# KTH-RPL/neural_graph_mapping

Hardware: AMD Instinct MI355X
Metric: ray-samples/sec (train step: fwd+loss+bwd+Adam, 4096 rays x 128 samples per GPU) (higher is better)
Workload: dtype f32 via 3xbf16 split, fp32 accumulate (hidden-layer matrix products, forward and backward); everything else f32; 1 GPU; M1: 8 fields x 512 rays x (64 coarse + 64 depth-guided) samples per GPU, Fourier(64,raw)+2x64 MLP, nrgbd compositing, NRGBD intrinsics; fields_per_gpu=8, rays_per_field=512, samples_per_ray=128, ranks_seen=1, spin_up_steps=200, jitter=in-kernel Philox, launch=hipGraph replay

## Files before the change

include/ngm_hip.h:

```cpp
#ifndef NGM_HIP_H
#define NGM_HIP_H

#include <stdint.h>

#ifdef __cplusplus
extern "C" {
#endif

#define NGM_ABI_VERSION 11
#define NGM_MAX_LAYERS 4
#define NGM_NUM_LOSS_SUMS 16

enum ngm_status {
  NGM_OK = 0,
  NGM_E_INVALID = -1,
  NGM_E_UNSUPPORTED = -2,
  NGM_E_WORKSPACE = -3,
  NGM_E_HIP = -4
};

enum ngm_encoding { NGM_ENC_NONE = 0, NGM_ENC_FOURIER = 1, NGM_ENC_NERF = 2, NGM_ENC_PERMUTO = 3, NGM_ENC_TRIPLANE = 4 };
enum ngm_triplane_mode { NGM_TRI_SUM = 0, NGM_TRI_PRODUCT = 1, NGM_TRI_CONCAT = 2 };
enum ngm_skip_mode { NGM_SKIP_NO = 0, NGM_SKIP_ADD = 1, NGM_SKIP_CONCAT = 2 };
enum ngm_matmul_mode { NGM_MATMUL_F32 = 0, NGM_MATMUL_BF16X3 = 1, NGM_MATMUL_AUTO = 2 };
// ... 11 lines not shown
  NGM_LS_TSDF_SUM = 6,
  NGM_LS_TSDF_CNT = 7,
  NGM_LS_TERM_SUM = 8,
  NGM_LS_TERM_CNT = 9,
  NGM_LS_PHOTO_L1_SUM = 10
};

typedef struct ngm_field_cfg {
  int32_t encoding;
  int32_t dim_enc;
  int32_t raw_coords;
  int32_t num_octaves;
  int32_t start_octave;
  int32_t num_layers;
  int32_t dim_hidden;
  int32_t dim_out;
  int32_t scale_mode;
  float field_radius;
  int32_t nr_levels;
  int32_t nr_feat_per_level;
  int32_t log2_hashmap_size;
  float coarsest_scale, finest_scale;
  float level_scale[16 * 3];
  int32_t skip_mode;
  int32_t matmul_mode;
  int32_t tri_resolution;
  int32_t tri_mode;
  int32_t activation_stash;
  int32_t hash_grad_atomics;
} ngm_field_cfg;
enum ngm_activation_stash { NGM_STASH_FULL = 0, NGM_STASH_HALF = 1 };
enum ngm_hash_grad_atomics { NGM_HASH_ATOMICS_EXACT = 0, NGM_HASH_ATOMICS_FLOAT = 1 };

int ngm_permuto_fill_scales(ngm_field_cfg* cfg);

typedef struct ngm_params {
  const float* enc_w;
  int64_t enc_w_stride;
  const float* w[NGM_MAX_LAYERS + 1];
  int64_t w_stride[NGM_MAX_LAYERS + 1];
  const float* b[NGM_MAX_LAYERS + 1];
  int64_t b_stride[NGM_MAX_LAYERS + 1];
  const int64_t* field_index;
  const float* lattice;
  int64_t lattice_stride;
  const float* shift;
  int64_t shift_stride;
  int32_t dtype;
  int32_t reserved_;
  const float* planes;
  int64_t planes_stride;
  const float* neus_sd;
  int64_t neus_sd_stride;
} ngm_params;

typedef struct ngm_grads {
  float* enc_w;
  int64_t enc_w_stride;
  float* w[NGM_MAX_LAYERS + 1];
  int64_t w_stride[NGM_MAX_LAYERS + 1];
  float* b[NGM_MAX_LAYERS + 1];
  int64_t b_stride[NGM_MAX_LAYERS + 1];
  float* lattice;
  int64_t lattice_stride;
  float* neus_sd;
  float* planes;
  int64_t planes_stride;
} ngm_grads;

typedef enum ngm_photometric_mode { NGM_PHOTO_L1 = 0, NGM_PHOTO_L2 = 1, NGM_PHOTO_GAUSSIAN_NLL = 2 } ngm_photometric_mode;
typedef enum ngm_depth_mode { NGM_DEPTH_HUBER = 0, NGM_DEPTH_GAUSSIAN_NLL = 1, NGM_DEPTH_LAPLACIAN_NLL = 2 } ngm_depth_mode;

typedef struct ngm_render_cfg {
  int32_t geometry_mode;
  int32_t num_samples_coarse;
  int32_t num_samples_guided;
  int32_t overwrite_behind_camera;
  float geometry_factor;
  float color_factor;
  float truncation_distance;
  float range_depth_guided;
  float fx, fy, cx, cy;
  float w_termination, w_photometric, w_depth, w_freespace, w_tsdf;
  float huber_delta;
  float term_threshold;
  int32_t photometric_mode;
  int32_t depth_mode;
} ngm_render_cfg;

typedef struct ngm_rays {
  int32_t F, R;
  const int64_t* ijs;
  const float* c2ws;
  int32_t c2w_per_ray;
  int32_t philox_offset_autoinc;
  const float* near;
  const float* far;
  const float* gt;
  float near_const, far_const;
  const float* field_pos;
  const float* field_quat;
  const float* u_coarse;
  const float* u_guided;
  const float* lin_coarse;
  const float* lin_guided;
  uint64_t philox_seed;
// ... 61 lines not shown
int ngm_composite_bwd(const ngm_render_cfg* cfg, int64_t N, int32_t S, const float* colors,
                      const float* geoms, const float* dists, const float* depths,
                      const float* neus_isds, const float* dC, const float* dD,
                      const float* dterm, float* d_colors, float* d_geoms, float* d_neus_isds,
                      void* stream);

int64_t ngm_render_workspace(const ngm_field_cfg* fcfg, const ngm_render_cfg* rcfg, int32_t F,
                             int32_t R, int32_t train);
int ngm_render_fwd(const ngm_field_cfg* fcfg, const ngm_render_cfg* rcfg,
                   const ngm_params* params, const ngm_rays* rays, const ngm_targets* targets,
                   const ngm_prediction* pred, float* loss_sums, void* workspace,
                   int64_t workspace_bytes, void* stream);
int ngm_render_bwd(const ngm_field_cfg* fcfg, const ngm_render_cfg* rcfg,
                   const ngm_params* params, const ngm_rays* rays, const ngm_targets* targets,
                   const ngm_prediction* pred, const float* loss_sums, const ngm_grads* grads,
                   float* loss_out, void* workspace, int64_t workspace_bytes, void* stream);
int ngm_render_bwd_seeded(const ngm_field_cfg* fcfg, const ngm_render_cfg* rcfg,
                          const ngm_params* params, const ngm_rays* rays, const float* d_rgbds,
                          const float* d_term, const float* d_geom_samples,
                          const ngm_grads* grads, void* workspace, int64_t workspace_bytes,
                          void* stream);
int ngm_render_bwd_seeded_vars(const ngm_field_cfg* fcfg, const ngm_render_cfg* rcfg,
                               const ngm_params* params, const ngm_rays* rays, const ngm_prediction* pred,
                               const float* d_rgbds, const float* d_color_vars, const float* d_depth_vars,
                               const float* d_term, const float* d_geom_samples, const ngm_grads* grads,
                               void* workspace, int64_t workspace_bytes, void* stream);
int ngm_render_read_samples(const ngm_field_cfg* fcfg, const ngm_render_cfg* rcfg, int32_t F,
                            int32_t R, int32_t S, const void* workspace, float* geoms, float* dists,
                            void* stream);

int ngm_adam_sparse(float* param, float* exp_avg, float* exp_avg_sq, int64_t stride,
                    const float* grad, int64_t grad_stride, const int64_t* field_index, int32_t F,
                    int64_t numel_per_field, int64_t step, float lr, float beta1, float beta2,
                    float eps, float weight_decay, void* stream);

typedef struct ngm_adam_tensor {
  float* param; float* exp_avg; float* exp_avg_sq;
  const float* grad;
  int64_t stride, grad_stride, numel;
  void* param_lp;
  int32_t lp_dtype;
  int32_t reserved_;
} ngm_adam_tensor;
int ngm_adam_sparse_multi(const ngm_adam_tensor* tensors, int32_t num_tensors, const int64_t* field_index,
                          int32_t F, int64_t step, int64_t* step_dev, float lr, float beta1, float beta2,
                          float eps, float weight_decay, int32_t advance_step_dev,
                          uint64_t* advance_philox_offset_dev, void* stream);
int ngm_render_bwd_adam(const ngm_field_cfg* fcfg, const ngm_render_cfg* rcfg, const ngm_params* params,
                        const ngm_rays* rays, const ngm_targets* targets, const ngm_prediction* pred,
                        const float* loss_sums, const ngm_grads* grads, const ngm_adam_tensor* mlp_tensors,
                        int32_t num_mlp_tensors, const ngm_adam_tensor* lattice_tensor, const int64_t* field_index,
                        int64_t step, int64_t* step_dev, float lr, float beta1, float beta2, float eps,
                        float weight_decay, float* loss_values, void* workspace, int64_t workspace_bytes, void* stream);
int ngm_render_fwd_counted(const ngm_field_cfg* fcfg, const ngm_render_cfg* rcfg,
                           const ngm_params* params, const ngm_rays* rays, const ngm_targets* targets,
                           const ngm_prediction* pred, float* loss_sums, void* workspace,
                           int64_t workspace_bytes, void* stream, const int32_t* num_active);
int ngm_render_bwd_counted(const ngm_field_cfg* fcfg, const ngm_render_cfg* rcfg,
                           const ngm_params* params, const ngm_rays* rays, const ngm_targets* targets,
                           const ngm_prediction* pred, const float* loss_sums, const ngm_grads* grads,
                           float* loss_out, void* workspace, int64_t workspace_bytes, void* stream,
                           const int32_t* num_active);
int ngm_render_bwd_adam_counted(const ngm_field_cfg* fcfg, const ngm_render_cfg* rcfg, const ngm_params* params,
                                const ngm_rays* rays, const ngm_targets* targets, const ngm_prediction* pred,
                                const float* loss_sums, const ngm_grads* grads, const ngm_adam_tensor* mlp_tensors,
                                int32_t num_mlp_tensors, const ngm_adam_tensor* lattice_tensor, const int64_t* field_index,
                                int64_t step, int64_t* step_dev, float lr, float beta1, float beta2, float eps,
                                float weight_decay, float* loss_values, void* workspace, int64_t workspace_bytes, void* stream,
                                const int32_t* num_active);
int ngm_step_advance(int64_t* step_dev, uint64_t* philox_offset_dev, void* stream);

int64_t ngm_field_eval_knn_workspace(int32_t num_fields, int64_t P, int32_t num_knn);
int ngm_field_eval_knn(const ngm_field_cfg* fcfg, const ngm_params* params, int32_t num_fields,
                       int64_t P, const float* points, const float* field_pos,
                       const float* field_quat, int32_t num_knn, float distance_factor,
                       float outside_value, float mask_radius, float* out, void* workspace, int64_t workspace_bytes,
                       void* stream);

int64_t ngm_render_eval_knn_workspace(const ngm_render_cfg* rcfg, int32_t num_fields, int32_t ray_block, int32_t num_knn);
int ngm_render_eval_knn(const ngm_field_cfg* fcfg, const ngm_render_cfg* rcfg, const ngm_params* params,
                        int32_t num_fields, const float* field_pos, const float* field_quat, const ngm_rays* rays,
                        int32_t num_knn, float distance_factor, float outside_value, float mask_radius, int32_t ray_block,
                        const ngm_prediction* pred, void* workspace, int64_t workspace_bytes, void* stream);

typedef struct ngm_keyframes {
  int32_t num_frames;
  int32_t height, width;
  int32_t reserved0;
  const float* c2ws;
  const float* rgbd;
  const int64_t* frame_to_store;
  float fx, fy, cx, cy;
} ngm_keyframes;

typedef struct ngm_target_out {
  int64_t* ijs;
  float* c2ws;
  float* near;
  float* far;
  float* gt;
  float* rgbds;
  uint8_t* rgb_mask;
  uint8_t* depth_mask;
  float* term_probs;
  uint8_t* term_mask;
} ngm_target_out;
// ... 174 lines not shown
```

neural_graph_mapping_amd/_capi.py:

```python
import ctypes as C
import os

HERE = os.path.dirname(os.path.abspath(__file__))
LIB_PATH = os.environ.get("NGM_LIB_PATH") or os.path.join(HERE, "lib", "libngm_hip.so")

NGM_MAX_LAYERS = 4
NGM_NUM_LOSS_SUMS = 16
ENC = {"none": 0, "fourier": 1, "nerf": 2, "permuto": 3, "triplane": 4}
TRI = {"sum": 0, "product": 1, "concat": 2}
SCALE = {"no": 0, "unit_ball": 1, "unit_cube": 2}
GEO = {"nrgbd": 0, "occupancy": 1, "density": 2, "neus": 3}
PHOTO = {"l1": 0, "l2": 1, "gaussian_nll": 2}
DEPTH = {"huber": 0, "gaussian_nll": 1, "laplacian_nll": 2}
LS = dict(PHOTO_SUM=0, PHOTO_CNT=1, DEPTH_SUM=2, DEPTH_CNT=3, FS_SUM=4, FS_CNT=5, TSDF_SUM=6,
          TSDF_CNT=7, TERM_SUM=8, TERM_CNT=9, PHOTO_L1_SUM=10)

f32p = C.c_void_p
LArr = C.c_void_p * (NGM_MAX_LAYERS + 1)
SArr = C.c_int64 * (NGM_MAX_LAYERS + 1)


class FieldCfg(C.Structure):
    _fields_ = [("encoding", C.c_int32), ("dim_enc", C.c_int32), ("raw_coords", C.c_int32),
                ("num_octaves", C.c_int32), ("start_octave", C.c_int32), ("num_layers", C.c_int32),
                ("dim_hidden", C.c_int32), ("dim_out", C.c_int32), ("scale_mode", C.c_int32),
                ("field_radius", C.c_float), ("nr_levels", C.c_int32), ("nr_feat_per_level", C.c_int32),
                ("log2_hashmap_size", C.c_int32), ("coarsest_scale", C.c_float), ("finest_scale", C.c_float),
                ("level_scale", C.c_float * 48), ("skip_mode", C.c_int32), ("matmul_mode", C.c_int32),
                ("tri_resolution", C.c_int32), ("tri_mode", C.c_int32),
                ("activation_stash", C.c_int32), ("hash_grad_atomics", C.c_int32)]


class Params(C.Structure):
    _fields_ = [("enc_w", f32p), ("enc_w_stride", C.c_int64), ("w", LArr), ("w_stride", SArr),
                ("b", LArr), ("b_stride", SArr), ("field_index", C.c_void_p),
                ("lattice", f32p), ("lattice_stride", C.c_int64), ("shift", f32p), ("shift_stride", C.c_int64),
                ("dtype", C.c_int32), ("reserved_", C.c_int32), ("planes", f32p), ("planes_stride", C.c_int64),
                ("neus_sd", f32p), ("neus_sd_stride", C.c_int64)]


class Grads(C.Structure):
    _fields_ = [("enc_w", f32p), ("enc_w_stride", C.c_int64), ("w", LArr), ("w_stride", SArr),
                ("b", LArr), ("b_stride", SArr), ("lattice", f32p), ("lattice_stride", C.c_int64), ("neus_sd", f32p),
                ("planes", f32p), ("planes_stride", C.c_int64)]


class RenderCfg(C.Structure):
    _fields_ = [("geometry_mode", C.c_int32), ("num_samples_coarse", C.c_int32),
                ("num_samples_guided", C.c_int32), ("overwrite_behind_camera", C.c_int32),
                ("geometry_factor", C.c_float), ("color_factor", C.c_float),
                ("truncation_distance", C.c_float), ("range_depth_guided", C.c_float),
                ("fx", C.c_float), ("fy", C.c_float), ("cx", C.c_float), ("cy", C.c_float),
                ("w_termination", C.c_float), ("w_photometric", C.c_float), ("w_depth", C.c_float),
                ("w_freespace", C.c_float), ("w_tsdf", C.c_float), ("huber_delta", C.c_float),
                ("term_threshold", C.c_float), ("photometric_mode", C.c_int32), ("depth_mode", C.c_int32)]


class Rays(C.Structure):
    _fields_ = [("F", C.c_int32), ("R", C.c_int32), ("ijs", C.c_void_p), ("c2ws", f32p),
                ("c2w_per_ray", C.c_int32), ("philox_offset_autoinc", C.c_int32), ("near", f32p), ("far", f32p),
                ("gt", f32p), ("near_const", C.c_float), ("far_const", C.c_float),
                ("field_pos", f32p), ("field_quat", f32p), ("u_coarse", f32p), ("u_guided", f32p),
                ("lin_coarse", f32p), ("lin_guided", f32p), ("philox_seed", C.c_uint64),
                ("philox_offset", C.c_uint64), ("pose_index", C.c_void_p), ("philox_offset_dev", C.c_void_p)]


class AdamTensor(C.Structure):
    _fields_ = [("param", f32p), ("exp_avg", f32p), ("exp_avg_sq", f32p), ("grad", f32p),
                ("stride", C.c_int64), ("grad_stride", C.c_int64), ("numel", C.c_int64),
                ("param_lp", C.c_void_p), ("lp_dtype", C.c_int32), ("reserved_", C.c_int32)]


class PeerExchange(C.Structure):
    _fields_ = [("world", C.c_int32), ("rank", C.c_int32), ("mailbox", C.c_void_p * 8), ("seq", C.c_void_p),
                ("status", C.c_void_p)]


class Targets(C.Structure):
    _fields_ = [("rgbds", f32p), ("depth_mask", C.c_void_p), ("term_mask", C.c_void_p),
                ("term_probs", f32p)]


class Prediction(C.Structure):
    _fields_ = [("rgbds", f32p), ("color_vars", f32p), ("depth_vars", f32p), ("term_probs", f32p)]


class Keyframes(C.Structure):
    _fields_ = [("num_frames", C.c_int32), ("height", C.c_int32), ("width", C.c_int32), ("reserved0", C.c_int32),
                ("c2ws", f32p), ("rgbd", f32p), ("frame_to_store", C.c_void_p),
                ("fx", C.c_float), ("fy", C.c_float), ("cx", C.c_float), ("cy", C.c_float)]

# ... 85 lines not shown
def grow_counts(num_current, num_fields, max_current, max_fields, num_train_fields):
    nf = min(max(num_fields, 0), max_fields)
    nc = min(max(num_current, 0), min(max_current, nf))
    n_obs = min(num_train_fields // 2, nc)
    return nf, nc, n_obs, max(min(num_train_fields - n_obs, nf - n_obs), 0)


_lib = None


def lib():
    global _lib
    if _lib is not None:
        return _lib
    if not os.path.exists(LIB_PATH):
        raise RuntimeError(
            f"{LIB_PATH} is missing: the HIP extension is not built. Run "
            "`python -m neural_graph_mapping_amd.build` (hipcc, gfx950). There is no CPU fallback.")
    L = C.CDLL(LIB_PATH)
    vp, i32, i64, f32 = C.c_void_p, C.c_int32, C.c_int64, C.c_float
    P = C.POINTER
    L.ngm_abi_version.restype = C.c_int
    L.ngm_permuto_fill_scales.argtypes = [P(FieldCfg)]
    L.ngm_permuto_fill_scales.restype = C.c_int
    L.ngm_last_error.restype = C.c_char_p
    L.ngm_device_info.argtypes = [P(C.c_int), C.c_char_p, C.c_int]
    L.ngm_sample_rays.argtypes = [P(RenderCfg), P(Rays), vp, vp, vp, vp]
    L.ngm_sample_rays_world.argtypes = [P(RenderCfg), P(Rays), vp, vp, vp, vp, vp]
    L.ngm_sample_rays_weighted.argtypes = [P(RenderCfg), P(Rays), i32, vp, vp, vp, vp, vp, vp]
    L.ngm_sample_rays_weighted.restype = C.c_int
    L.ngm_composite_fwd_packed.argtypes = [P(RenderCfg), i64, i32, vp, vp, vp, vp, vp, vp, vp, vp]
    L.ngm_sample_rays_world.restype = C.c_int
    L.ngm_composite_fwd_packed.restype = C.c_int
    L.ngm_field_eval_fwd.argtypes = [P(FieldCfg), P(Params), i32, i64, vp, vp, vp, vp, vp]
    L.ngm_encode_fwd.argtypes = [P(FieldCfg), P(Params), i32, i64, vp, vp, vp, vp, vp]
    L.ngm_encode_fwd.restype = C.c_int
    L.ngm_encode_bwd.argtypes = [P(FieldCfg), P(Params), i32, i64, vp, vp, vp, vp, P(Grads), vp, i64, vp]
    L.ngm_encode_bwd.restype = C.c_int
    L.ngm_encode_bwd_workspace.argtypes = [P(FieldCfg), i32, i64]
    L.ngm_encode_bwd_workspace.restype = i64
    L.ngm_field_eval_bwd.argtypes = [P(FieldCfg), P(Params), i32, i64, vp, vp, vp, vp, P(Grads), vp, i64, vp]
    L.ngm_field_eval_bwd_workspace.argtypes = [P(FieldCfg), i32, i64]
    L.ngm_field_eval_bwd_workspace.restype = i64
    L.ngm_field_eval_stash_bytes.argtypes = [P(FieldCfg), i32, i64]
    L.ngm_field_eval_stash_bytes.restype = i64
    L.ngm_field_eval_fwd_train.argtypes = [P(FieldCfg), P(Params), i32, i64, vp, vp, vp, vp, vp, i64, vp]
    L.ngm_field_eval_fwd_train.restype = C.c_int
    L.ngm_field_eval_bwd_stash.argtypes = [P(FieldCfg), P(Params), i32, i64, vp, vp, vp, vp, P(Grads), vp, i64, vp, i64, vp]
    L.ngm_field_eval_bwd_stash.restype = C.c_int
    L.ngm_composite_fwd.argtypes = [P(RenderCfg), i64, i32] + [vp] * 11 + [vp]
    L.ngm_composite_bwd.argtypes = [P(RenderCfg), i64, i32] + [vp] * 11 + [vp]
    L.ngm_render_workspace.argtypes = [P(FieldCfg), P(RenderCfg), i32, i32, i32]
    L.ngm_render_workspace.restype = i64
    L.ngm_render_fwd.argtypes = [P(FieldCfg), P(RenderCfg), P(Params), P(Rays), P(Targets),
                                 P(Prediction), vp, vp, i64, vp]
    L.ngm_render_bwd.argtypes = [P(FieldCfg), P(RenderCfg), P(Params), P(Rays), P(Targets),
                                 P(Prediction), vp, P(Grads), vp, vp, i64, vp]
    L.ngm_render_bwd_seeded.argtypes = [P(FieldCfg), P(RenderCfg), P(Params), P(Rays), vp, vp, vp,
                                        P(Grads), vp, i64, vp]
    L.ngm_render_bwd_seeded_vars.argtypes = [P(FieldCfg), P(RenderCfg), P(Params), P(Rays), P(Prediction), vp, vp, vp, vp, vp,
                                             P(Grads), vp, i64, vp]
    L.ngm_render_bwd_seeded_vars.restype = C.c_int
    L.ngm_render_bwd_adam.argtypes = [P(FieldCfg), P(RenderCfg), P(Params), P(Rays), P(Targets), P(Prediction), vp,
                                      P(Grads), P(AdamTensor), i32, P(AdamTensor), vp, i64, vp, f32, f32, f32, f32, f32,
                                      vp, vp, i64, vp]
    L.ngm_render_bwd_adam.restype = C.c_int
    for name in ("ngm_render_fwd", "ngm_render_bwd", "ngm_render_bwd_adam"):
        counted = getattr(L, name + "_counted")
        counted.argtypes = list(getattr(L, name).argtypes) + [vp]
        counted.restype = C.c_int
    L.ngm_render_read_samples.argtypes = [P(FieldCfg), P(RenderCfg), i32, i32, i32, vp, vp, vp, vp]
    L.ngm_adam_sparse.argtypes = [vp, vp, vp, i64, vp, i64, vp, i32, i64, i64, f32, f32, f32, f32, f32, vp]
    L.ngm_adam_sparse_multi.argtypes = [P(AdamTensor), i32, vp, i32, i64, vp, f32, f32, f32, f32, f32, i32, vp, vp]
    L.ngm_step_advance.argtypes = [vp, vp, vp]
    L.ngm_peer_mailbox_bytes.restype = i64
    L.ngm_peer_alloc.argtypes = [i64, P(C.c_void_p)]
    L.ngm_peer_free.argtypes = [vp]
    L.ngm_ipc_export.argtypes = [vp, C.c_char_p]
    L.ngm_ipc_open.argtypes = [C.c_char_p, P(C.c_void_p)]
    L.ngm_ipc_close.argtypes = [vp]
    L.ngm_loss_exchange.argtypes = [P(PeerExchange), vp, vp]
    L.ngm_peer_set_timeout.argtypes = [C.c_double]
    L.ngm_peer_set_timeout.restype = C.c_double
    L.ngm_adam_sparse_multi.restype = C.c_int
    L.ngm_step_advance.restype = C.c_int
    L.ngm_field_eval_knn.argtypes = [P(FieldCfg), P(Params), i32, i64, vp, vp, vp, i32, f32, f32, f32, vp, vp, i64, vp]
    L.ngm_field_eval_knn_workspace.argtypes = [i32, i64, i32]
    L.ngm_field_eval_knn_workspace.restype = i64
    L.ngm_render_eval_knn.argtypes = [P(FieldCfg), P(RenderCfg), P(Params), i32, vp, vp, P(Rays), i32, f32, f32, f32, i32,
                                      P(Prediction), vp, i64, vp]
    L.ngm_render_eval_knn.restype = C.c_int
    L.ngm_render_eval_knn_workspace.argtypes = [P(RenderCfg), i32, i32, i32]
    L.ngm_render_eval_knn_workspace.restype = i64
    L.ngm_target_visibility.argtypes = [P(Keyframes), i32, vp, i32, vp, f32, vp, vp, vp]
    L.ngm_target_rays.argtypes = [P(Keyframes), i32, i32, vp, f32, vp, vp, vp, P(TargetOut), vp]
    L.ngm_target_visibility.restype = C.c_int
    L.ngm_target_rays.restype = C.c_int
    L.ngm_target_sv_intersect.argtypes = [i32, i64, vp, vp, f32, vp, vp]
    L.ngm_target_sv_intersect.restype = C.c_int
    L.ngm_target_sv_rays.argtypes = [i32, i32, vp, f32, vp, vp, vp, i32, i32, f32, f32, f32, f32, P(TargetOut), vp]
    L.ngm_target_sv_rays.restype = C.c_int
    L.ngm_target_sample_mv_workspace.argtypes = [i32, i32, i32, i32]
    L.ngm_target_sample_mv_workspace.restype = i64
    L.ngm_target_sample_mv.argtypes = [P(Keyframes), P(TargetSample), P(TargetOut), vp, i64, vp]
    L.ngm_target_sample_mv.restype = C.c_int
    L.ngm_target_sample_mv_live_workspace.argtypes = [i32, i32, i32, i32]
    L.ngm_target_sample_mv_live_workspace.restype = i64
    L.ngm_target_sample_mv_live.argtypes = [P(Keyframes), P(TargetSample), P(TargetLive), P(TargetOut), vp, i64, vp]
    L.ngm_target_sample_mv_live.restype = C.c_int
    L.ngm_target_observed_fields_workspace.argtypes = [i32, i32]
    L.ngm_target_observed_fields_workspace.restype = i64
    L.ngm_target_observed_fields.argtypes = [P(ObservedFields), vp, i64, vp]
    L.ngm_target_observed_fields.restype = C.c_int
    L.ngm_field_counts_add.argtypes = [vp, vp, i32, vp, i32, vp]
    L.ngm_field_counts_add.restype = C.c_int
    L.ngm_fields_append.argtypes = [P(FieldsAppendArgs), vp]
    L.ngm_fields_append.restype = C.c_int
    L.ngm_target_sample_mv_grow_workspace.argtypes = [i32, i32, i32, i32]
    L.ngm_target_sample_mv_grow_workspace.restype = i64
    L.ngm_target_sample_mv_grow.argtypes = [P(Keyframes), P(TargetSample), P(TargetLive), vp, P(TargetOut), vp, i64, vp]
    L.ngm_target_sample_mv_grow.restype = C.c_int
    L.ngm_target_observed_fields_grow_workspace.argtypes = [i32, i32]
    L.ngm_target_observed_fields_grow_workspace.restype = i64
    L.ngm_target_observed_fields_grow.argtypes = [P(ObservedFields), vp, vp, i64, vp]
    L.ngm_target_observed_fields_grow.restype = C.c_int
    L.ngm_marching_cubes_workspace.argtypes = [i32, i32, i32]
    L.ngm_marching_cubes_workspace.restype = i64
    L.ngm_marching_cubes_count.argtypes = [vp, i32, i32, i32, f32, vp, vp, i64, vp]
    L.ngm_marching_cubes_emit.argtypes = [vp, i32, i32, i32, f32, vp, i64, vp, i64, vp, i64, vp]
    L.ngm_marching_cubes_tables.argtypes = [vp, vp]
    for name in ("ngm_marching_cubes_count", "ngm_marching_cubes_emit", "ngm_marching_cubes_tables"):
        getattr(L, name).restype = C.c_int
    L.ngm_debug_plan_bwd.argtypes = [P(FieldCfg), P(RenderCfg), i32, i64, i32, i32, i32, P(i32)]
    L.ngm_debug_plan_bwd.restype = C.c_int
    L.ngm_debug_plan_fwd.argtypes = [P(FieldCfg), P(RenderCfg), i32, i32, i64, i32, P(i32)]
    L.ngm_debug_plan_fwd.restype = C.c_int
    L.ngm_profile_enable.argtypes = [i32]
    L.ngm_profile_read.argtypes = [i32, P(C.c_double), P(i64)]
    for name in ("ngm_profile_enable", "ngm_profile_reset", "ngm_profile_read"):
        getattr(L, name).restype = C.c_int
    for name in ("ngm_sample_rays", "ngm_field_eval_fwd", "ngm_field_eval_bwd", "ngm_composite_fwd",
                 "ngm_composite_bwd", "ngm_render_fwd", "ngm_render_bwd", "ngm_render_bwd_seeded",
                 "ngm_render_read_samples", "ngm_adam_sparse", "ngm_field_eval_knn", "ngm_device_info"):
        getattr(L, name).restype = C.c_int
    _lib = L
    return L


EXPORTED = ["ngm_abi_version", "ngm_last_error", "ngm_device_info", "ngm_permuto_fill_scales", "ngm_sample_rays", "ngm_sample_rays_world", "ngm_sample_rays_weighted",
            "ngm_composite_fwd_packed",
            "ngm_field_eval_fwd", "ngm_encode_fwd", "ngm_encode_bwd", "ngm_encode_bwd_workspace", "ngm_field_eval_bwd", "ngm_field_eval_bwd_workspace",
            "ngm_field_eval_stash_bytes", "ngm_field_eval_fwd_train", "ngm_field_eval_bwd_stash",
            "ngm_composite_fwd", "ngm_composite_bwd", "ngm_render_workspace", "ngm_render_fwd",
            "ngm_render_bwd", "ngm_render_bwd_adam", "ngm_render_bwd_seeded", "ngm_render_bwd_seeded_vars", "ngm_render_read_samples", "ngm_adam_sparse",
            "ngm_field_eval_knn", "ngm_field_eval_knn_workspace", "ngm_render_eval_knn", "ngm_render_eval_knn_workspace", "ngm_adam_sparse_multi", "ngm_step_advance", "ngm_profile_enable", "ngm_profile_reset", "ngm_profile_read",
            "ngm_debug_phase_cycles", "ngm_debug_fwd_phase_cycles", "ngm_debug_last_bwd_variant", "ngm_debug_last_matmul", "ngm_debug_last_fwd_one_tile", "ngm_debug_last_comp_fused", "ngm_debug_disable_fused_comp", "ngm_debug_stash_mode", "ngm_debug_last_stash_mode", "ngm_debug_plan_bwd", "ngm_debug_plan_fwd", "ngm_target_visibility", "ngm_target_rays", "ngm_target_sv_intersect", "ngm_target_sv_rays",
            "ngm_target_sample_mv_workspace", "ngm_target_sample_mv",
            "ngm_target_sample_mv_live_workspace", "ngm_target_sample_mv_live", "ngm_target_observed_fields_workspace",
            "ngm_target_observed_fields", "ngm_field_counts_add",
            "ngm_fields_append", "ngm_target_sample_mv_grow_workspace", "ngm_target_sample_mv_grow",
            "ngm_target_observed_fields_grow_workspace", "ngm_target_observed_fields_grow",
            "ngm_render_fwd_counted", "ngm_render_bwd_counted", "ngm_render_bwd_adam_counted",
            "ngm_peer_mailbox_bytes", "ngm_peer_alloc", "ngm_peer_free", "ngm_ipc_export", "ngm_ipc_open", "ngm_ipc_close", "ngm_loss_exchange", "ngm_peer_set_timeout",
            "ngm_marching_cubes_workspace", "ngm_marching_cubes_count", "ngm_marching_cubes_emit", "ngm_marching_cubes_tables"]

NO_GRAD_PARAMS = frozenset({"_encoding.random_shift_per_level"})

KERNEL_IDS = dict(render_fwd=0, stash_bwd=1, field_bwd=2, grad_reduce=3, adam=4, points_fwd=5, composite_fwd=6,
                  composite_bwd=7, hash_grad=8, hash_reduce=9, loss_reduce=10, knn_assign=11, knn_eval=12, sampler=13)


NGM_OK, NGM_E_INVALID, NGM_E_UNSUPPORTED, NGM_E_WORKSPACE, NGM_E_HIP = 0, -1, -2, -3, -4


class NgmError(RuntimeError):

    def __init__(self, msg, code=None):
        super().__init__(msg)
        self.code = code


def check(rc, what=""):
    if rc != 0:
        msg = lib().ngm_last_error().decode(errors="replace")
        raise NgmError(f"{what} failed with status {rc}: {msg}", code=int(rc))


SKIP = {"no": 0, "add": 1, "concat": 2}
STASH = {"full": 0, "half": 1}
HASH_ATOMICS = {"exact": 0, "float": 1}
MATMUL = {"f32": 0, "bf16x3": 1, "auto": 2}


def field_cfg(encoding="fourier", dim_enc=64, raw_coords=True, num_octaves=8, start_octave=0,
              num_layers=2, dim_hidden=None, dim_out=4, scale_mode="unit_cube", field_radius=1.0,
              nr_levels=16, nr_feat_per_level=2, log2_hashmap_size=12, coarsest_scale=1.0, finest_scale=1e-4,
              skip_mode="no", matmul_mode="f32", resolution=32, num_components=64, tri_mode="sum"):
    if skip_mode not in SKIP:
        raise NotImplementedError(f"skip_mode={skip_mode!r}: 'no', 'add' and 'concat' have kernels; the reference's own "
                                  "constructor raises for 'rezero' (models.py:131-132)")
    if encoding == "nerf":
        dim_enc = 6 * num_octaves
    if encoding == "none":
        dim_enc = 3
    if encoding == "permuto":
        dim_enc = nr_levels * nr_feat_per_level
# ... 104 lines not shown
```

neural_graph_mapping_amd/csrc/ngm_api.hip:

```cpp
#include <hip/hip_runtime.h>
#include <stdio.h>
#include <stdlib.h>
#include <string.h>

#include "../../include/ngm_hip.h"
#include "ngm_launch.h"

int ngm_launch_sampler_weighted(const ngm_render_cfg* rc, const ngm_rays* rays, int S, int B, const float* boundaries,
                                const float* weights, float* points_cam, float* distances, float* dirs, hipStream_t st);
int ngm_launch_sampler(const ngm_render_cfg* rc, const ngm_rays* rays, int S, float* points_cam, float* distances,
                       float* dirs, float* points_world, hipStream_t st);
int ngm_launch_loss_values(const ngm_render_cfg* rc, const float* sums, float* out, hipStream_t st);
int ngm_launch_loss_reduce(const float* partials, int nblocks, float* sums, uint64_t* counter, hipStream_t st);
int ngm_launch_neus_sd_grad(const float* d_isd_rays, int F, int R, const float* neus_sd, int64_t sd_stride,
                            const int64_t* field_index, float* d_sd, hipStream_t st);
int ngm_launch_read_stash(const float4* sa, const float2* sb, int64_t n, float* geoms, float* dists, hipStream_t st);
int ngm_launch_adam(float* param, float* m, float* v, int64_t stride, const float* grad, int64_t gstride, int F, int64_t numel,
                    const AdamHyper& h, hipStream_t st);
int ngm_launch_adam_multi(const ngm_adam_tensor* tensors, int n, int F, const AdamHyper& h, int64_t* advance_step,
                          uint64_t* advance_offset, hipStream_t st, const int32_t* num_active = nullptr);
int ngm_launch_step_advance(int64_t* step_dev, uint64_t* off_dev, hipStream_t st);
int64_t ngm_mc_workspace_bytes(int nx, int ny, int nz);
int ngm_launch_mc_count(const float* vol, int nx, int ny, int nz, float iso, int64_t* counts, void* workspace,
                        int64_t workspace_bytes, hipStream_t st);
// ... 286 lines not shown
  switch (p.variant) {
    case 3: e = ngm_launch_field_bwd_b3(a, blocks, st); break;
    case 5: e = ngm_launch_hash_mlp_bwd(a, blocks, st); break;
    case 2: e = ngm_launch_field_bwd16s(a, blocks, st); break;
    case 1: e = ngm_launch_field_bwd16(a, blocks, st); break;
    case 0: e = ngm_launch_field_bwd(a, blocks, st); break;
  }
  return e ? fail(e, "MLP backward: the launcher does not take the planned problem (internal error)") : check_launch("ngm_field_bwd");
}

static int check_field_cfg(const ngm_field_cfg* fc, bool mlp = true) {
  if (!fc) return fail(NGM_E_INVALID, "field cfg is NULL");
  if (fc->dim_out != 4) return fail(NGM_E_UNSUPPORTED, "dim_out must be 4 (r,g,b,geometry)");
  if (fc->num_layers < 1 || fc->num_layers > NGM_MAX_LAYERS) return fail(NGM_E_UNSUPPORTED, "num_layers out of range");
  if (mlp && fc->num_layers > 3)
    return fail(NGM_E_UNSUPPORTED, "num_layers = 4: no entry point has a kernel for four hidden layers (1-2: everything; 3: forward only, 33..64-wide)");
  if (mlp && fc->num_layers == 3 && (fc->dim_enc <= 32 || fc->dim_hidden <= 32))
    return fail(NGM_E_UNSUPPORTED, "num_layers = 3 needs dim_enc and dim_hidden in 33..64: no entry point has a three-layer kernel for layers of 32 units or fewer");
  if (fc->encoding == NGM_ENC_PERMUTO) {
    if (fc->nr_feat_per_level != 2 || fc->nr_levels < 1 || fc->nr_levels > 16 || fc->dim_enc != 2 * fc->nr_levels)
      return fail(NGM_E_UNSUPPORTED, "permutohedral encoding: nr_feat_per_level must be 2, nr_levels <= 16, no concat_points");
    if (fc->log2_hashmap_size < 4 || fc->log2_hashmap_size > 24) return fail(NGM_E_UNSUPPORTED, "permutohedral: log2_hashmap_size out of range");
    if (!(fc->level_scale[0] > 0.f)) return fail(NGM_E_INVALID, "permutohedral: level_scale not filled (ngm_permuto_fill_scales)");
  }
  if (fc->encoding == NGM_ENC_NERF && fc->dim_enc != 6 * fc->num_octaves) return fail(NGM_E_INVALID, "nerf: dim_enc != 6*octaves");
  if (fc->encoding == NGM_ENC_TRIPLANE) {
    if (fc->tri_resolution < 2 || fc->tri_resolution > 4096 || fc->tri_mode < NGM_TRI_SUM || fc->tri_mode > NGM_TRI_CONCAT ||
        (fc->tri_mode == NGM_TRI_CONCAT && fc->dim_enc % 3))
      return fail(NGM_E_INVALID, "triplane: resolution / mode / dim_enc inconsistent");
  }
  if (fc->encoding == NGM_ENC_NONE && fc->dim_enc != 3) return fail(NGM_E_INVALID, "no encoding: dim_enc must be 3");
  if (fc->dim_enc < 1 || fc->dim_enc > 64 || fc->dim_hidden < 1 || fc->dim_hidden > 64)
    return fail(NGM_E_UNSUPPORTED, "dim_enc / dim_hidden must be <= 64");
  if (((fc->dim_enc + 31) / 32) != ((fc->dim_hidden + 31) / 32) && !(fc->dim_enc <= 32 && fc->dim_hidden <= 32))
    return fail(NGM_E_UNSUPPORTED, "dim_enc and dim_hidden must pad to the same multiple of 32");
  if (fc->skip_mode != NGM_SKIP_NO && fc->skip_mode != NGM_SKIP_ADD && fc->skip_mode != NGM_SKIP_CONCAT)
    return fail(NGM_E_UNSUPPORTED, "skip_mode: no / add / concat");
  if (fc->skip_mode == NGM_SKIP_ADD && fc->dim_hidden < fc->dim_enc)
    return fail(NGM_E_UNSUPPORTED, "skip_mode add: needs dim_hidden >= dim_enc");
  if (fc->activation_stash != NGM_STASH_FULL && fc->activation_stash != NGM_STASH_HALF)
    return fail(NGM_E_INVALID, "activation_stash: NGM_STASH_FULL / NGM_STASH_HALF (ABI 10: is the struct the caller built 276 bytes?)");
  if (fc->hash_grad_atomics != NGM_HASH_ATOMICS_EXACT && fc->hash_grad_atomics != NGM_HASH_ATOMICS_FLOAT)
    return fail(NGM_E_INVALID, "hash_grad_atomics: NGM_HASH_ATOMICS_EXACT / NGM_HASH_ATOMICS_FLOAT");
  return NGM_OK;
}
static int check_params(const ngm_field_cfg* fc, const ngm_params* pr) {
  if (!pr) return fail(NGM_E_INVALID, "params is NULL");
  if (fc->encoding == NGM_ENC_FOURIER && !pr->enc_w) return fail(NGM_E_INVALID, "fourier encoding needs enc_w");
  if (fc->encoding == NGM_ENC_PERMUTO && (!pr->lattice || !pr->shift)) return fail(NGM_E_INVALID, "permutohedral encoding needs lattice + shift");
  if (fc->encoding == NGM_ENC_TRIPLANE && (!pr->planes || pr->dtype != NGM_DT_F32)) return fail(NGM_E_INVALID, "triplane encoding needs fp32 planes");
  for (int l = 0; l <= fc->num_layers; ++l)
    if (!pr->w[l] || !pr->b[l]) return fail(NGM_E_INVALID, "missing layer weight/bias pointer");
  if (pr->dtype != NGM_DT_F32 && pr->dtype != NGM_DT_BF16 && pr->dtype != NGM_DT_F16) return fail(NGM_E_INVALID, "params.dtype");
  return NGM_OK;
}

extern "C" {

int ngm_abi_version(void) { return NGM_ABI_VERSION; }

int ngm_permuto_fill_scales(ngm_field_cfg* cfg) {
  if (!cfg || cfg->nr_levels < 1 || cfg->nr_levels > 16 || !(cfg->coarsest_scale > 0) || !(cfg->finest_scale > 0))
    return fail(NGM_E_INVALID, "ngm_permuto_fill_scales: bad configuration");
  const int L = cfg->nr_levels;
  const double la = log10((double)cfg->coarsest_scale), lb = log10((double)cfg->finest_scale);
  for (int l = 0; l < L; ++l) {
    double sig = (L == 1) ? cfg->coarsest_scale : pow(10.0, la + (lb - la) * (double)l / (double)(L - 1));
    if (l == 0) sig = cfg->coarsest_scale;
    if (l == L - 1 && L > 1) sig = cfg->finest_scale;
    for (int i = 0; i < 3; ++i) cfg->level_scale[3 * l + i] = (float)((1.0 / sqrt((double)((i + 1) * (i + 2)))) / sig);
  }
  return NGM_OK;
}
const char* ngm_last_error(void) { return g_err; }

int ngm_profile_enable(int32_t on) {
  std::lock_guard<std::mutex> lk(g_prof_mu);
  g_prof_on = on != 0;
  return NGM_OK;
}
int ngm_profile_reset(void) {
  std::lock_guard<std::mutex> lk(g_prof_mu);
  prof_drain();
  for (int k = 0; k < NGM_K_COUNT; ++k) { g_prof_ms[k] = 0; g_prof_n[k] = 0; }
  return NGM_OK;
}
int ngm_profile_read(int32_t kernel_id, double* total_ms, int64_t* launches) {
  if (kernel_id < 0 || kernel_id >= NGM_K_COUNT) return fail(NGM_E_INVALID, "bad kernel id");
  std::lock_guard<std::mutex> lk(g_prof_mu);
  prof_drain();
  if (total_ms) *total_ms = g_prof_ms[kernel_id];
  if (launches) *launches = g_prof_n[kernel_id];
  return NGM_OK;
}

static int check_keyframes(const ngm_keyframes* kf) {
  if (!kf || !kf->c2ws || !kf->rgbd || !kf->frame_to_store) return fail(NGM_E_INVALID, "target sampler: NULL keyframe argument");
  if (kf->num_frames < 1 || kf->height < 1 || kf->width < 1) return fail(NGM_E_INVALID, "target sampler: empty keyframe set");
  return NGM_OK;
}
int ngm_target_visibility(const ngm_keyframes* kf, int32_t F, const float* field_pos, int32_t num_offsets, const float* offsets,
                          float radius, uint8_t* kf_mask, float* bbox, void* stream) {
  int e = check_keyframes(kf);
  if (e) return e;
  if (F < 0 || num_offsets < 1 || !field_pos || !offsets || !kf_mask || !bbox) return fail(NGM_E_INVALID, "ngm_target_visibility: bad argument");
  if (F == 0) return NGM_OK;
// ... 451 lines not shown
  if (!cfg || !colors || !geoms || !dists || !depths || N < 0) return fail(NGM_E_INVALID, "ngm_composite_bwd: bad argument");
  if (N == 0) return NGM_OK;
  CompositeArgs a;
  memset(&a, 0, sizeof(a));
  a.rc = *cfg; a.N = N; a.S = S; a.colors = colors; a.geoms = geoms; a.dists = dists; a.depths = depths; a.isds = neus_isds;
  a.dC = dC; a.dD = dD; a.dterm = dterm; a.d_colors = d_colors; a.d_geoms = d_geoms; a.d_isds = d_neus_isds;
  const int rc = ngm_launch_composite_bwd(a, (hipStream_t)stream);
  if (rc) return fail(rc, "ngm_composite_bwd: S > 1024");
  return check_launch("ngm_composite_bwd");
}

struct RenderPlan {
  int S;
  FwdPlan fwd;
  BwdPlan bwd;
  int64_t p_pad;
  int64_t off_rayseed;
  int64_t off_raytab, off_stashA, off_stashB, off_losspart, off_gradpart, off_hash, off_act, act_layer_stride, total;
  int64_t off_dout, off_disd;
};
static RenderPlan plan_render(const ngm_field_cfg* fc, const ngm_render_cfg* rc, int F, int R, bool guided, bool train,
                              BwdAsk ask = BwdAsk(), bool counted = false) {
  RenderPlan p = RenderPlan();
  p.S = rc->num_samples_coarse + (guided ? rc->num_samples_guided : 0);
  FwdAsk fq;
  fq.rc = rc; fq.F = F; fq.n = R; fq.S = p.S; fq.counted = counted;
  p.fwd = plan_fwd(fc, fq);
  p.p_pad = param_pad(fc);
  int64_t o = 0;
  if (train) {
    const int64_t NR = (int64_t)F * R, NS = NR * p.S;
    p.off_raytab = o; o = align_up(o + NR * 8 * 4, 256);
    p.off_rayseed = o; o = align_up(o + NR * 8 * 4, 256);
    p.off_stashA = o; o = align_up(o + NS * 16, 256);
    p.off_stashB = o; o = align_up(o + NS * 8, 256);
    p.off_losspart = o; o = align_up(o + (int64_t)p.fwd.blocks * NGM_NUM_LOSS_SUMS * 4, 256);
    if (rc->geometry_mode == NGM_GEO_NEUS) {
      p.off_dout = o; o = align_up(o + NS * 16, 256);
      p.off_disd = o; o = align_up(o + NR * 4, 256);
    }
    ask.rc = rc; ask.F = F; ask.P = (int64_t)R * p.S;
    p.bwd = plan_mlp_bwd(fc, ask);
    p.off_gradpart = o; o = align_up(o + (int64_t)F * p.bwd.blocks_per_field * p.p_pad * 4, 256);
    p.off_hash = o; o = align_up(o + hash_scratch_bytes(fc, F, (int64_t)R * p.S), 256);
    if (p.bwd.stash_kind) {
      p.act_layer_stride = p.bwd.stash_kind == 1 ? align_up(NS, 32) * 64 + 2048 : align_up(NS, 32) * 32 + 1024;
      p.off_act = o; o = align_up(o + p.bwd.stash_layers * p.act_layer_stride * 4 + 64, 256);
    }
  }
  p.total = o + 256;
  return p;
}

int64_t ngm_render_workspace(const ngm_field_cfg* fcfg, const ngm_render_cfg* rcfg, int32_t F, int32_t R, int32_t train) {
  const int e = check_field_cfg(fcfg);
  if (e) return e;
  if (!rcfg || F < 1 || R < 1) return NGM_E_INVALID;
  return plan_render(fcfg, rcfg, F, R, true, train != 0).total;
}

static int check_enc_grads(const ngm_field_cfg* fc, const ngm_grads* grads, FieldBwdArgs& a) {
  if (fc->encoding == NGM_ENC_TRIPLANE) {
    if (!grads->planes || grads->planes_stride < tri_numel(fc)) return fail(NGM_E_INVALID, "triplane: grads.planes missing / stride too small");
    if (!a.tri_acc) return fail(NGM_E_WORKSPACE, "triplane: no accumulator scratch");
    a.planes_grad = grads->planes; a.planes_grad_stride = grads->planes_stride;
    return NGM_OK;
  }
  if (fc->encoding != NGM_ENC_PERMUTO) return NGM_OK;
  if (!grads->lattice) return fail(NGM_E_INVALID, "permutohedral: grads.lattice is NULL");
  const int64_t per = (int64_t)fc->nr_levels * ((int64_t)1 << fc->log2_hashmap_size) * 2;
  if (grads->lattice_stride < per) return fail(NGM_E_INVALID, "permutohedral: grads.lattice_stride too small");
  a.lattice_grad = grads->lattice; a.lattice_grad_stride = grads->lattice_stride;
  return NGM_OK;
}

static int check_render(const ngm_field_cfg* fc, const ngm_render_cfg* rc, const ngm_params* pr, const ngm_rays* rays) {
  int e = check_field_cfg(fc);
  if (e) return e;
  e = check_params(fc, pr);
  if (e) return e;
  if (!rc || !rays || !rays->ijs || !rays->c2ws || !rays->field_pos || !rays->field_quat)
    return fail(NGM_E_INVALID, "render: NULL ray argument");
  if (rays->F < 1 || rays->R < 1) return fail(NGM_E_INVALID, "render: empty batch");
  if (rc->geometry_mode == NGM_GEO_NEUS && !pr->neus_sd)
    return fail(NGM_E_INVALID, "fused render: the neus geometry mode needs params.neus_sd (the per-field _neus_sd, rm.py:641-644)");
  const int S = rc->num_samples_coarse + (rays->gt ? rc->num_samples_guided : 0);
  if (S < 1 || S > 1024) return fail(NGM_E_UNSUPPORTED, "fused render: samples per ray must be in [1,1024]");
  return NGM_OK;
}

static int check_counted(const char* who, const ngm_field_cfg* fc, const ngm_render_cfg* rc, const int32_t* num_active) {
  char msg[256];
  if (!num_active) {
    snprintf(msg, sizeof(msg), "%s: num_active is NULL (the un-suffixed entry point is the call for all F rows)", who);
    return fail(NGM_E_INVALID, msg);
  }
  const char* why = nullptr;
  if (rc && rc->geometry_mode == NGM_GEO_NEUS) why = "the neus geometry mode";
  else if (fc && fc->encoding == NGM_ENC_TRIPLANE) why = "the triplane encoding";
  else if (rc && (rc->photometric_mode == NGM_PHOTO_GAUSSIAN_NLL || rc->depth_mode != NGM_DEPTH_HUBER)) why = "the *_nll loss modes";
  if (why) {
    snprintf(msg, sizeof(msg), "%s: %s is outside the counted step (it launches over all F rows): slice the batch to its count and call the un-suffixed entry point", who, why);
    return fail(NGM_E_UNSUPPORTED, msg);
  }
  return NGM_OK;
}

static int render_fwd_impl(const ngm_field_cfg* fcfg, const ngm_render_cfg* rcfg, const ngm_params* params, const ngm_rays* rays,
                           const ngm_targets* targets, const ngm_prediction* pred, float* loss_sums, void* workspace,
                           int64_t workspace_bytes, void* stream, const int32_t* num_active) {
  int e = check_render(fcfg, rcfg, params, rays);
  if (e) return e;
  if (!pred) return fail(NGM_E_INVALID, "render_fwd: pred is NULL");
  const bool has_tg = targets != nullptr;
  const bool save = workspace != nullptr;
  if (has_tg && (!targets->rgbds || !targets->depth_mask)) return fail(NGM_E_INVALID, "render_fwd: incomplete targets");
  if (has_tg && targets->term_mask && !targets->term_probs) return fail(NGM_E_INVALID, "render_fwd: term_mask without term_probs");
  if (has_tg && !save) return fail(NGM_E_WORKSPACE, "render_fwd: targets need a workspace");
  if (save && (!pred->rgbds || !pred->term_probs)) return fail(NGM_E_INVALID, "render_fwd(save): pred.rgbds/term_probs required");
  const RenderPlan p = plan_render(fcfg, rcfg, rays->F, rays->R, rays->gt != nullptr, save, BwdAsk(), num_active != nullptr);
  if (p.fwd.status) return fail(p.fwd.status, p.fwd.why);
  if (save && workspace_bytes < p.total) return fail(NGM_E_WORKSPACE, "render_fwd: workspace too small");
  char* ws = reinterpret_cast<char*>(align_up((int64_t)workspace, 256));
  RenderFwdArgs a;
  memset(&a, 0, sizeof(a));
  a.fc = *fcfg; a.pr = *params; a.rc = *rcfg; a.rays = *rays; a.pred = *pred;
  a.fc.matmul_mode = p.fwd.matmul;
  if (p.fwd.neus) { a.neus_sd = params->neus_sd; a.neus_sd_stride = params->neus_sd_stride; }
  a.has_targets = has_tg ? 1 : 0;
  a.num_active = num_active;
  if (has_tg) a.tg = *targets;
  a.S = p.S; a.rays_per_block = p.fwd.rays_per_block; a.waves_per_block = p.fwd.waves; a.maxs = p.fwd.maxs;
  if (save) {
    a.raytab = reinterpret_cast<float*>(ws + p.off_raytab);
    if (has_tg) a.rayseed = reinterpret_cast<float*>(ws + p.off_rayseed);
    a.stashA = reinterpret_cast<float4*>(ws + p.off_stashA);
    a.stashB = reinterpret_cast<float2*>(ws + p.off_stashB);
    a.loss_partials = reinterpret_cast<float*>(ws + p.off_losspart);
    if (p.act_layer_stride) { a.act = reinterpret_cast<float*>(ws + p.off_act); a.act_layer_stride = p.act_layer_stride; }
    a.act_layers = p.bwd.half;
    static const bool timing = getenv("NGM_PHASE_TIMING") != nullptr;
    if (timing) {
      if (!g_debug_cycles_fwd) { (void)hipMalloc(&g_debug_cycles_fwd, NGM_FWD_DEBUG_WORDS * 8); (void)hipMemset(g_debug_cycles_fwd, 0, NGM_FWD_DEBUG_WORDS * 8); }
      a.debug_cycles = g_debug_cycles_fwd;
    }
  }
  e = ngm_launch_render_fwd(a, p.fwd, (hipStream_t)stream);
  if (e) return fail(e, no_instance);
  g_last_fwd[NGM_FWD_RENDER] = p.fwd;
  if (save) {
    note_forward_stash(workspace, p.bwd.half);
    note_forward_seeds(workspace, a.rayseed ? targets->rgbds : nullptr);
  }
  e = check_launch("ngm_render_fwd");
  if (e) return e;
  if (has_tg && loss_sums) {
    ngm_launch_loss_reduce(a.loss_partials, p.fwd.blocks, loss_sums,
                           (rays->philox_offset_autoinc && rays->philox_offset_dev) ? const_cast<uint64_t*>(rays->philox_offset_dev) : nullptr,
                           (hipStream_t)stream);
    e = check_launch("ngm_loss_reduce");
  }
  return e;
}
int ngm_render_fwd(const ngm_field_cfg* fcfg, const ngm_render_cfg* rcfg, const ngm_params* params, const ngm_rays* rays,
                   const ngm_targets* targets, const ngm_prediction* pred, float* loss_sums, void* workspace,
                   int64_t workspace_bytes, void* stream) {
  return render_fwd_impl(fcfg, rcfg, params, rays, targets, pred, loss_sums, workspace, workspace_bytes, stream, nullptr);
}
int ngm_render_fwd_counted(const ngm_field_cfg* fcfg, const ngm_render_cfg* rcfg, const ngm_params* params, const ngm_rays* rays,
                           const ngm_targets* targets, const ngm_prediction* pred, float* loss_sums, void* workspace,
                           int64_t workspace_bytes, void* stream, const int32_t* num_active) {
  const int e = check_counted("ngm_render_fwd_counted", fcfg, rcfg, num_active);
  if (e) return e;
  return render_fwd_impl(fcfg, rcfg, params, rays, targets, pred, loss_sums, workspace, workspace_bytes, stream, num_active);
// ... 14 lines not shown
    return fail(NGM_E_INVALID, "render_bwd: the *_nll loss modes need pred.color_vars and pred.depth_vars");
  char* ws = reinterpret_cast<char*>(align_up((int64_t)workspace, 256));
  FieldBwdArgs a;
  memset(&a, 0, sizeof(a));
  a.fc = *fcfg; a.pr = *params; a.F = rays->F; a.P = (int64_t)rays->R * p.S; a.S = p.S;
  a.num_active = num_active;
  carve_hash_scratch(fcfg, rays->F, a.P, ws + p.off_hash, a);
  int e = check_enc_grads(fcfg, grads, a);
  if (e) return e;
  sb.rc = *rcfg; sb.F = rays->F; sb.R = rays->R; sb.S = p.S;
  sb.num_active = num_active;
  if (!rays->gt) sb.rc.w_freespace = sb.rc.w_tsdf = 0.f;
  sb.stashA = reinterpret_cast<float4*>(ws + p.off_stashA);
  sb.stashB = reinterpret_cast<const float2*>(ws + p.off_stashB);
  sb.raytab = reinterpret_cast<const float*>(ws + p.off_raytab);
  const bool neus = rcfg->geometry_mode == NGM_GEO_NEUS;
  if (neus) {
    sb.neus_sd = params->neus_sd; sb.neus_sd_stride = params->neus_sd_stride; sb.field_index = params->field_index;
    sb.d_out = reinterpret_cast<float4*>(ws + p.off_dout);
    sb.d_isd_rays = reinterpret_cast<float*>(ws + p.off_disd);
  }
  if (sb.seed_mode == 0 && !sb.loss_sums) {
    sb.loss_partials = reinterpret_cast<const float*>(ws + p.off_losspart);
    sb.n_partials = p.fwd.blocks;
    sb.counter = (rays->philox_offset_autoinc && rays->philox_offset_dev)
                     ? reinterpret_cast<unsigned long long*>(const_cast<uint64_t*>(rays->philox_offset_dev)) : nullptr;
  }
  a.per_block = p.bwd.per_block; a.blocks_per_field = p.bwd.blocks_per_field;
  a.raytab = sb.raytab; a.stashB = sb.stashB; a.d_out = neus ? sb.d_out : sb.stashA;
  a.partials = reinterpret_cast<float*>(ws + p.off_gradpart); a.p_pad = p.p_pad;
  if (p.bwd.stash_kind) { a.act = reinterpret_cast<const float*>(ws + p.off_act); a.act_layer_stride = p.act_layer_stride; a.act_half = p.bwd.half; }
  if (p.bwd.fused_comp) {
    a.fused_comp = 1; a.rc = sb.rc;
    a.rayseed = reinterpret_cast<const float*>(ws + p.off_rayseed);
    a.loss_sums = sb.loss_sums; a.loss_partials = sb.loss_partials; a.n_partials = sb.n_partials;
    a.sums_out = sb.sums_out; a.loss_out = sb.loss_out; a.counter = sb.counter;
  } else {
    sb.xyz_out = a.hash_xyz;
    a.hash_xyz_ready = a.hash_xyz != nullptr;
    e = ngm_launch_stash_bwd(sb, st);
    if (e) return fail(e, "render_bwd: unsupported geometry mode");
    e = check_launch("ngm_stash_bwd");
    if (e) return e;
  }
  if (neus && grads->neus_sd)
    ngm_launch_neus_sd_grad(sb.d_isd_rays, rays->F, rays->R, params->neus_sd, params->neus_sd_stride, params->field_index,
                            grads->neus_sd, st);
  if (a.tri_acc) (void)hipMemsetAsync(a.tri_acc, 0, (size_t)a.F * a.tri_numel * 8, st);
  e = launch_mlp_bwd(p.bwd, a, st);
  if (e) return e;
  if (fcfg->encoding == NGM_ENC_TRIPLANE) { ngm_launch_tri_finish(a, st); e = check_launch("ngm_tri_finish"); if (e) return e; }
  GradReduceArgs g;
  memset(&g.adam, 0, sizeof(g.adam));
  if (adam) g.adam = *adam;
  g.num_active = num_active;
  g.fc = *fcfg; g.gr = *grads; g.F = rays->F; g.blocks_per_field = a.blocks_per_field; g.partials = a.partials; g.p_pad = a.p_pad;
  bool mlp_reduced = false;
  if (fcfg->encoding == NGM_ENC_PERMUTO) {
    if (lattice_adam) a.lattice_adam = *lattice_adam;
    e = ngm_launch_hash_grad(a, st, lattice_adam_applied, &g, &mlp_reduced);
    if (e == NGM_E_INVALID) return fail(e, "render_bwd_adam: adam tensors do not match the parameter segments");
    if (e) return fail(e, "permutohedral backward: hash table too large for the LDS-staged scatter");
    e = check_launch("ngm_hash_grad");
    if (e) return e;
  }
  if (mlp_reduced) return NGM_OK;
  if (ngm_launch_grad_reduce(g, st)) return fail(NGM_E_INVALID, "render_bwd_adam: adam tensors do not match the parameter segments");
  return check_launch("ngm_grad_reduce");
}

static int render_bwd_impl(const ngm_field_cfg* fcfg, const ngm_render_cfg* rcfg, const ngm_params* params, const ngm_rays* rays,
                           const ngm_targets* targets, const ngm_prediction* pred, const float* loss_sums, const ngm_grads* grads,
                           float* loss_out, void* workspace, int64_t workspace_bytes, void* stream, const int32_t* num_active) {
  int e = check_render(fcfg, rcfg, params, rays);
  if (e) return e;
  if (!targets || !targets->rgbds || !targets->depth_mask || !pred || !pred->rgbds || !pred->term_probs || !grads)
    return fail(NGM_E_INVALID, "render_bwd: NULL argument");
  StashBwdArgs sb;
  memset(&sb, 0, sizeof(sb));
  sb.seed_mode = 0; sb.tg = *targets; sb.pred = *pred; sb.loss_sums = loss_sums;
  sb.loss_out = loss_out;
  return render_bwd_common(fcfg, rcfg, params, rays, sb, grads, workspace, workspace_bytes, (hipStream_t)stream, nullptr, nullptr,
                           nullptr, num_active);
}
int ngm_render_bwd(const ngm_field_cfg* fcfg, const ngm_render_cfg* rcfg, const ngm_params* params, const ngm_rays* rays,
                   const ngm_targets* targets, const ngm_prediction* pred, const float* loss_sums, const ngm_grads* grads,
                   float* loss_out, void* workspace, int64_t workspace_bytes, void* stream) {
  return render_bwd_impl(fcfg, rcfg, params, rays, targets, pred, loss_sums, grads, loss_out, workspace, workspace_bytes, stream,
                         nullptr);
}
int ngm_render_bwd_counted(const ngm_field_cfg* fcfg, const ngm_render_cfg* rcfg, const ngm_params* params, const ngm_rays* rays,
                           const ngm_targets* targets, const ngm_prediction* pred, const float* loss_sums, const ngm_grads* grads,
                           float* loss_out, void* workspace, int64_t workspace_bytes, void* stream, const int32_t* num_active) {
  const int e = check_counted("ngm_render_bwd_counted", fcfg, rcfg, num_active);
  if (e) return e;
  return render_bwd_impl(fcfg, rcfg, params, rays, targets, pred, loss_sums, grads, loss_out, workspace, workspace_bytes, stream,
                         num_active);
}

static int render_bwd_adam_impl(const ngm_field_cfg* fcfg, const ngm_render_cfg* rcfg, const ngm_params* params, const ngm_rays* rays,
                                const ngm_targets* targets, const ngm_prediction* pred, const float* loss_sums, const ngm_grads* grads,
                                const ngm_adam_tensor* mlp_tensors, int32_t num_mlp_tensors, const ngm_adam_tensor* lattice_tensor,
                                const int64_t* field_index, int64_t step, int64_t* step_dev, float lr, float beta1, float beta2,
                                float eps, float weight_decay, float* loss_out, void* workspace, int64_t workspace_bytes,
                                void* stream, const int32_t* num_active) {
  int e = check_render(fcfg, rcfg, params, rays);
  if (e) return e;
// ... 296 lines not shown
```

neural_graph_mapping_amd/csrc/ngm_field.h:

```cpp
#pragma once
#include "ngm_device.h"

#define NGM_FK_ZERO 0.0f
#define NGM_FK_RAW 1.0f
#define NGM_FK_SIN 2.0f
#define NGM_FK_COS 3.0f

template <int MI, int MH, int L, bool CAT = false>
struct FieldLds {
  static constexpr int MIN(int l) { return l == 0 ? MI : (CAT ? MH + MI : MH); }
  static constexpr int MOUT_IN = CAT ? MH + MI : MH;
  static constexpr int ENCW = 0;
  static constexpr int ENCW_SIZE = MI * 32 * 4;
  static constexpr int w_off(int l) {
    int o = ENCW + ENCW_SIZE;
    for (int i = 0; i < l; ++i) o += wfrag_size(MH, MIN(i)) + MH * 32;
    return o;
  }
  static constexpr int b_off(int l) { return w_off(l) + wfrag_size(MH, MIN(l)); }
  static constexpr int WOUT = b_off(L - 1) + MH * 32;
  static constexpr int BOUT = WOUT + MOUT_IN * 32 * 4;
  static constexpr int TOTAL = (BOUT + 4 + 3) & ~3;
};

// ... 474 lines not shown

__device__ __forceinline__ void b3_split8(const float (&x)[8], ngm_bf16x8& H, ngm_bf16x8& M, ngm_bf16x8& Lo) {
#ifdef NGM_ABLB_NOSPLIT
  H = __builtin_bit_cast(ngm_bf16x8, ngm_u32x4{__float_as_uint(x[0]), __float_as_uint(x[1]), __float_as_uint(x[2]), __float_as_uint(x[3])});
  M = __builtin_bit_cast(ngm_bf16x8, ngm_u32x4{__float_as_uint(x[4]), __float_as_uint(x[5]), __float_as_uint(x[6]), __float_as_uint(x[7])});
  Lo = H;
  return;
#endif
  ngm_u32x4 h4, m4, l4;
#pragma unroll
  for (int p = 0; p < 4; ++p) {
    uint32_t h0, m0, l0, h1, m1, l1;
    b3_split(x[2 * p], h0, m0, l0);
    b3_split(x[2 * p + 1], h1, m1, l1);
    h4[p] = b3_pack(h0, h1); m4[p] = b3_pack(m0, m1); l4[p] = b3_pack(l0, l1);
  }
  H = __builtin_bit_cast(ngm_bf16x8, h4); M = __builtin_bit_cast(ngm_bf16x8, m4); Lo = __builtin_bit_cast(ngm_bf16x8, l4);
}

template <int MIN, int MOUT>
struct B3Planes {
  static constexpr int KB = 2 * MIN;
  static constexpr int PLANE = MOUT * KB * 2 * 32;
  static constexpr int LAYER = 3 * PLANE;
  static constexpr int idx(int p, int mo, int kb, int kh, int io) { return p * PLANE + ((mo * KB + kb) * 2 + kh) * 32 + io; }
};
template <int MI, int MH, int L>
struct B3Lds {
  static constexpr int off(int l) { return l == 0 ? 0 : B3Planes<MI, MH>::LAYER + (l - 1) * B3Planes<MH, MH>::LAYER; }
  static constexpr int TOTAL = off(L);
};

template <int MI, int MH, int L>
__device__ __forceinline__ void b3_build_planes(const float* sm, ngm_u32x4* planes) {
  using LY = FieldLds<MI, MH, L, false>;
#pragma unroll
  for (int l = 0; l < L; ++l) {
    const int MIN = (l == 0) ? MI : MH, KB = 2 * MIN;
    const float* W = sm + LY::w_off(l);
    ngm_u32x4* P = planes + B3Lds<MI, MH, L>::off(l);
    const int plane = MH * KB * 2 * 32;
    for (int e4 = threadIdx.x; e4 < plane; e4 += blockDim.x) {
      const int io = e4 & 31, kh = (e4 >> 5) & 1, kb = (e4 >> 6) % KB, mo = (e4 >> 6) / KB;
      const int mi = kb >> 1, b = kb & 1;
      float x[8];
#pragma unroll
      for (int e = 0; e < 8; ++e) x[e] = W[((((mo * MIN + mi) * 16 + 8 * b + e) * 2 + kh) * NGM_WGS) + io];
      ngm_bf16x8 H, M, Lo;
      b3_split8(x, H, M, Lo);
      P[e4] = __builtin_bit_cast(ngm_u32x4, H);
      P[plane + e4] = __builtin_bit_cast(ngm_u32x4, M);
      P[2 * plane + e4] = __builtin_bit_cast(ngm_u32x4, Lo);
    }
  }
}

__device__ __forceinline__ f32x16 mfma_bf16(ngm_bf16x8 a, ngm_bf16x8 b, f32x16 c) {
#ifdef NGM_ABLB_NOMFMA
  const ngm_u32x4 ua = __builtin_bit_cast(ngm_u32x4, a), ub = __builtin_bit_cast(ngm_u32x4, b);
  c[0] += __uint_as_float((ua[0] ^ ub[1]) & 0x3fffffffu);
  return c;
#endif
  return __builtin_amdgcn_mfma_f32_32x32x16_bf16(a, b, c, 0, 0, 0);
}

struct ActStash {
  float* base;
  int64_t layer_stride;
  int64_t g0;
  int nvalid;
  int nlayers;
};

template <int MIN, int MOUT, int NT>
__device__ __forceinline__ void layer_fwd_b3(const ngm_u32x4* __restrict__ P, const float* __restrict__ B, int lane,
                                             const f32x16 (&X)[NT][MIN], f32x16 (&Y)[NT][MOUT]) {
  using PL = B3Planes<MIN, MOUT>;
  const int io = lane & 31, hi = lane >> 5;
#pragma unroll
  for (int mo = 0; mo < MOUT; ++mo)
#pragma unroll
    for (int q = 0; q < 4; ++q) {
      const float4 b4 = *reinterpret_cast<const float4*>(B + 32 * mo + 8 * q + 4 * hi);
#pragma unroll
      for (int nt = 0; nt < NT; ++nt) {
        Y[nt][mo][4 * q] = b4.x; Y[nt][mo][4 * q + 1] = b4.y; Y[nt][mo][4 * q + 2] = b4.z; Y[nt][mo][4 * q + 3] = b4.w;
      }
    }
#pragma unroll
  for (int kb = 0; kb < PL::KB; ++kb) {
    const int mi = kb >> 1, b = kb & 1;
    ngm_bf16x8 ah[MOUT], am[MOUT], al[MOUT];
#pragma unroll
    for (int mo = 0; mo < MOUT; ++mo) {
      ah[mo] = __builtin_bit_cast(ngm_bf16x8, P[PL::idx(0, mo, kb, hi, io)]);
      am[mo] = __builtin_bit_cast(ngm_bf16x8, P[PL::idx(1, mo, kb, hi, io)]);
      al[mo] = __builtin_bit_cast(ngm_bf16x8, P[PL::idx(2, mo, kb, hi, io)]);
    }
    ngm_bf16x8 bh[NT], bm[NT], bl[NT];
#pragma unroll
    for (int nt = 0; nt < NT; ++nt) {
      float x[8];
#pragma unroll
      for (int e = 0; e < 8; ++e) x[e] = X[nt][mi][8 * b + e];
      b3_split8(x, bh[nt], bm[nt], bl[nt]);
    }
// ... 254 lines not shown
```

neural_graph_mapping_amd/csrc/ngm_field_bwd.hip:

```cpp
#include <stdlib.h>
#include <string.h>
#include <algorithm>
#include "ngm_field.h"
#include "ngm_launch.h"

#define WAVE_SYNC()                                        \
  do {                                                     \
    __builtin_amdgcn_fence(__ATOMIC_RELEASE, "wavefront"); \
    __builtin_amdgcn_wave_barrier();                       \
    __builtin_amdgcn_fence(__ATOMIC_ACQUIRE, "wavefront"); \
  } while (0)

template <int MI, int MH, int L, bool CAT = false>
struct BwdLds {
  using LY = FieldLds<MI, MH, L, CAT>;
  static constexpr int STR_E = 32 * MI + 4;
  static constexpr int STR_H = 32 * MH + 4;
  static constexpr int STR_D = (STR_E > STR_H) ? STR_E : STR_H;
  static constexpr int X0 = 0;
  static constexpr int x_off(int l) { return l == 0 ? 0 : 32 * STR_E + (l - 1) * 32 * STR_H; }
  static constexpr int DBUF = 32 * STR_E + (L - 1) * 32 * STR_H;
  static constexpr int PBUF = DBUF + 32 * STR_D;
  static constexpr int OBUF = PBUF + 128;
  static constexpr int WAVE_TOTAL = OBUF + 128;
// ... 417 lines not shown
      for (int mo = 0; mo < MH; ++mo) {
#pragma unroll
        for (int r = 0; r < 16; ++r) {
          const int o = 32 * mo + frow(r, hi);
          if (o < H) {
#pragma unroll
            for (int mi = 0; mi < MI; ++mi) {
              const int i = 32 * mi + j;
              if (i < D) red[w_off[0] + (int64_t)o * D + i] += acc0[mo][mi][r];
            }
#pragma unroll
            for (int l = 1; l < L; ++l) {
#pragma unroll
              for (int mi = 0; mi < MH; ++mi) {
                const int i = 32 * mi + j;
                if (i < H) red[w_off[l] + (int64_t)o * DC + i] += accH[l - 1][mo][mi][r];
              }
              if constexpr (CAT) {
#pragma unroll
                for (int mi = 0; mi < MI; ++mi) {
                  const int i = 32 * mi + j;
                  if (i < D) red[w_off[l] + (int64_t)o * DC + H + i] += accE[l - 1][mo][mi][r];
                }
              }
            }
          }
        }
      }
      if (lane < 32 * MH && lane < H) {
#pragma unroll
        for (int l = 0; l < L; ++l) red[b_off[l] + lane] += dbh[l];
#pragma unroll
        for (int c = 0; c < 4; ++c) red[w_off[L] + (int64_t)c * DC + lane] += dwo[c];
      }
      if (CAT && lane < 32 * MI && lane < D) {
#pragma unroll
        for (int c = 0; c < 4; ++c) red[w_off[L] + (int64_t)c * DC + H + lane] += dwoE[c];
      }
      if (lane < 4) red[b_off[L] + lane] += (lane == 0 ? dbo[0] : lane == 1 ? dbo[1] : lane == 2 ? dbo[2] : dbo[3]);
      if (ENC_GRAD && a.fc.encoding == NGM_ENC_FOURIER) {
        const int n_raw = a.fc.raw_coords ? 3 : 0;
        if (lane < 32 * MI && lane < D && lane >= n_raw) {
#pragma unroll
          for (int c = 0; c < 3; ++c) red[enc_off + (int64_t)(lane - n_raw) * 3 + c] += dwf[c];
        }
      }
    }
    __syncthreads();
  }
  float* dst = a.partials + (int64_t)blockIdx.x * a.p_pad;
  for (int64_t p = threadIdx.x; p < ptot; p += NGM_BLOCK) dst[p] = red[p];
}

struct GradSeg { int64_t off, size; float* dst; int64_t stride; float* param; float* m; float* v; int64_t pstride; void* lp; int lp_dt; };
struct GradReduceK {
  int F, blocks_per_field, nseg;
  const float* partials;
  int64_t p_pad, ptot;
  GradSeg seg[2 * (NGM_MAX_LAYERS + 1) + 1];
  AdamHyper hyper;
  const int32_t* num_active;
};

template <bool COUNTED>
__global__ void __launch_bounds__(256) k_grad_reduce(GradReduceK a) {
  __shared__ float part[4][64];
  const int f = blockIdx.y, q = threadIdx.x >> 6, l = threadIdx.x & 63;
  if constexpr (COUNTED) {
    if (f >= *a.num_active) return;
  }
  const int64_t p = (int64_t)blockIdx.x * 64 + l;
  int seg = -1;
  int64_t so = 0;
  float pv = 0.f, m0 = 0.f, v0 = 0.f;
  AdamCoef co = {0.f, 1.f};
  const bool adam = q == 0 && p < a.ptot;
  if (adam) {
    for (int k = 0; k < a.nseg; ++k)
      if (p >= a.seg[k].off && p < a.seg[k].off + a.seg[k].size) { seg = k; break; }
    if (seg >= 0 && a.seg[seg].param) {
      const int64_t row = a.hyper.field_index ? a.hyper.field_index[f] : f;
      so = row * a.seg[seg].pstride + (p - a.seg[seg].off);
      pv = a.seg[seg].param[so]; m0 = a.seg[seg].m[so]; v0 = a.seg[seg].v[so];
    }
  }
  const float* src = a.partials + (int64_t)f * a.p_pad + p;
  const int64_t cs = (int64_t)a.F * a.p_pad;
  int c = q;
  float v8[8] = {0.f, 0.f, 0.f, 0.f, 0.f, 0.f, 0.f, 0.f};
  const bool pre = p < a.ptot && c + 28 < a.blocks_per_field;
  if (pre) {
#pragma unroll
    for (int j = 0; j < 8; ++j) v8[j] = src[(c + 4 * j) * cs];
  }
  if (adam && seg >= 0 && a.seg[seg].param) {
    const double step = (double)(a.hyper.step_dev ? *a.hyper.step_dev : a.hyper.step);
    co = adam_coef(a.hyper.lr, a.hyper.beta1, a.hyper.beta2, step);
  }
  float s = 0.f;
  if (pre) {
#pragma unroll
    for (int j = 0; j < 8; ++j) s += v8[j];
    c += 32;
  }
  if (p < a.ptot) {
#pragma unroll 1
    for (; c + 28 < a.blocks_per_field; c += 32) {
      float v[8];
#pragma unroll
      for (int j = 0; j < 8; ++j) v[j] = src[(c + 4 * j) * cs];
#pragma unroll
      for (int j = 0; j < 8; ++j) s += v[j];
    }
#pragma unroll 1
    for (; c + 12 < a.blocks_per_field; c += 16) {
      const float v0_ = src[c * cs], v1 = src[(c + 4) * cs], v2 = src[(c + 8) * cs], v3 = src[(c + 12) * cs];
      s += v0_; s += v1; s += v2; s += v3;
    }
    for (; c < a.blocks_per_field; c += 4) s += src[c * cs];
  }
  part[q][l] = s;
  __syncthreads();
  if (q != 0 || p >= a.ptot || seg < 0) return;
  s = ((part[0][l] + part[1][l]) + part[2][l]) + part[3][l];
  const int64_t i = p - a.seg[seg].off;
  if (a.seg[seg].dst) a.seg[seg].dst[(int64_t)f * a.seg[seg].stride + i] = s;
  if (a.seg[seg].param) {
    const float pn = adam_update(pv, m0, v0, s, co, a.hyper.beta1, a.hyper.beta2, a.hyper.eps, a.hyper.wd);
    a.seg[seg].m[so] = m0; a.seg[seg].v[so] = v0;
    a.seg[seg].param[so] = pn;
    if (a.seg[seg].lp) ngm_stp(a.seg[seg].lp, so, pn, a.seg[seg].lp_dt);
  }
}

template <bool COUNTED>
__device__ __forceinline__ void grad_reduce_one(const GradReduceK& a, int f, int64_t p) {
  if (p >= a.ptot) return;
  if constexpr (COUNTED) {
    if (f >= *a.num_active) return;
  }
  int seg = -1;
  for (int k = 0; k < a.nseg; ++k)
    if (p >= a.seg[k].off && p < a.seg[k].off + a.seg[k].size) { seg = k; break; }
  int64_t so = 0;
  float pv = 0.f, m0 = 0.f, v0 = 0.f;
  const bool adam = seg >= 0 && a.seg[seg].param;
  if (adam) {
    const int64_t row = a.hyper.field_index ? a.hyper.field_index[f] : f;
    so = row * a.seg[seg].pstride + (p - a.seg[seg].off);
    pv = a.seg[seg].param[so]; m0 = a.seg[seg].m[so]; v0 = a.seg[seg].v[so];
  }
  const float* src = a.partials + (int64_t)f * a.p_pad + p;
  const int64_t cs = (int64_t)a.F * a.p_pad;
  float q[4] = {0.f, 0.f, 0.f, 0.f};
  if (a.blocks_per_field <= 8) {
    float v[8];
#pragma unroll
    for (int c = 0; c < 8; ++c) v[c] = (c < a.blocks_per_field) ? src[c * cs] : 0.f;
#pragma unroll
    for (int i = 0; i < 4; ++i) {
      float s = 0.f;
      if (i < a.blocks_per_field) s += v[i];
      if (i + 4 < a.blocks_per_field) s += v[i + 4];
      q[i] = s;
    }
  } else {
    for (int c0 = 0; c0 < a.blocks_per_field; c0 += 16) {
      float v[16];
#pragma unroll
      for (int u = 0; u < 16; ++u) v[u] = (c0 + u < a.blocks_per_field) ? src[(int64_t)(c0 + u) * cs] : 0.f;
#pragma unroll
      for (int u = 0; u < 16; ++u)
        if (c0 + u < a.blocks_per_field) q[u & 3] += v[u];
    }
  }
  AdamCoef co = {0.f, 1.f};
  if (adam) {
    const double step = (double)(a.hyper.step_dev ? *a.hyper.step_dev : a.hyper.step);
    co = adam_coef(a.hyper.lr, a.hyper.beta1, a.hyper.beta2, step);
  }
  const float s = ((q[0] + q[1]) + q[2]) + q[3];
  if (seg < 0) return;
  const int64_t i = p - a.seg[seg].off;
  if (a.seg[seg].dst) a.seg[seg].dst[(int64_t)f * a.seg[seg].stride + i] = s;
  if (adam) {
    const float pn = adam_update(pv, m0, v0, s, co, a.hyper.beta1, a.hyper.beta2, a.hyper.eps, a.hyper.wd);
    a.seg[seg].m[so] = m0; a.seg[seg].v[so] = v0;
    a.seg[seg].param[so] = pn;
    if (a.seg[seg].lp) ngm_stp(a.seg[seg].lp, so, pn, a.seg[seg].lp_dt);
  }
}
template <bool COUNTED>
__global__ void __launch_bounds__(256) k_grad_reduce_flat(GradReduceK a) {
  grad_reduce_one<COUNTED>(a, blockIdx.y, (int64_t)blockIdx.x * 256 + threadIdx.x);
}

static int build_grad_reduce(const GradReduceArgs& g, GradReduceK& k) {
  k.F = g.F; k.blocks_per_field = g.blocks_per_field; k.partials = g.partials; k.p_pad = g.p_pad;
  k.num_active = g.num_active;
  int64_t enc_off, w_off[NGM_MAX_LAYERS + 1], b_off[NGM_MAX_LAYERS + 1];
  k.ptot = ngm_param_offsets(&g.fc, &enc_off, w_off, b_off);
  int n = 0;
  if (g.fc.encoding == NGM_ENC_FOURIER) {
    const int64_t sz = (int64_t)(g.fc.raw_coords ? g.fc.dim_enc - 3 : g.fc.dim_enc) * 3;
    k.seg[n++] = GradSeg{enc_off, sz, g.gr.enc_w, g.gr.enc_w_stride, nullptr, nullptr, nullptr, 0, nullptr, 0};
  }
  for (int l = 0; l <= g.fc.num_layers; ++l) {
    const int din = (l == 0) ? g.fc.dim_enc : g.fc.dim_hidden + (g.fc.skip_mode == NGM_SKIP_CONCAT ? g.fc.dim_enc : 0);
    const int dout = (l == g.fc.num_layers) ? g.fc.dim_out : g.fc.dim_hidden;
    k.seg[n++] = GradSeg{w_off[l], (int64_t)din * dout, g.gr.w[l], g.gr.w_stride[l], nullptr, nullptr, nullptr, 0, nullptr, 0};
    k.seg[n++] = GradSeg{b_off[l], (int64_t)dout, g.gr.b[l], g.gr.b_stride[l], nullptr, nullptr, nullptr, 0, nullptr, 0};
  }
  k.nseg = n;
  k.hyper = AdamHyper{nullptr, nullptr, 1, 0.f, 0.f, 0.f, 0.f, 0.f};
  if (g.adam.tensors) {
    if (g.adam.num != n) return NGM_E_INVALID;
    for (int i = 0; i < n; ++i) {
      const ngm_adam_tensor& t = g.adam.tensors[i];
      if (t.numel != k.seg[i].size || !t.param || !t.exp_avg || !t.exp_avg_sq) return NGM_E_INVALID;
      k.seg[i].param = t.param; k.seg[i].m = t.exp_avg; k.seg[i].v = t.exp_avg_sq; k.seg[i].pstride = t.stride;
      k.seg[i].lp = t.param_lp; k.seg[i].lp_dt = t.lp_dtype;
    }
    k.hyper = g.adam.hyper;
  }
  return 0;
}
int ngm_launch_grad_reduce(const GradReduceArgs& g, hipStream_t st) {
  NgmProfScope prof_(NGM_K_GRAD_REDUCE, st);
  GradReduceK k;
  const int rc = build_grad_reduce(g, k);
  if (rc) return rc;
  if (k.blocks_per_field <= 8) {
    dim3 grid((unsigned)((k.ptot + 255) / 256), (unsigned)g.F);
    if (k.num_active) hipLaunchKernelGGL(k_grad_reduce_flat<true>, grid, dim3(256), 0, st, k);
    else hipLaunchKernelGGL(k_grad_reduce_flat<false>, grid, dim3(256), 0, st, k);
    return 0;
  }
  dim3 grid((unsigned)((k.ptot + 63) / 64), (unsigned)g.F);
  if (k.num_active) hipLaunchKernelGGL(k_grad_reduce<true>, grid, dim3(256), 0, st, k);
  else hipLaunchKernelGGL(k_grad_reduce<false>, grid, dim3(256), 0, st, k);
  return 0;
}

template <int MI, int MH, int L>
static int launch_bwd(const FieldBwdArgs& a, int blocks, hipStream_t st) {
#define NGM_LB(NC, EG, HS, CT)                                                                                          \
  do {                                                                                                                  \
    const size_t lds = BwdLds<MI, MH, L, CT>::TOTAL * sizeof(float);                                                    \
    static_assert(BwdLds<MI, MH, L, CT>::TOTAL * sizeof(float) <= NGM_LDS_MAX, "k_field_bwd: LDS over 160 KiB");          \
    (void)hipFuncSetAttribute((const void*)k_field_bwd<MI, MH, L, NC, EG, HS, CT>, hipFuncAttributeMaxDynamicSharedMemorySize, \
                              (int)lds);                                                                                \
    hipLaunchKernelGGL((k_field_bwd<MI, MH, L, NC, EG, HS, CT>), dim3(blocks), dim3(NGM_BLOCK), lds, st, a);            \
  } while (0)
  const bool cat = a.fc.skip_mode == NGM_SKIP_CONCAT;
  if (a.fc.encoding == NGM_ENC_PERMUTO) {
    if constexpr (MI == 1) { if (cat) NGM_LB(false, false, 1, true); else NGM_LB(false, false, 1, false); }
    else return NGM_E_INVALID;
  } else if (a.fc.encoding == NGM_ENC_TRIPLANE) {
    if (!a.tri_acc) return NGM_E_INVALID;
    if (cat) NGM_LB(false, false, 2, true); else NGM_LB(false, false, 2, false);
  } else if (a.fc.encoding == NGM_ENC_FOURIER) { if (cat) NGM_LB(false, true, 0, true); else NGM_LB(false, true, 0, false); }
  else if (a.fc.encoding == NGM_ENC_NERF) { if (cat) NGM_LB(true, false, 0, true); else NGM_LB(true, false, 0, false); }
  else { if (cat) NGM_LB(false, false, 0, true); else NGM_LB(false, false, 0, false); }
#undef NGM_LB
  return 0;
}

__global__ void k_tri_finish(const long long* acc, int64_t numel, float* grad, int64_t gstride) {
  const int f = blockIdx.y;
  for (int64_t i = (int64_t)blockIdx.x * blockDim.x + threadIdx.x; i < numel; i += (int64_t)gridDim.x * blockDim.x)
    grad[(int64_t)f * gstride + i] = (float)((double)acc[(int64_t)f * numel + i] * (1.0 / 1099511627776.0));
}
int ngm_launch_tri_finish(const FieldBwdArgs& a, hipStream_t st) {
  if (!a.tri_acc || !a.planes_grad) return NGM_E_INVALID;
  const int bx = (int)std::min<int64_t>((a.tri_numel + 255) / 256, 1024);
  hipLaunchKernelGGL(k_tri_finish, dim3(bx, a.F), dim3(256), 0, st, a.tri_acc, a.tri_numel, a.planes_grad, a.planes_grad_stride);
// ... 327 lines not shown
```

neural_graph_mapping_amd/csrc/ngm_field_bwd_b3.hip:

```cpp
#include "ngm_bwd_b3.h"

template <bool NEED_COS, bool ENC_GRAD>
__device__ __forceinline__ void recompute_with_encoding(const ngm_u32x4* __restrict__ P, const float* __restrict__ tile,
                                                        const float* __restrict__ pb, const float4 (&encw)[2], int lane,
                                                        f32x16 (&Hc)[2], float (&Eb)[2][2][8], float (&Cb)[2][2][8]) {
  const int hi = lane >> 5;
  const float inv2pi = 0.15915494309189535f;
  const f32x16 zero = {0.f, 0.f, 0.f, 0.f, 0.f, 0.f, 0.f, 0.f, 0.f, 0.f, 0.f, 0.f, 0.f, 0.f, 0.f, 0.f};
  RowRegs R;
  PlaneRegs W[2];
  float4 pq[2][4];
  load_rows(tile, lane, R);
  load_planes(P, 0, lane, W[0]);
  auto ldq = [&](int q) __attribute__((always_inline)) {
#pragma unroll
    for (int j = 0; j < 4; ++j) {
      const int b = q >> 1, e = 4 * (q & 1) + j;
      pq[q & 1][j] = *reinterpret_cast<const float4*>(pb + 4 * (8 * ((8 * b + e) >> 2) + 4 * hi + (e & 3)));
    }
  };
  ldq(0);
  __builtin_amdgcn_sched_barrier(0);
  B3Op A = b3_rows(R.g[0][0], R.g[0][1]);
  __builtin_amdgcn_sched_barrier(0);
// ... 6 lines not shown
      const int j = idx >> 1, m = idx & 1, b = kb >> 1, e = 4 * (kb & 1) + j;
      float4 p = pq[kb & 1][j];
      asm volatile("" : "+v"(p.x));
      const float4 w = encw[m];
      const float arg = fmaf(w.z, p.z, fmaf(w.y, p.y, w.x * p.x));
      const float rev = __builtin_amdgcn_fractf(arg * inv2pi);
      const float sn = __builtin_amdgcn_sinf(rev);
      float v = sn;
      if (NEED_COS) v = (w.w == NGM_FK_COS) ? __builtin_amdgcn_cosf(rev) : sn;
      if (m == 0) v = (w.w == NGM_FK_RAW) ? arg : v;
      asm volatile("" : "+v"(v));
      Eb[b][m][e] = v;
      if (ENC_GRAD) {
        float c = __builtin_amdgcn_cosf(rev);
        asm volatile("" : "+v"(c));
        Cb[b][m][e] = c;
      }
    };
    auto spl = [&](int pr) __attribute__((always_inline)) {
      if (kb < 3) {
        const float4 g = R.g[kb < 3 ? kb + 1 : 3][pr >> 1];
        float x0 = (pr & 1) ? g.z : g.x, x1 = (pr & 1) ? g.w : g.y;
        asm volatile("" : "+v"(x0), "+v"(x1));
        b3_split2(x0, x1, nh[pr], nm[pr], nl[pr]);
        asm volatile("" : "+v"(nh[pr]), "+v"(nm[pr]), "+v"(nl[pr]));
      }
    };
#define NGM_HS_STEP(PA, PW, NT_, Z, WORK)                                                                       \
    asm volatile("" : "+v"(A.PA));             \
    Hc[NT_] = mfma_bf16(A.PA, __builtin_bit_cast(ngm_bf16x8, Wk.PW[NT_]), (Z) ? zero : Hc[NT_]);                \
    WORK;                                                                                                       \
    __builtin_amdgcn_sched_barrier(0);
    NGM_HS_STEP(l, h, 0, kb == 0, enc(0))
    NGM_HS_STEP(l, h, 1, kb == 0, spl(0))
    NGM_HS_STEP(h, l, 0, false, enc(1))
    NGM_HS_STEP(h, l, 1, false, enc(2))
    NGM_HS_STEP(m, m, 0, false, spl(1))
    NGM_HS_STEP(m, m, 1, false, enc(3))
    NGM_HS_STEP(m, h, 0, false, enc(4))
    NGM_HS_STEP(m, h, 1, false, spl(2))
    NGM_HS_STEP(h, m, 0, false, enc(5))
    NGM_HS_STEP(h, m, 1, false, enc(6))
    NGM_HS_STEP(h, h, 0, false, spl(3))
    NGM_HS_STEP(h, h, 1, false, enc(7))
#undef NGM_HS_STEP
    if (kb < 3) {
      A.h = __builtin_bit_cast(ngm_bf16x8, ngm_u32x4{nh[0], nh[1], nh[2], nh[3]});
      A.m = __builtin_bit_cast(ngm_bf16x8, ngm_u32x4{nm[0], nm[1], nm[2], nm[3]});
      A.l = __builtin_bit_cast(ngm_bf16x8, ngm_u32x4{nl[0], nl[1], nl[2], nl[3]});
    }
  }
}

template <int L, bool NEED_COS, bool ENC_GRAD, bool FC = false, bool HS = false, bool COUNTED = false>
__global__ __launch_bounds__(B3B_THREADS) void k_field_bwd_b3(FieldBwdArgs a) {
  extern __shared__ __attribute__((aligned(16))) float sm[];
  using LY = LdsB3b<L, ENC_GRAD, HS>;
#ifdef NGM_PROLOGUE_TIMING
  unsigned long long ptk_[8] = {0, 0, 0, 0, 0, 0, 0, 0};
  const unsigned long long pt0_ = __builtin_readcyclecounter();
#define PTK(i) ptk_[i] = __builtin_readcyclecounter() - pt0_
#else
#define PTK(i)
#endif
  const int f = blockIdx.x % a.F, chunk = blockIdx.x / a.F;
  if constexpr (COUNTED) {
    if (f >= *a.num_active) {
      if constexpr (FC) ngm_counted_idle_bookkeeping(a);
      return;
    }
  }
  const int64_t row = a.pr.field_index ? a.pr.field_index[f] : f;
  const int lane = threadIdx.x & 63, wave = threadIdx.x >> 6;
  const int i = lane & 31, hi = lane >> 5;
  PTK(0);
  ngm_u32x4* planes = reinterpret_cast<ngm_u32x4*>(sm);
  float* wl = sm + LY::PLANES + wave * LY::WAVE_TOTAL;
  float* inb = wl + LY::INB;
  float* pbuf = wl + LY::PB;
  float* obuf = wl + LY::OB;
  float* inb2 = wl + LY::INB2;
  float* pbuf2 = wl + LY::PB2;
  float* obuf2 = wl + LY::OB2;
  const uint32_t wl_lds = __builtin_amdgcn_readfirstlane((uint32_t)(uintptr_t)(__attribute__((address_space(3))) char*)wl);
  float4* accl = reinterpret_cast<float4*>(wl + LY::ACCL) + lane;
  if constexpr (HS) {
#pragma unroll
    for (int q = 0; q < 5; ++q) accl[64 * q] = make_float4(0.f, 0.f, 0.f, 0.f);
  }

  f32x16 acc[L][2][2];
#pragma unroll
  for (int l = 0; l < L; ++l)
#pragma unroll
    for (int mo = 0; mo < 2; ++mo)
#pragma unroll
      for (int mi = 0; mi < 2; ++mi)
#pragma unroll
        for (int r = 0; r < 16; ++r) acc[l][mo][mi][r] = 0.f;
  float dbh[L][2], dwo[2][4], dwf[2][3], dbo[4];
#pragma unroll
  for (int m = 0; m < 2; ++m) {
#pragma unroll
    for (int l = 0; l < L; ++l) dbh[l][m] = 0.f;
#pragma unroll
    for (int c = 0; c < 4; ++c) dwo[m][c] = 0.f;
    dwf[m][0] = dwf[m][1] = dwf[m][2] = 0.f;
  }
  dbo[0] = dbo[1] = dbo[2] = dbo[3] = 0.f;

// ... 9 lines not shown
    tstep = -32;
  } else {
    end = bend;
    first = beg + 32u * (uint32_t)wave;
    ntiles = first < end ? (end - first + TSTRIDE - 1u) / TSTRIDE : 0u;
    tstep = (int32_t)TSTRIDE;
  }
  FieldStreams fs;
  const bool pts = !FC && a.points != nullptr;
  const char* pts_base = pts ? reinterpret_cast<const char*>(a.points + (int64_t)f * a.P * 3) : nullptr;
  __shared__ float s_pose[12];
  if (pts && threadIdx.x == 0) {
    float div, off;
    scale_consts(a.fc.scale_mode, a.fc.field_radius, &div, &off);
    const bool posed = a.pos != nullptr;
    s_pose[0] = posed ? a.pos[3 * f] : 0.f; s_pose[1] = posed ? a.pos[3 * f + 1] : 0.f; s_pose[2] = posed ? a.pos[3 * f + 2] : 0.f;
    s_pose[3] = posed ? a.quat[4 * f] : 1.f; s_pose[4] = posed ? a.quat[4 * f + 1] : 0.f; s_pose[5] = posed ? a.quat[4 * f + 2] : 0.f;
    s_pose[6] = posed ? a.quat[4 * f + 3] : 0.f; s_pose[7] = div; s_pose[8] = off; s_pose[9] = posed ? 1.f : 0.f;
  }
  {
    const int64_t g0 = (int64_t)f * a.P;
    fs.raytab = pts ? nullptr : reinterpret_cast<const char*>(a.raytab) + 32 * (g0 / a.S);
    fs.dout = reinterpret_cast<const char*>(a.d_out + g0);
    fs.tpair = pts ? nullptr : reinterpret_cast<const char*>(a.stashB + (g0 & ~(int64_t)1));
    fs.par = (uint32_t)(g0 & 1);
    fs.gb = (uint32_t)(g0 & 31);
    fs.act[0] = reinterpret_cast<const char*>(a.act + (g0 >> 5) * 2048);
    fs.act[1] = reinterpret_cast<const char*>(a.act + a.act_layer_stride + (g0 >> 5) * 2048);
  }
  const char* seeds = FC ? reinterpret_cast<const char*>(a.rayseed) + 32 * (((int64_t)f * a.P) / a.S) : nullptr;
  const float inv_s = 1.0f / (float)a.S;
  auto issue_small = [&](uint32_t n0, int which) __attribute__((always_inline)) {
    const uint32_t dst = wl_lds + (which ? LY::INB2 : LY::INB) * 4;
    issue_inputs(fs, a.S, n0, end, lane, dst);
    issue_inputs(fs, a.S, n0 + 16, end, lane, dst + 1024);
    uint32_t n = n0 + (uint32_t)(lane & 31);
    if (n >= end) n = end - 1;
    dma16_so_c(seeds, 32u * (uint32_t)fdiv_idx32((int)n, inv_s, a.S) + 16u * (uint32_t)(lane >> 5), dst + 2048);
  };
  if (ntiles) {
    if constexpr (FC) {
      issue_small(first, 0);
      if (ntiles > 1u) issue_small(first - 32u, 1);
    } else if (pts) {
      issue_inputs_pts(fs.dout, pts_base, first, end, lane, wl_lds + LY::INB * 4, wl_lds + LY::INB * 4 + 2048);
      issue_inputs_pts(fs.dout, pts_base, first + 16, end, lane, wl_lds + LY::INB * 4 + 1024, wl_lds + LY::INB * 4 + 2048 + 256);
    } else {
      issue_inputs(fs, a.S, first, end, lane, wl_lds + LY::INB * 4);
      issue_inputs(fs, a.S, first + 16, end, lane, wl_lds + LY::INB * 4 + 1024);
    }
    if constexpr (!HS) issue_tile32(fs.act[L - 1], fs.gb, first, end, lane, wl_lds + LY::HL * 4);
    if (L == 2) issue_tile32(fs.act[0], fs.gb, first, end, lane, wl_lds + LY::H1 * 4);
  }
  float4* cwout = reinterpret_cast<float4*>(sm + LY::CONSTS);
  float4* cenc = cwout + 64;
  __shared__ float s_red[FC ? 16 : 1][17];
  __shared__ float s_sums[NGM_NUM_LOSS_SUMS];
  constexpr int NSETS = (ENC_GRAD ? 1 : 0) + (L == 2 ? 1 : 0) + (HS ? 1 : 0);
  constexpr int NPX = NSETS > 0 ? NSETS * 16 : 1;
  float px_[NPX];
  {
    int off_[NPX];
    int si = 0;
    if (ENC_GRAD) { planes_offsets<false>(a.fc, 0, 0, *reinterpret_cast<int(*)[8]>(off_ + 16 * si)); planes_offsets<false>(a.fc, 0, 1, *reinterpret_cast<int(*)[8]>(off_ + 16 * si + 8)); ++si; }
    if (L == 2) { planes_offsets<false>(a.fc, 1, 0, *reinterpret_cast<int(*)[8]>(off_ + 16 * si)); planes_offsets<false>(a.fc, 1, 1, *reinterpret_cast<int(*)[8]>(off_ + 16 * si + 8)); ++si; }
    if (HS) { planes_offsets<true>(a.fc, 1, 0, *reinterpret_cast<int(*)[8]>(off_ + 16 * si)); planes_offsets<true>(a.fc, 1, 1, *reinterpret_cast<int(*)[8]>(off_ + 16 * si + 8)); ++si; }
    si = 0;
    if (ENC_GRAD) { ngm_ldp_gather<16>(a.pr.w[0], row * a.pr.w_stride[0], *reinterpret_cast<int(*)[16]>(off_ + 16 * si), a.pr.dtype, *reinterpret_cast<float(*)[16]>(px_ + 16 * si)); ++si; }
    if (L == 2) { ngm_ldp_gather<16>(a.pr.w[1], row * a.pr.w_stride[1], *reinterpret_cast<int(*)[16]>(off_ + 16 * si), a.pr.dtype, *reinterpret_cast<float(*)[16]>(px_ + 16 * si)); ++si; }
    if (HS) { ngm_ldp_gather<16>(a.pr.w[1], row * a.pr.w_stride[1], *reinterpret_cast<int(*)[16]>(off_ + 16 * si), a.pr.dtype, *reinterpret_cast<float(*)[16]>(px_ + 16 * si)); ++si; }
  }
  constexpr int PMAX = 20;
  float pv_[FC ? PMAX : 1];
  const int lslot = threadIdx.x & 15, lpart = threadIdx.x >> 4;
  if constexpr (FC) {
    if (a.loss_partials) {
#pragma unroll
      for (int q = 0; q < PMAX; ++q) {
        const int b_ = lpart + 16 * q;
        pv_[q] = (b_ < a.n_partials) ? a.loss_partials[(int64_t)b_ * NGM_NUM_LOSS_SUMS + lslot] : 0.f;
      }
    }
  }
  float4 cw_ = make_float4(0.f, 0.f, 0.f, 0.f), ce_ = make_float4(0.f, 0.f, 0.f, NGM_FK_ZERO);
  float cb_ = 0.f;
  if (threadIdx.x < 64) {
    const int ft = threadIdx.x, H = a.fc.dim_hidden;
    const float* W = a.pr.w[L];
    const int64_t w0 = row * a.pr.w_stride[L];
    if (ft < H) cw_ = make_float4(ngm_ldp(W, w0 + ft, a.pr.dtype), ngm_ldp(W, w0 + H + ft, a.pr.dtype),
                                  ngm_ldp(W, w0 + 2 * H + ft, a.pr.dtype), ngm_ldp(W, w0 + 3 * H + ft, a.pr.dtype));
    ce_ = enc_row_of(a.fc, a.pr, row, ft);
    if constexpr (HS) cb_ = (ft < H) ? ngm_ldp(a.pr.b[1], row * a.pr.b_stride[1] + ft, a.pr.dtype) : 0.f;
  }
  if (threadIdx.x < 64) {
    cwout[threadIdx.x] = cw_;
    cenc[threadIdx.x] = ce_;
    if constexpr (HS) sm[LY::CONSTS + 512 + threadIdx.x] = cb_;
  }
  if constexpr (FC) {
    if (a.loss_partials) {
      float s_ = 0.f;
#pragma unroll
      for (int q = 0; q < PMAX; ++q) s_ += pv_[q];
      for (int b_ = lpart + 16 * PMAX; b_ < a.n_partials; b_ += 16) s_ += a.loss_partials[(int64_t)b_ * NGM_NUM_LOSS_SUMS + lslot];
      s_red[lpart][lslot] = s_;
    }
  }
  {
    int si = 0;
    if (ENC_GRAD) { planes_commit<false>(a.fc, 0, 0, px_ + 16 * si, planes + LY::plane_slot(0) * 3 * PLANE_G); planes_commit<false>(a.fc, 0, 1, px_ + 16 * si + 8, planes + LY::plane_slot(0) * 3 * PLANE_G); ++si; }
    if (L == 2) { planes_commit<false>(a.fc, 1, 0, px_ + 16 * si, planes + LY::plane_slot(1) * 3 * PLANE_G); planes_commit<false>(a.fc, 1, 1, px_ + 16 * si + 8, planes + LY::plane_slot(1) * 3 * PLANE_G); ++si; }
    if (HS) { planes_commit<true>(a.fc, 1, 0, px_ + 16 * si, planes + LY::fwd_slot() * 3 * PLANE_G); planes_commit<true>(a.fc, 1, 1, px_ + 16 * si + 8, planes + LY::fwd_slot() * 3 * PLANE_G); ++si; }
  }
  PTK(1);
  __syncthreads();
  PTK(2);
  __shared__ __attribute__((aligned(16))) float s_k[8];
  if constexpr (FC) {
    if (threadIdx.x < NGM_NUM_LOSS_SUMS) {
      float t = 0.f;
      if (a.loss_partials) {
#pragma unroll
        for (int p = 0; p < 16; ++p) t += s_red[p][threadIdx.x];
      } else t = a.loss_sums[threadIdx.x];
      s_sums[threadIdx.x] = t;
      if (blockIdx.x == 0 && a.sums_out) a.sums_out[threadIdx.x] = t;
    }
    __syncthreads();
    if (threadIdx.x == 0) {
      const float n_m = s_sums[NGM_LS_PHOTO_CNT], n_d = s_sums[NGM_LS_DEPTH_CNT], n_t = s_sums[NGM_LS_TERM_CNT],
                  n_fs = s_sums[NGM_LS_FS_CNT], n_ts = s_sums[NGM_LS_TSDF_CNT];
      float k_photo = n_m > 0 ? a.rc.w_photometric / (3.0f * n_m) : 0.f;
      if (a.rc.photometric_mode == NGM_PHOTO_L2) k_photo = 2.0f * k_photo;
      s_k[0] = k_photo;
      s_k[1] = n_d > 0 ? a.rc.w_depth / n_d : 0.f;
      s_k[2] = n_t > 0 ? a.rc.w_termination * 2.0f / n_t : 0.f;
      s_k[3] = n_fs > 0 ? a.rc.w_freespace * 2.0f / n_fs : 0.f;
      s_k[4] = n_ts > 0 ? a.rc.w_tsdf * 2.0f / n_ts : 0.f;
      if (blockIdx.x == 0) {
        if (a.loss_partials && a.counter) *a.counter += 1ull;
        if (a.loss_out) loss_values_from_sums(a.rc, s_sums, a.loss_out);
      }
    }
    __syncthreads();
  }
  PTK(3);
  float carryQ = 0.f;
  if constexpr (FC) {
    if (ntiles) carryQ = comp_suffix_beyond(a, (int64_t)f * a.P, end, lane, inv_s, s_k[0], s_k[1], s_k[2]);
  }

  int col[4];
#pragma unroll
  for (int j = 0; j < 4; ++j) col[j] = (i >> 2) * 128 + (i & 3) + 4 * ((4 * hi + j) ^ (i >> 2));
#define COL_OFF(m, r) ((m) * 1024 + col[(r) & 3] + 32 * ((r) >> 2))

  PTK(4);
  DMA_WAIT(0);
  PTK(5);
  TICK_DECL;
  TICK(0);
// ... 427 lines not shown
    for (int it = 0; it < NIV; ++it) {
      const int e = it * B3B_THREADS + threadIdx.x;
      const int k = min(e >> 5, NV - 1), ii = e & 31;
      float s0 = 0.f;
#pragma unroll
      for (int w = 0; w < B3B_WAVES; ++w) s0 += stagev[(w * NV + k) * 64 + ii] + stagev[(w * NV + k) * 64 + 32 + ii];
      sv[it] = s0;
    }
#pragma unroll
    for (int it = 0; it < NIV; ++it) {
      const int e = it * B3B_THREADS + threadIdx.x;
      if (e >= NV * 32) break;
      const int k = e >> 5, ii = e & 31;
      const float s0 = sv[it];
      if (k < 2 * L) {
        const int l = k >> 1, ft = 32 * (k & 1) + ii;
        if (ft < H) dst[b_off[l] + ft] = s0;
      } else if (k < 2 * L + 8) {
        const int u = k - 2 * L, ft = 32 * (u >> 2) + ii, c = u & 3;
        if (ft < H) dst[w_off[L] + (int64_t)c * H + ft] = s0;
      } else if (k < 2 * L + 14) {
        const int u = k - 2 * L - 8, ft = 32 * (u / 3) + ii, c = u % 3;
        if (fourier && ft < D && ft >= n_raw) dst[enc_off + (int64_t)(ft - n_raw) * 3 + c] = s0;
      } else if (ii == 0) {
        dst[b_off[L] + (k - 2 * L - 14)] = 0.5f * s0;
      }
    }
  }
  if (!fourier)
    for (int64_t p = enc_off + threadIdx.x; p < w_off[0]; p += B3B_THREADS) dst[p] = 0.f;
  TICK(11);
  TICK_REPORT
#ifdef NGM_PROLOGUE_TIMING
  PTK(7);
  if (a.debug_cycles && blockIdx.x == gridDim.x / 2 && threadIdx.x == 0) {
    for (int k = 0; k < 8; ++k) a.debug_cycles[k] = ptk_[k];
    for (int k = 8; k < 13; ++k) a.debug_cycles[k] = 0;
    a.debug_cycles[12] = ptk_[7];
  }
#endif
#undef PTK
}

template <int L, bool HS>
static int launch_bwd_b3(const FieldBwdArgs& a, int blocks, hipStream_t st) {
#define NGM_LBB3(NC, EG)                                                                                              \
  do {                                                                                                                \
    static_assert(LdsB3b<L, EG, HS>::TOTAL * sizeof(float) <= NGM_LDS_MAX, "k_field_bwd_b3: LDS over 160 KiB");       \
    const size_t lds = (size_t)LdsB3b<L, EG, HS>::TOTAL * sizeof(float);                                              \
    if (a.fused_comp) NGM_LBB3_ONE(NC, EG, true); else NGM_LBB3_ONE(NC, EG, false);                                    \
  } while (0)
#define NGM_LBB3_ONE(NC, EG, FC_)                                                                                     \
  do {                                                                                                                \
    if (a.num_active) {                                                                                               \
      (void)hipFuncSetAttribute((const void*)k_field_bwd_b3<L, NC, EG, FC_, HS, true>, hipFuncAttributeMaxDynamicSharedMemorySize, \
                                (int)lds);                                                                            \
      hipLaunchKernelGGL((k_field_bwd_b3<L, NC, EG, FC_, HS, true>), dim3(blocks), dim3(B3B_THREADS), lds, st, a);    \
    } else {                                                                                                          \
      (void)hipFuncSetAttribute((const void*)k_field_bwd_b3<L, NC, EG, FC_, HS>, hipFuncAttributeMaxDynamicSharedMemorySize, \
                                (int)lds);                                                                            \
      hipLaunchKernelGGL((k_field_bwd_b3<L, NC, EG, FC_, HS>), dim3(blocks), dim3(B3B_THREADS), lds, st, a);          \
    }                                                                                                                 \
  } while (0)
  if (a.fc.encoding == NGM_ENC_FOURIER) NGM_LBB3(false, true);
  else if (a.fc.encoding == NGM_ENC_NERF) NGM_LBB3(true, false);
  else NGM_LBB3(false, false);
#undef NGM_LBB3
#undef NGM_LBB3_ONE
  return 0;
}

bool ngm_field_bwd_b3_takes(const ngm_field_cfg& fc, const BwdProblem& q) {
  const int MI = (fc.dim_enc + 31) / 32, MH = (fc.dim_hidden + 31) / 32, L = fc.num_layers;
  if (q.stash_kind != 1 || (q.points && (q.fused_comp || q.half)) || fc.skip_mode != NGM_SKIP_NO || fc.matmul_mode == NGM_MATMUL_F32 || MI != 2 || MH != 2 || L < 1 || L > 2)
    return false;
  if (fc.encoding != NGM_ENC_FOURIER && fc.encoding != NGM_ENC_NERF && fc.encoding != NGM_ENC_NONE) return false;
  if ((q.P + 64) * 256 >= ((int64_t)1 << 32)) return false;
  if (q.half && L != 2) return false;
  if (q.fused_comp && q.per_block % (B3B_WAVES * 32)) return false;
#ifdef NGM_FAST_BUILD
  if (L != 2) return false;
#endif
  return true;
}
int ngm_launch_field_bwd_b3(const FieldBwdArgs& a, int blocks, hipStream_t st) {
  if (!ngm_field_bwd_b3_takes(a.fc, bwd_problem(a)) || (a.fused_comp && !a.rayseed)) return NGM_E_INVALID;
  NgmProfScope prof_(NGM_K_FIELD_BWD, st);
  if (a.fc.num_layers == 2) return a.act_half ? launch_bwd_b3<2, true>(a, blocks, st) : launch_bwd_b3<2, false>(a, blocks, st);
#ifndef NGM_FAST_BUILD
  if (a.fc.num_layers == 1) return launch_bwd_b3<1, false>(a, blocks, st);
#endif
  return NGM_E_INVALID;
}
```

neural_graph_mapping_amd/csrc/ngm_field_fwd.hip:

```cpp
#include "ngm_field.h"
#include "ngm_launch.h"

#include <algorithm>
#include <cstring>

#define WAVE_SYNC()                                        \
  do {                                                     \
    __builtin_amdgcn_fence(__ATOMIC_RELEASE, "wavefront"); \
    __builtin_amdgcn_wave_barrier();                       \
    __builtin_amdgcn_fence(__ATOMIC_ACQUIRE, "wavefront"); \
  } while (0)

template <int MI, int MH, int L, bool NEED_COS, int HASH, int SKIP, bool B3 = false, int NT = NGM_BLOCK>
__global__ __launch_bounds__(NT) void k_field_points_fwd(PointsFwdArgs a) {
  extern __shared__ __attribute__((aligned(16))) float sm[];
  const int f = blockIdx.x % a.F, chunk = blockIdx.x / a.F;
  const int64_t row = a.pr.field_index ? a.pr.field_index[f] : f;
  {
    FieldStage<MI, MH, L, SKIP == 2> fstage;
    fstage.issue(a.fc, a.pr, row);
    fstage.commit(sm, a.fc);
  }
  __syncthreads();
  ngm_u32x4* const b3w = reinterpret_cast<ngm_u32x4*>(sm + FieldLds<MI, MH, L, SKIP == 2>::TOTAL);
// ... 570 lines not shown
        }
        if (ra[10] != 0.f) {
          const float e = term - ra[11];
          ls[NGM_LS_TERM_SUM] += e * e; cnt_r += 1u << 20;
        }
        if (a.rayseed) {
          const float e0 = ra[0] - tg.x, e1 = ra[1] - tg.y, e2 = ra[2] - tg.z, ed = ra[3] - tg.w, dlt = a.rc.huber_delta;
          const bool l2 = a.rc.photometric_mode == NGM_PHOTO_L2;
          float4 s0 = make_float4(0.f, 0.f, 0.f, 0.f);
          if (m) {
            s0.x = l2 ? e0 : (float)((e0 > 0.f) - (e0 < 0.f)); s0.y = l2 ? e1 : (float)((e1 > 0.f) - (e1 < 0.f));
            s0.z = l2 ? e2 : (float)((e2 > 0.f) - (e2 < 0.f));
            s0.w = (fabsf(ed) < dlt) ? ed : dlt * (float)((ed > 0.f) - (ed < 0.f));
          }
          float4* o = reinterpret_cast<float4*>(a.rayseed + ray * 8);
          o[0] = s0;
          o[1] = make_float4((ra[10] != 0.f) ? term - ra[11] : 0.f, 0.f, 0.f, 0.f);
        }
      }
    }
    WAVE_SYNC();
    PTICK(pc, 10);
    if (rb + BR < r_end) prepare(rb + BR);
  }
  if (a.has_targets && a.loss_partials) {
    __syncthreads();
    float* red = sm + LY::TOTAL;
    ls[NGM_LS_FS_CNT] = (float)(cnt_s & 0xffffu); ls[NGM_LS_TSDF_CNT] = (float)(cnt_s >> 16);
    ls[NGM_LS_PHOTO_CNT] = (float)(cnt_r & 1023u); ls[NGM_LS_DEPTH_CNT] = (float)((cnt_r >> 10) & 1023u);
    ls[NGM_LS_TERM_CNT] = (float)(cnt_r >> 20);
#pragma unroll
    for (int i = 0; i < 11; ++i) {
      const float v = wave_sum(ls[i]);
      if (lane == 0) red[wave * 16 + i] = v;
    }
    __syncthreads();
    if (threadIdx.x < NGM_NUM_LOSS_SUMS) {
      float v = 0.f;
      if (threadIdx.x < 11)
        for (int w = 0; w < nwaves; ++w) v += red[w * 16 + threadIdx.x];
      a.loss_partials[(int64_t)blockIdx.x * NGM_NUM_LOSS_SUMS + threadIdx.x] = v;
    }
  }
#ifdef NGM_PHASE_TIMING
  PTICK(pc, 11);
  if (pc && blockIdx.x == gridDim.x / 2 && threadIdx.x == 0) {
    for (int k = 0; k < 14; ++k) a.debug_cycles[k] = pclk.acc[k];
    a.debug_cycles[14] = __builtin_readcyclecounter() - pclk.start;
    a.debug_cycles[15] = __builtin_amdgcn_s_memrealtime() - pclk.rstart;
  }
#endif
}

static bool fwd_shape_compiled(const ngm_field_cfg& fc) { return ngm_fwd_lds_bytes(fc, false, 0, 0) >= 0; }
int64_t ngm_fwd_lds_bytes(const ngm_field_cfg& fc, bool b3, int waves, int maxs) {
  const FieldShape s = field_shape(&fc);
  const bool cat = fc.skip_mode == NGM_SKIP_CONCAT;
  const int64_t wave_floats = (int64_t)waves * RenderWaveLds::floats(maxs);
#define NGM_FWD_LDS(MI_, MH_, L_)                                                                                              \
  if (s.MI == MI_ && s.MH == MH_ && s.L == L_)                                                                                 \
    return ((cat ? FieldLds<MI_, MH_, L_, true>::TOTAL : FieldLds<MI_, MH_, L_>::TOTAL) + wave_floats) * (int64_t)sizeof(float) + \
           (b3 ? (int64_t)B3Lds<MI_, MH_, L_>::TOTAL * 16 : 0);
  NGM_FWD_SHAPES(NGM_FWD_LDS)
#undef NGM_FWD_LDS
  return -1;
}
bool ngm_points_fwd_takes(const ngm_field_cfg& fc, bool b3) {
  if (!fwd_shape_compiled(fc) || (fc.encoding == NGM_ENC_PERMUTO && fc.dim_enc > 32)) return false;
  return !b3 || ngm_fwd_split_takes(fc);
}
bool ngm_render_fwd_takes(const ngm_field_cfg& fc, bool neus, bool b3) {
  if (!ngm_points_fwd_takes(fc, b3)) return false;
  return !neus || (!b3 && fc.skip_mode == NGM_SKIP_NO && (fc.encoding == NGM_ENC_FOURIER || fc.encoding == NGM_ENC_NONE));
}

template <typename Args>
static int launch_inst(void (*kernel)(Args), const Args& a, const FwdPlan& p, hipStream_t st) {
  (void)hipFuncSetAttribute((const void*)kernel, hipFuncAttributeMaxDynamicSharedMemorySize, (int)p.lds_bytes);
  hipLaunchKernelGGL(kernel, dim3(p.blocks), dim3(p.threads), (size_t)p.lds_bytes, st, a);
  return 0;
}
template <int MI, int MH, int L, bool NC, int HS>
static int launch_points_skips(const PointsFwdArgs& a, const FwdPlan& p, hipStream_t st) {
  return p.skip == 1   ? launch_inst(k_field_points_fwd<MI, MH, L, NC, HS, 1>, a, p, st)
         : p.skip == 2 ? launch_inst(k_field_points_fwd<MI, MH, L, NC, HS, 2>, a, p, st)
                       : launch_inst(k_field_points_fwd<MI, MH, L, NC, HS, 0>, a, p, st);
}
template <int MI, int MH, int L>
static int launch_points(const PointsFwdArgs& a, const FwdPlan& p, hipStream_t st) {
  if (p.matmul == NGM_MATMUL_BF16X3) {
    if constexpr (ngm_fwd_split_shape(MI, MH, L)) {
      if (p.need_cos || p.hash || p.skip || p.threads != 512) return NGM_E_INVALID;
      return launch_inst(k_field_points_fwd<MI, MH, L, false, 0, 0, true, 512>, a, p, st);
    }
    return NGM_E_INVALID;
  }
  if (p.threads != NGM_BLOCK) return NGM_E_INVALID;
  if (p.hash == 1) {
    if constexpr (MI == 1) return launch_points_skips<MI, MH, L, false, 1>(a, p, st);
    return NGM_E_INVALID;
  }
  if (p.hash == 2) return launch_points_skips<MI, MH, L, false, 2>(a, p, st);
  return p.need_cos ? launch_points_skips<MI, MH, L, true, 0>(a, p, st) : launch_points_skips<MI, MH, L, false, 0>(a, p, st);
}
template <int MI, int MH, int L, bool NC, int HS, int SK, bool B3, bool HALF>
static int launch_render_inst(const RenderFwdArgs& a, const FwdPlan& p, hipStream_t st) {
// ... 55 lines not shown
```

neural_graph_mapping_amd/csrc/ngm_launch.h:

```cpp
#pragma once
#include <hip/hip_runtime.h>

#include "../../include/ngm_hip.h"
#include "ngm_adam.h"

#ifndef NGM_BLOCK
#define NGM_WAVE 64
#define NGM_BLOCK 256
#define NGM_WAVES_PER_BLOCK 4
#endif

struct PointsFwdArgs {
  ngm_field_cfg fc;
  ngm_params pr;
  int F;
  int64_t P;
  int64_t per_block;
  const float* points;
  const float* pos;
  const float* quat;
  float* out;
  float* act;
  int64_t act_layer_stride;
};
// ... 45 lines not shown
  const float4* d_out;
  float* partials;
  int64_t p_pad;
  float* lattice_grad;
  int64_t lattice_grad_stride;
  float2* hash_dE;
  float4* hash_xyz;
  float* hash_part;
  int hash_xyz_ready;
  long long* tri_acc;
  int64_t tri_numel;
  float* planes_grad;
  int64_t planes_grad_stride;
  const float* act;
  int64_t act_layer_stride;
  int act_half;
  unsigned long long* debug_cycles;
  GradAdam lattice_adam;
  int fused_comp;
  ngm_render_cfg rc;
  const float* rayseed;
  const float* loss_sums;
  const float* loss_partials; int n_partials;
  float* sums_out; float* loss_out; unsigned long long* counter;
  const int32_t* num_active;
};
struct BwdProblem {
  bool points;
  int64_t P, per_block;
  int stash_kind;
  bool half, fused_comp;
};
static inline BwdProblem bwd_problem(const FieldBwdArgs& a) {
  return {a.points != nullptr, a.P, a.per_block, a.act ? (a.fc.encoding == NGM_ENC_PERMUTO ? 2 : 1) : 0, a.act_half != 0, a.fused_comp != 0};
}
bool ngm_field_bwd_b3_takes(const ngm_field_cfg& fc, const BwdProblem& q);
bool ngm_hash_mlp_bwd_takes(const ngm_field_cfg& fc, const BwdProblem& q);
bool ngm_field_bwd16s_takes(const ngm_field_cfg& fc, const BwdProblem& q);
bool ngm_field_bwd16_takes(const ngm_field_cfg& fc, const BwdProblem& q);
bool ngm_field_bwd_takes(const ngm_field_cfg& fc, const BwdProblem& q);
struct GradReduceArgs;
int ngm_launch_hash_grad(const FieldBwdArgs& a, hipStream_t st, bool* adam_applied = nullptr, const GradReduceArgs* mlp_reduce = nullptr,
                         bool* mlp_reduced = nullptr);

struct GradReduceArgs {
  ngm_field_cfg fc;
  ngm_grads gr;
  int F;
  int blocks_per_field;
  const float* partials;
  int64_t p_pad;
  GradAdam adam;
  const int32_t* num_active = nullptr;
};

struct CompositeArgs {
  ngm_render_cfg rc;
  int64_t N;
  int S;
  const float* colors; const float* geoms; const float* dists; const float* depths; const float* isds;
  const float4* out4; const float* pcam; float* rgbd;
  const int* pair_field; const float* pair_w; const float4* pair_out; int pair_K; float outside_value; const float* ray_dir;
  float* C; float* D; float* Cv; float* Dv; float* term; float* weights;
  const float* dC; const float* dD; const float* dterm;
  float* d_colors; float* d_geoms; float* d_isds;
};

struct StashBwdArgs {
  ngm_render_cfg rc;
  int F, R, S;
  float4* stashA;
  const float2* stashB;
  const float* raytab;
  int seed_mode;
  ngm_targets tg;
  ngm_prediction pred;
  const float* loss_sums;
  const float* d_rgbds;
  const float* d_term;
  const float* d_geom_samples;
  const float* d_cvars;
  const float* d_dvars;
  float* loss_out;
  const float* neus_sd; int64_t neus_sd_stride; const int64_t* field_index;
  float4* d_out;
  float* d_isd_rays;
  const float* loss_partials;
  int n_partials;
  float* sums_out;
  unsigned long long* counter;
  float4* xyz_out;
  const int32_t* num_active;
};

#ifdef NGM_FAST_BUILD
#define NGM_FWD_SHAPES(X) X(2, 2, 2)
#else
#define NGM_FWD_SHAPES(X) X(2, 2, 2) X(2, 2, 1) X(1, 1, 1) X(1, 1, 2) X(2, 2, 3)
#endif
#define NGM_LDS_MAX (160 * 1024)
constexpr bool ngm_fwd_split_shape(int MI, int MH, int L) { return MI == 2 && MH == 2 && L <= 2; }
static inline bool ngm_fwd_split_takes(const ngm_field_cfg& fc) {
  return ngm_fwd_split_shape((fc.dim_enc + 31) / 32, (fc.dim_hidden + 31) / 32, fc.num_layers) && fc.skip_mode == NGM_SKIP_NO &&
         (fc.encoding == NGM_ENC_FOURIER || fc.encoding == NGM_ENC_NONE);
}
enum { NGM_FWD_RENDER = 0, NGM_FWD_POINTS = 1, NGM_FWD_KNN = 2 };
struct FwdPlan {
  int status = NGM_OK; const char* why = nullptr;
  int surface = NGM_FWD_RENDER;
  int MI = 0, MH = 0, L = 0;
  int matmul = -1;
  bool need_cos = false;
  int hash = 0, skip = 0;
  bool neus = false, one_tile = false, counted = false;
  int waves = 0, threads = 0;
  int rays_per_block = 0, maxs = 0;
  int64_t per_block = 0;
  int blocks = 0;
  int64_t lds_bytes = 0;
};
bool ngm_render_fwd_takes(const ngm_field_cfg& fc, bool neus, bool b3);
bool ngm_points_fwd_takes(const ngm_field_cfg& fc, bool b3);
bool ngm_knn_eval_takes(const ngm_field_cfg& fc, bool b3);
int64_t ngm_fwd_lds_bytes(const ngm_field_cfg& fc, bool b3, int waves, int maxs);
int ngm_launch_points_fwd(const PointsFwdArgs& a, const FwdPlan& p, hipStream_t st);
int64_t ngm_encode_bwd_fourier_scratch(int F, int64_t P);
int ngm_launch_encode_bwd_fourier(const ngm_field_cfg& fc, const ngm_params& pr, int F, int64_t P, const float* points,
                                  const float* pos, const float* quat, const float* d_enc, float* grad, int64_t grad_stride,
                                  float* scratch, hipStream_t st);
int ngm_launch_encode_bwd_prep_hash(const ngm_field_cfg& fc, const ngm_params& pr, int F, int64_t P, const float* points,
                                    const float* pos, const float* quat, const float* d_enc, float2* dE, float4* xyz,
                                    hipStream_t st);
int ngm_launch_encode_points(const ngm_field_cfg& fc, const ngm_params& pr, int F, int64_t P, const float* points, const float* pos,
                             const float* quat, float* out, hipStream_t st);
int ngm_launch_render_fwd(const RenderFwdArgs& a, const FwdPlan& p, hipStream_t st);
int ngm_launch_field_bwd(const FieldBwdArgs& a, int blocks, hipStream_t st);
int ngm_launch_tri_finish(const FieldBwdArgs& a, hipStream_t st);
int ngm_launch_field_bwd_b3(const FieldBwdArgs& a, int blocks, hipStream_t st);
int ngm_launch_hash_mlp_bwd(const FieldBwdArgs& a, int blocks, hipStream_t st);
int ngm_launch_field_bwd16s(const FieldBwdArgs& a, int blocks, hipStream_t st);
int ngm_launch_field_bwd16(const FieldBwdArgs& a, int blocks, hipStream_t st);
int ngm_launch_grad_reduce(const GradReduceArgs& a, hipStream_t st);
int ngm_launch_composite_fwd(const CompositeArgs& a, hipStream_t st);
int ngm_launch_composite_bwd(const CompositeArgs& a, hipStream_t st);
int ngm_launch_stash_bwd(const StashBwdArgs& a, hipStream_t st);
int ngm_launch_loss_exchange(const ngm_peer_exchange& px, float* sums, hipStream_t st);
double ngm_peer_set_timeout_impl(double seconds);
int ngm_peer_alloc_impl(int64_t bytes, void** out);

int ngm_launch_target_visibility(const ngm_keyframes& kf, int F, const float* field_pos, int num_offsets, const float* offsets,
                                 float radius, uint8_t* kf_mask, float* bbox, hipStream_t st);
int ngm_launch_target_sv_intersect(int F, int64_t N, const float* pos_c, const float* points, float radius, uint8_t* hit, hipStream_t st);
int ngm_launch_target_sv_rays(int F, int R, const float* pos_c, float radius, const int64_t* pts_ijs, const int64_t* segments,
                              const float* image, int height, int width, float fx, float fy, float cx, float cy, const ngm_target_out& o,
                              hipStream_t st);
int ngm_launch_target_rays(const ngm_keyframes& kf, int F, int R, const float* field_pos, float radius, const float* bbox,
                           const int64_t* frame_cids, const float* u_xy, const ngm_target_out& o, hipStream_t st);
int64_t ngm_target_sample_mv_bytes(int num_frames, int num_current, int num_fields, int capacity);
int ngm_launch_target_sample_mv(const ngm_keyframes& kf, const ngm_target_sample& s, const ngm_target_live* live ,
                                const ngm_target_out& o, void* workspace, hipStream_t st,
                                const int32_t* num_fields_dev = nullptr );
int64_t ngm_target_observed_fields_bytes(int height, int width);
int ngm_launch_target_observed_fields(const ngm_observed_fields& a, void* workspace, hipStream_t st,
                                      const int32_t* num_fields_dev = nullptr);
int ngm_launch_fields_append(const ngm_fields_append_args& a, hipStream_t st);
int ngm_launch_field_counts_add(const int64_t* field_ids, const int32_t* count, int rows, int num_fields, int64_t* training_iterations,
                                hipStream_t st);

__host__ __device__ static inline int64_t ngm_param_offsets(const ngm_field_cfg* fc, int64_t* enc_off, int64_t* w_off, int64_t* b_off) {
  int64_t o = 0;
  *enc_off = 0;
  if (fc->encoding == NGM_ENC_FOURIER) o += (int64_t)(fc->raw_coords ? fc->dim_enc - 3 : fc->dim_enc) * 3;
  for (int l = 0; l <= fc->num_layers; ++l) {
    const int din = (l == 0) ? fc->dim_enc : fc->dim_hidden + (fc->skip_mode == NGM_SKIP_CONCAT ? fc->dim_enc : 0);
    const int dout = (l == fc->num_layers) ? fc->dim_out : fc->dim_hidden;
    w_off[l] = o; o += (int64_t)din * dout;
    b_off[l] = o; o += dout;
  }
// ... 9 lines not shown
```

neural_graph_mapping_amd/ops.py:

```python
import ctypes as C
from typing import Dict, List, Optional, Tuple

import torch

from . import _capi as K


NS = "ngm355"


_BLOBS: Dict[bytes, torch.Tensor] = {}
_STRUCTS: Dict[int, object] = {}


def cfg_blob(struct) -> torch.Tensor:
    raw = bytes(struct)
    t = _BLOBS.get(raw)
    if t is None:
        if len(_BLOBS) > 4096:
            _BLOBS.clear(); _STRUCTS.clear()
        t = _BLOBS[raw] = torch.frombuffer(bytearray(raw), dtype=torch.uint8)
        _STRUCTS[id(t)] = type(struct).from_buffer_copy(raw)
    return t

# ... 749 lines not shown

@_op("adam_sparse_", mutates_args=("param", "exp_avg", "exp_avg_sq"))
def _adam_sparse_op(param: torch.Tensor, exp_avg: torch.Tensor, exp_avg_sq: torch.Tensor, grad: torch.Tensor,
                    field_index: torch.Tensor, step: int, lr: float, beta1: float, beta2: float, eps: float,
                    weight_decay: float) -> None:
    F = grad.shape[0]
    numel = grad[0].numel()
    K.check(K.lib().ngm_adam_sparse(_ptr(param), _ptr(exp_avg), _ptr(exp_avg_sq), param.stride(0), _ptr(grad),
                                    grad.stride(0), _ptr(field_index), F, numel, int(step), lr, beta1, beta2, eps,
                                    weight_decay, _stream()), "ngm_adam_sparse")


def adam_sparse_(param, exp_avg, exp_avg_sq, grad, field_index, step, lr=1e-3, betas=(0.9, 0.999), eps=1e-15,
                 weight_decay=1e-5):
    _require_gpu(param, exp_avg, exp_avg_sq, grad, field_index)
    torch.ops.ngm355.adam_sparse_(param, exp_avg, exp_avg_sq, grad, field_index, int(step), float(lr), float(betas[0]),
                                  float(betas[1]), float(eps), float(weight_decay))


def _adam_tensor(p, st, g, lp=None):
    t = K.AdamTensor(p.data_ptr(), st["exp_avg"].data_ptr(), st["exp_avg_sq"].data_ptr(), g.data_ptr(), p.stride(0), g.stride(0),
                     g[0].numel())
    if lp is not None and lp.dtype != torch.float32:
        if lp.shape != p.shape or lp.stride(0) != p.stride(0):
            raise ValueError("reduced-precision copy must mirror the master tensor's layout")
        t.param_lp, t.lp_dtype = lp.data_ptr(), _TORCH_DT[lp.dtype]
    return t


def adam_tensor_arrays(fc, params, state, grads, lp=None):
    names = [n for n in K.param_names(fc) if n not in K.NO_GRAD_PARAMS]
    mlp = [n for n in names if n not in ("_encoding.lattice_values", "_encoding.plane_coef")]
    arr = (K.AdamTensor * len(mlp))()
    for i, n in enumerate(mlp):
        arr[i] = _adam_tensor(params[n], state[n], grads[n], None if lp is None else lp[n])
    lat = None
    if "_encoding.lattice_values" in names:
        n = "_encoding.lattice_values"
        lat = (K.AdamTensor * 1)(_adam_tensor(params[n], state[n], grads[n], None if lp is None else lp[n]))
    return arr, len(mlp), lat


def adam_sparse_multi_(fc, params, state, grads, field_index, step, step_dev=None, lr=1e-3, betas=(0.9, 0.999),
                       eps=1e-15, weight_decay=1e-5, advance=False, philox_offset_dev=None, lp=None):
    names = [n for n in K.param_names(fc) if n not in K.NO_GRAD_PARAMS]
    arr = (K.AdamTensor * len(names))()
    for i, n in enumerate(names):
        arr[i] = _adam_tensor(params[n], state[n], grads[n], None if lp is None else lp[n])
    K.check(K.lib().ngm_adam_sparse_multi(arr, len(names), _ptr(field_index), grads[names[0]].shape[0], int(step),
                                          _ptr(step_dev), lr, betas[0], betas[1], eps, weight_decay,
                                          int(bool(advance and step_dev is not None)),
                                          _ptr(philox_offset_dev) if advance else None, _stream()),
            "ngm_adam_sparse_multi")


def keyframes_struct(c2ws, rgbd_store, frame_to_store, fx, fy, cx, cy) -> K.Keyframes:
    _require_gpu(c2ws, rgbd_store, frame_to_store)
    assert c2ws.is_contiguous() and rgbd_store.is_contiguous() and frame_to_store.dtype == torch.int64
    kf = K.Keyframes()
    kf.num_frames, kf.height, kf.width = c2ws.shape[0], rgbd_store.shape[1], rgbd_store.shape[2]
    kf.c2ws = C.cast(c2ws.data_ptr(), K.f32p)
    kf.rgbd = C.cast(rgbd_store.data_ptr(), K.f32p)
    kf.frame_to_store = frame_to_store.data_ptr()
    kf.fx, kf.fy, kf.cx, kf.cy = float(fx), float(fy), float(cx), float(cy)
    return kf


def target_visibility(kf: K.Keyframes, field_pos, offsets, radius):
    field_pos, offsets = _f32c(field_pos), _f32c(offsets)
    F, Nc = field_pos.shape[0], kf.num_frames
    mask = torch.empty(F, Nc, dtype=torch.uint8, device=field_pos.device)
    bbox = torch.empty(F, Nc, 4, device=field_pos.device)
    K.check(K.lib().ngm_target_visibility(C.byref(kf), F, _ptr(field_pos), offsets.shape[0], _ptr(offsets), float(radius),
                                          _ptr(mask), _ptr(bbox), _stream()), "ngm_target_visibility")
    return mask.bool(), bbox


def target_rays(kf: K.Keyframes, field_pos, radius, bbox, frame_cids, u_xy):
    field_pos, bbox, u_xy = _f32c(field_pos), _f32c(bbox), _f32c(u_xy)
    frame_cids = frame_cids.contiguous()
    F, R = frame_cids.shape
    dev = field_pos.device
    o = dict(ijs=torch.empty(F, R, 2, dtype=torch.int64, device=dev), c2ws=torch.empty(F, R, 4, 4, device=dev),
             near=torch.empty(F, R, device=dev), far=torch.empty(F, R, device=dev), gt=torch.empty(F, R, device=dev),
             rgbds=torch.empty(F, R, 4, device=dev), rgb_mask=torch.empty(F, R, dtype=torch.uint8, device=dev),
             depth_mask=torch.empty(F, R, dtype=torch.uint8, device=dev), term_probs=torch.empty(F, R, device=dev),
             term_mask=torch.empty(F, R, dtype=torch.uint8, device=dev))
    out = K.TargetOut()
    out.ijs = o["ijs"].data_ptr()
    for k in ("c2ws", "near", "far", "gt", "rgbds", "term_probs"):
        setattr(out, k, C.cast(o[k].data_ptr(), K.f32p))
    for k in ("rgb_mask", "depth_mask", "term_mask"):
        setattr(out, k, o[k].data_ptr())
    K.check(K.lib().ngm_target_rays(C.byref(kf), F, R, _ptr(field_pos), float(radius), _ptr(bbox), _ptr(frame_cids),
                                    _ptr(u_xy), C.byref(out), _stream()), "ngm_target_rays")
    for k in ("rgb_mask", "depth_mask", "term_mask"):
        o[k] = o[k].bool()
    return o


def target_sv_intersect(pos_c, points, radius):
    pos_c, points = _f32c(pos_c), _f32c(points)
    F, N = pos_c.shape[0], points.shape[0]
    hit = torch.empty(F, N, dtype=torch.uint8, device=points.device)
    K.check(K.lib().ngm_target_sv_intersect(F, N, _ptr(pos_c), _ptr(points), float(radius), _ptr(hit), _stream()),
            "ngm_target_sv_intersect")
# ... 395 lines not shown
```

neural_graph_mapping_amd/renderer.py:

```python
import ctypes as C
from collections import namedtuple
import warnings
from typing import Dict, Optional

import torch

from . import _capi as K
from . import ops
from .models import NeuralFieldSet

Target = namedtuple("Target", ["ijs", "c2ws", "near_distances", "far_distances", "gt_distances", "field_ids", "rgbds",
                               "rgb_mask", "depth_mask", "term_probs", "term_mask"])
Prediction = namedtuple("Prediction", ["rgbds", "color_vars", "depth_vars", "term_probs", "freespace_geometry",
                                       "tsdf_residuals"])


class DeviceTarget(namedtuple("DeviceTarget", Target._fields + ("count", "subset_observed", "subset_random", "offsets",
                                                                "frame_cids", "u_xy", "world_size"))):
    __slots__ = ()

    @staticmethod
    def from_sampler(o: dict, world_size: int) -> "DeviceTarget":
        rows = (o["ijs"], o["c2ws"], o["near"], o["far"], o["gt"], o["field_ids"], o["rgbds"], o["rgb_mask"], o["depth_mask"],
                o["term_probs"], o["term_mask"], o["count"], o["subset_observed"], o["subset_random"], o["offsets"],
# ... 68 lines not shown
def check_config(config: dict) -> None:
    missing = [k for k in REQUIRED_CONFIG_KEYS if k not in config]
    if missing:
        raise KeyError(f"config lacks {missing}: NeuralGraphMap._read_config reads them unconditionally (rm.py:116-220)")
    if config["photometric_loss"] not in K.PHOTO:
        raise NotImplementedError(f"photometric_loss {config['photometric_loss']!r} is not built (built: {sorted(K.PHOTO)}, "
                                  "losses.py:26-36)")
    if config["depth_loss"] not in K.DEPTH:
        raise NotImplementedError(f"depth_loss {config['depth_loss']!r} is not built (built: {sorted(K.DEPTH)}, losses.py:60-75)")
    if config["geometry_mode"] not in K.GEO:
        raise ValueError(f"Unsupported geometry mode {config['geometry_mode']}")


def make_render_cfg(camera: Camera, config: dict, guided: bool = True) -> K.RenderCfg:
    check_config(config)
    fx, fy, cx, cy, _ = camera.get_pinhole_camera_parameters(0.0)
    tau = config.get("truncation_distance", 0.1)
    rho = config.get("range_depth_guided") or tau
    return K.render_cfg(
        geometry_mode=config["geometry_mode"], num_samples_coarse=config["num_samples_coarse"],
        num_samples_guided=config["num_samples_depth_guided"] if guided else 0,
        geometry_factor=config.get("geometry_factor", 1.0), color_factor=config.get("color_factor", 1.0),
        truncation_distance=tau, range_depth_guided=rho, fx=fx, fy=fy, cx=cx, cy=cy,
        w_termination=config["termination_weight"], w_photometric=config["photometric_weight"],
        w_depth=config["depth_weight"], w_freespace=config["freespace_weight"],
        w_tsdf=config.get("tsdf_weight", 0.0), photometric_loss=config["photometric_loss"], depth_loss=config["depth_loss"])


class NeuralGraphRenderer:

    def __init__(self, model: NeuralFieldSet, camera: Camera, config: dict, device="cuda"):
        self._model, self._camera, self._config, self._device = model, camera, dict(config), device
        self._field_radius = config.get("field_radius", model._field_radius)
        self._fc = model.field_cfg()
        mm = config.get("mlp_matmul", "auto")
        self._fc.matmul_mode = K.MATMUL[mm]
        self._fc.activation_stash = K.STASH[config.get("activation_stash") or "full"]
        self._fc.hash_grad_atomics = K.HASH_ATOMICS[config.get("hash_grad_atomics") or "exact"]
        fc = self._fc
        compiled = (fc.encoding in (K.ENC["fourier"], K.ENC["none"]) and fc.skip_mode == K.SKIP["no"] and 1 <= fc.num_layers <= 2
                    and 32 < fc.dim_enc <= 64 and 32 < fc.dim_hidden <= 64)
        self.mlp_matmul = ("bf16x3" if compiled else "f32") if mm == "auto" else mm
        self._rc_train = make_render_cfg(camera, config, guided=True)
        self._rc_cache = {}
        self._mode = "train"
        self._global_map_dict = None
        self._learning_rate = config.get("learning_rate", 1e-3)
        self._adam_eps = config.get("adam_eps", 1e-15)
        self._adam_weight_decay = config.get("adam_weight_decay", 0.0)
        self._optim_state: Optional[Dict[str, Dict[str, torch.Tensor]]] = None
        self._step = 0
        self._step_dev = None
        self._ws_cache = {}
        self.process_group = None
        self.eval_fused = True
        self.eval_fallbacks = []
        self.last_eval_path = None
        self.peer_exchange = None
        self.peer_check_interval = 256
        self._peer_calls = 0
        self.field_draw_generator = None
        self._target_iter_dev = None
        self._warned_counted_fallback = False
        self.track_training_iterations = False
        self._observe_frame_dev = None
        self.last_observed = None
        self._reserved: Optional[dict] = None
        self._reserve_epoch = 0

    def last_matmul(self, kernel: str = "forward") -> Optional[str]:
        v = K.lib().ngm_debug_last_matmul({"forward": 0, "points": 1, "knn": 2}[kernel])
        return {K.MATMUL["f32"]: "f32", K.MATMUL["bf16x3"]: "bf16x3"}.get(v)

    def set_field_poses(self, positions: torch.Tensor, orientations: torch.Tensor):
        rs = self._reserved
        if rs is not None:
            num = self._global_map_dict["num"]
            if positions.shape[0] != num or orientations.shape[0] != num:
                raise ValueError(f"set_field_poses: {positions.shape[0]} / {orientations.shape[0]} poses for {num} fields (reserved "
                                 "rows: add fields with add_fields(num_new, positions=, orientations=))")
            rs["positions"][:num].copy_(positions)
            rs["orientations"][:num].copy_(orientations)
            return
        old = self._global_map_dict
        self._global_map_dict = {"positions": positions, "orientations": orientations, "num": positions.shape[0]}
        if old is not None and "training_iterations" in old:
            self._global_map_dict["training_iterations"] = old["training_iterations"]

    def _training_iterations(self) -> torch.Tensor:
        md = self._global_map_dict
        if self._reserved is not None:
            return self._reserved["training_iterations"]
        ti, num = md.get("training_iterations"), md["num"]
        if ti is None or ti.shape[0] < num:
            if torch.cuda.is_current_stream_capturing():
                raise RuntimeError("training_iterations must exist before a graph capture (capture_iteration / "
                                   "capture_training create it when track_training_iterations is set)")
            new = torch.zeros(num, dtype=torch.int64, device=self._device)
            if ti is not None:
                new[:ti.shape[0]] = ti
            md["training_iterations"] = ti = new
        return ti

    def _count_training_iteration(self, field_ids: torch.Tensor, count: Optional[torch.Tensor]) -> None:
        if self.track_training_iterations and field_ids.shape[0] > 0:
            fids = field_ids if field_ids.dtype == torch.int64 else field_ids.long()
# ... 22 lines not shown
        pdev = next(iter(caps.values())).device
        pos, quat = torch.zeros(max_fields, 3, device=pdev), torch.zeros(max_fields, 4, device=pdev)
        quat[:, 0] = 1.0
        ti = torch.zeros(max_fields, dtype=torch.int64, device=pdev)
        if md is not None:
            pos[:num], quat[:num] = md["positions"], md["orientations"]
            if md.get("training_iterations") is not None:
                ti[:num] = md["training_iterations"][:num]
        nfd = torch.zeros(1, dtype=torch.int32, device=pdev)
        nfd.fill_(num)
        self._reserve_epoch += 1
        self._reserved = dict(max=max_fields, epoch=self._reserve_epoch, state=state, positions=pos, orientations=quat,
                              training_iterations=ti, num_fields_dev=nfd)
        self._set_num(num)

    def _set_num(self, num: int) -> None:
        rs = self._reserved
        self._optim_state = {k: {n: t[:num] for n, t in st.items()} for k, st in rs["state"].items()}
        self._global_map_dict = {"positions": rs["positions"][:num], "orientations": rs["orientations"][:num], "num": num,
                                 "training_iterations": rs["training_iterations"]}

    def _append_reserved(self, num_new: int, positions, orientations) -> None:
        rs, m = self._reserved, self._model
        first = m._check_room(num_new)
        pdev = rs["positions"].device
        if positions is None:
            positions = torch.zeros(num_new, 3, device=pdev)
        if orientations is None:
            orientations = torch.zeros(num_new, 4, device=pdev)
            orientations[:, 0] = 1.0
        if tuple(positions.shape) != (num_new, 3) or tuple(orientations.shape) != (num_new, 4):
            raise ValueError(f"add_fields({num_new}): positions must be ({num_new}, 3) and orientations ({num_new}, 4), got "
                             f"{tuple(positions.shape)} and {tuple(orientations.shape)}")
        positions = positions.to(device=pdev, dtype=torch.float32).contiguous()
        orientations = orientations.to(device=pdev, dtype=torch.float32).contiguous()
        if not rs["positions"].is_cuda:
            m.add_fields(num_new)
            for st in rs["state"].values():
                st["exp_avg"][first:first + num_new] = 0.0
                st["exp_avg_sq"][first:first + num_new] = 0.0
            rs["positions"][first:first + num_new] = positions
            rs["orientations"][first:first + num_new] = orientations
            rs["training_iterations"][first:first + num_new] = 0
            rs["num_fields_dev"].fill_(first + num_new)
        else:
            mr = m._reserved
            proto = m._prototype_field.state_dict()
            tensors = [dict(param=mr["params"][k], exp_avg=rs["state"][k]["exp_avg"], exp_avg_sq=rs["state"][k]["exp_avg_sq"],
                            prototype=proto[k].detach().contiguous(), lp=None if mr["lp"] is None else mr["lp"].get(k))
                       for k in mr["params"]]
            ops.fields_append(tensors, positions, orientations, rs["positions"], rs["orientations"], rs["training_iterations"],
                              rs["num_fields_dev"], first)
            m._set_num(first + num_new)
        self._set_num(first + num_new)

    def add_fields(self, num_new: int, positions: Optional[torch.Tensor] = None, orientations: Optional[torch.Tensor] = None):
        if self._reserved is not None:
            return self._append_reserved(int(num_new), positions, orientations)
        if positions is not None or orientations is not None:
            raise ValueError("add_fields(positions=, orientations=) needs reserve_fields; without a reservation the poses "
                             "are the caller's tensors (set_field_poses)")
        self._model.add_fields(num_new)
        allp = self._model.all_fields_params
        new_state = {}
        for k, v in allp.items():
            m, s = torch.zeros_like(v), torch.zeros_like(v)
            if self._optim_state is not None:
                m[:-num_new] = self._optim_state[k]["exp_avg"]
                s[:-num_new] = self._optim_state[k]["exp_avg_sq"]
            new_state[k] = {"exp_avg": m, "exp_avg_sq": s}
        self._optim_state = new_state

    def save_model(self, path: str) -> None:
        self.check_exchange()
        md, allp = self._global_map_dict, self._model.all_fields_params
        if self._reserved is not None:
            num = md["num"]
            md = {k: (v[:num].clone() if isinstance(v, torch.Tensor) else v) for k, v in md.items()}
            allp = {k: v.clone() for k, v in allp.items()}
        torch.save({"map_dict": md, "all_fields_params": allp, "state_dict": self._model.state_dict()}, path)

    def load_model(self, path: str) -> None:
        self._reserved = self._model._reserved = None
        ck = torch.load(path, map_location=self._device)
        self._model.load_state_dict(ck["state_dict"])
        self._model.all_fields_params = {k: v.to(self._device) for k, v in ck["all_fields_params"].items()}
        self._global_map_dict = ck["map_dict"]
        self._model.refresh_lp()
        self._optim_state = {k: {"exp_avg": torch.zeros_like(v), "exp_avg_sq": torch.zeros_like(v)}
                             for k, v in self._model.all_fields_params.items()}

    @torch.no_grad()
    def evaluate_points(self, points: torch.Tensor, block_size: Optional[int] = None) -> torch.Tensor:
        num = self._global_map_dict["num"]
        pos = self._global_map_dict["positions"][:num]
        quat = self._global_map_dict["orientations"][:num]
        params = self._model.kernel_params()
        m = self._model
        lead = points.shape[:-1]
        pts = points.reshape(-1, 3)
        block = int(block_size or self._config.get("block_size", 3000000))
        outs = [ops.field_eval_knn(self._fc, params, pts[s:s + block], pos, quat, m._num_knn, m._distance_factor,
                                   m._outside_value) for s in range(0, pts.shape[0], block)]
        return torch.cat(outs).reshape(*lead, 4)

    def extract_mesh(self, mesh_file_path=None, resolution: Optional[float] = None, threshold: Optional[float] = None,
# ... 184 lines not shown
        pc, pw, dists = ops.sample_rays_world(rc, ijs, c2ws, near, far, gt_sampler, u_coarse, u_guided, seed,
                                              near_const=self._config.get("near_distance", 0.0),
                                              far_const=self._config.get("far_distance", 8.0))
        F, R, S = dists.shape
        out = ops.field_eval(self._fc, {k: v for k, v in params.items() if k != "_neus_sd"}, pw.reshape(F, R * S, 3),
                             pos, quat).view(F, R, S, 4)
        colors = rc.color_factor * out[..., :3]
        geoms = out[..., 3]
        depths = -pc[..., 2]
        if overwrite_behind and near is not None and not bool((near >= 0).all()):
            const = -100.0 if rc.geometry_mode in (K.GEO["occupancy"], K.GEO["density"]) else 1.0
            geoms = torch.where(pc[..., 2] > 0, torch.full_like(geoms, const), geoms)
        isds = None
        if rc.geometry_mode == K.GEO["neus"]:
            isds = 1.0 / torch.abs(params["_neus_sd"].view(-1, 1, 1))
        C, D, Cv, Dv, term, _ = ops.quadrature(rc, colors, geoms, dists, depths, isds)
        fs = ts = None
        tau = rc.truncation_distance
        if gt is not None:
            g = gt[..., None]
            if rc.w_freespace != 0.0:
                fs = geoms[dists < (g - tau) * (g != 0.0)] * tau
            if rc.w_tsdf != 0.0:
                deltas = g - dists
                m = (deltas.abs() < tau) & (g != 0.0)
                ts = geoms[m] * tau - deltas[m]
        return Prediction(torch.cat([C, D[..., None]], -1), Cv, Dv, term, fs, ts)

    def optimization_iteration_staged(self, target: Target, u_coarse=None, u_guided=None, seed=0, update=True) -> dict:
        fids = target.field_ids
        pred = self.render_ijs(target.ijs, target.c2ws, field_ids=fids, use_vmap=True, near_distances=target.near_distances,
                               far_distances=target.far_distances, gt_distances=target.gt_distances,
                               u_coarse=u_coarse, u_guided=u_guided, seed=seed)
        loss = self.compute_losses(target, pred)
        params = self._model.vmap_fields_params
        names = [n for n, v in params.items() if v.requires_grad and n not in K.NO_GRAD_PARAMS]
        grads = torch.autograd.grad(loss["combined"], [params[n] for n in names], allow_unused=True)
        gd = {n: (g if g is not None else torch.zeros_like(params[n])) for n, g in zip(names, grads)}
        out = {k: v.detach() for k, v in loss.items()}
        out["prediction"] = pred
        if not update:
            out["grads"] = gd
            return out
        self._step += 1
        with torch.no_grad():
            for n in names:
                allp = self._model.all_fields_params[n]
                st = self._optim_state[n]
                ops.adam_sparse_(allp, st["exp_avg"], st["exp_avg_sq"], gd[n].contiguous(), fids, self._step,
                                 lr=self._learning_rate, eps=self._adam_eps, weight_decay=self._adam_weight_decay)
        if self._step_dev is not None:
            self._step_dev.fill_(self._step)
        self._model.refresh_lp()
        self._count_training_iteration(fids, None)
        return out

    def compute_losses(self, target: Target, prediction: Prediction) -> dict:
        rc = self._rc_train
        pk = "photometric_" + self._config["photometric_loss"]
        m = target.depth_mask & (prediction.term_probs > rc.term_threshold)
        loss = {}
        tm = target.term_mask
        loss["termination"] = ((prediction.term_probs[tm] - target.term_probs[tm]) ** 2).mean()
        diff = target.rgbds[m][:, :3] - prediction.rgbds[m][:, :3]
        dk = "depth_" + self._config["depth_loss"]
        p_d, t_d = prediction.rgbds[m][:, 3], target.rgbds[m][:, 3]
        if rc.photometric_mode == K.PHOTO["gaussian_nll"]:
            cv = prediction.color_vars[m]
            nlls = 0.5 * diff ** 2 / cv + torch.log(torch.sqrt(cv))
            loss[pk] = diff.abs().mean() if nlls.mean() > 2 else nlls.mean()
        else:
            loss[pk] = diff.abs().mean() if rc.photometric_mode == K.PHOTO["l1"] else (diff ** 2).mean()
        if rc.depth_mode == K.DEPTH["gaussian_nll"]:
            dv = prediction.depth_vars[m] + 1e-15
            loss[dk] = (0.5 * (p_d - t_d) ** 2 / dv + torch.log(torch.sqrt(dv))).mean()
        elif rc.depth_mode == K.DEPTH["laplacian_nll"]:
            dv = prediction.depth_vars[m]
            loss[dk] = ((t_d - p_d).abs() / torch.sqrt(0.5 * dv + 1e-6) + 0.5 * torch.log(2 * dv + 1e-6)).mean()
        else:
            loss[dk] = torch.nn.functional.huber_loss(p_d, t_d, delta=rc.huber_delta)
        total = (rc.w_termination * loss["termination"] + rc.w_photometric * loss[pk]
                 + rc.w_depth * loss[dk])
        if prediction.freespace_geometry is not None:
            loss["freespace"] = ((prediction.freespace_geometry - rc.truncation_distance) ** 2).mean()
            total = total + rc.w_freespace * loss["freespace"]
        if prediction.tsdf_residuals is not None:
            loss["tsdf"] = (prediction.tsdf_residuals ** 2).mean()
            total = total + rc.w_tsdf * loss["tsdf"]
        loss["combined"] = total
        return loss

    @torch.no_grad()
    def sample_target_mv(self, current_field_ids, c_c2w, nc_rgbd, frame_cid_to_ncid, num_train_fields, num_rays_per_field,
                         num_fields=None, camera: Optional[Camera] = None, draws: Optional[dict] = None,
                         field_draw: str = "reference", world_size: int = 1) -> Target:
        if field_draw not in ("reference", "balanced_by_owner"):
            raise NotImplementedError(f"field_draw={field_draw!r}: 'reference' or 'balanced_by_owner'")
        cam = camera or self._camera
        dev = self._device
        radius = self._field_radius + 0.0
        num_fields = self._global_map_dict["num"] if num_fields is None else num_fields
        d = draws or {}
        cur = current_field_ids.to(dev)
        if field_draw == "balanced_by_owner" and world_size > 1 and not draws:
            from . import distributed as D
            if self.field_draw_generator is None:
# ... 152 lines not shown
        S, near_c, far_c = self._mode_sampling()
        rc = self._rc_for(cam, False)
        w = cam.width
        dev = self._device
        idx = torch.arange(begin, end, device=dev)
        ijs = torch.stack((idx // w, idx % w), -1)
        num = self._global_map_dict["num"]
        pos = self._global_map_dict["positions"][:num]
        quat = self._global_map_dict["orientations"][:num]
        if params is None:
            params = self._model.kernel_params()
        params = {k: v for k, v in params.items() if k != "_neus_sd"}
        m = self._model
        block = int(cfg.get("pixel_block_size", 8192))
        if self.eval_fused:
            rb = int(cfg.get("eval_ray_block") or max(block, 32768))
            pred = self._fused_eval(lambda ray_block: ops.render_eval_knn(
                self._fc, rc, params, ijs, c2w, pos, quat, m._num_knn, m._distance_factor, m._outside_value,
                u=None if u is None else u[begin:end], seed=seed + begin, near_const=near_c, far_const=far_c,
                ray_block=ray_block), rb, block)
            if pred is not None:
                return pred[0], pred[2]
        else:
            self.last_eval_path = "staged"
        rgbds, dvars = [], []
        for s0 in range(0, ijs.shape[0], block):
            ij = ijs[s0:s0 + block]
            ub = None if u is None else u[begin + s0:begin + s0 + block][None]
            pc, pw, dist = ops.sample_rays_world(rc, ij, c2w, None, None, None, ub, None, seed + begin + s0,
                                                 near_const=near_c, far_const=far_c)
            out4 = ops.field_eval_knn(self._fc, params, pw.view(-1, 3), pos, quat, m._num_knn, m._distance_factor,
                                      m._outside_value)
            rgbd, _, dv, _ = ops.composite_packed(rc, out4, dist.view(-1, S), pc.view(-1, S, 3))
            rgbds.append(rgbd)
            dvars.append(dv)
        if not rgbds:
            return torch.empty(0, 4, device=dev), torch.empty(0, device=dev)
        return torch.cat(rgbds), torch.cat(dvars)

    @torch.no_grad()
    def render_image(self, c2w: torch.Tensor, camera: Optional[Camera] = None, u: Optional[torch.Tensor] = None,
                     seed: int = 0):
        cam = camera or self._camera
        rgbd, dv = self.render_pixels(c2w, 0, cam.height * cam.width, camera=cam, u=u, seed=seed)
        return rgbd.reshape(cam.height, cam.width, 4), dv.reshape(cam.height, cam.width)

    @staticmethod
    def psnr(prediction: torch.Tensor, target: torch.Tensor, crop: int = 0) -> float:
        if crop > 0:
            prediction, target = prediction[crop:-crop, crop:-crop], target[crop:-crop, crop:-crop]
        mse = ((prediction.clamp(0.0, 1.0) - target.clamp(0.0, 1.0)) ** 2).mean()
        return float(10.0 * torch.log10(1.0 / mse))

    def _workspace(self, F, R):
        key = (F, R)
        if key not in self._ws_cache:
            wsb = K.lib().ngm_render_workspace(C.byref(self._fc), C.byref(self._rc_train), F, R, 1)
            if wsb < 0:
                K.check(int(wsb), "ngm_render_workspace")
            dev = self._device
            self._ws_cache[key] = dict(
                ws=torch.empty(wsb, device=dev, dtype=torch.uint8), wsb=wsb,
                rgbds=torch.empty(F, R, 4, device=dev), color_vars=torch.empty(F, R, 3, device=dev),
                depth_vars=torch.empty(F, R, device=dev), term_probs=torch.empty(F, R, device=dev),
                sums=torch.zeros(K.NGM_NUM_LOSS_SUMS, device=dev), loss=torch.zeros(8, device=dev),
                philox=torch.zeros(1, device=dev, dtype=torch.int64))
        return self._ws_cache[key]

    def optimization_iteration(self, target: Target, u_coarse=None, u_guided=None, seed=0, update=True) -> dict:
        if isinstance(target, DeviceTarget):
            return self._counted_iteration(target, u_coarse, u_guided, seed, update)
        if self._rc_train.geometry_mode == K.GEO["neus"] and not self._neus_fused():
            return self.optimization_iteration_staged(target, u_coarse, u_guided, seed, update)
        return self._fused_iteration(target, u_coarse, u_guided, seed, update)

    def _fused_iteration(self, target: Target, u_coarse, u_guided, seed, update, count=None) -> dict:
        if target.ijs.shape[0] == 0:
            return self._idle_iteration(update)
        ctx = self._iteration_forward(target, u_coarse, u_guided, seed, advance=update, count=count)
        if self.process_group is not None:
            self._exchange(ctx["w"]["sums"])
        return self._iteration_backward(ctx, update)

    def counted_step_unsupported(self) -> Optional[str]:
        rc, fc = self._rc_train, self._fc
        if rc.geometry_mode == K.GEO["neus"]:
            return "geometry mode 'neus'"
        if fc.encoding == K.ENC["triplane"]:
            return "the triplane encoding"
        if rc.photometric_mode == K.PHOTO["gaussian_nll"] or rc.depth_mode != K.DEPTH["huber"]:
            return "the *_nll loss modes"
        return None

    def _counted_iteration(self, target: "DeviceTarget", u_coarse=None, u_guided=None, seed=0, update=True) -> dict:
        why = self.counted_step_unsupported()
        if why is not None:
            if torch.cuda.is_current_stream_capturing():
                raise RuntimeError(f"optimization_iteration(DeviceTarget): {why} is outside the counted step and the "
                                   "fallback (DeviceTarget.materialize()) synchronises: it cannot be captured")
            if not self._warned_counted_fallback:
                self._warned_counted_fallback = True
                warnings.warn(f"optimization_iteration(DeviceTarget): {why} is outside the counted step; falling back to "
                              "DeviceTarget.materialize(), which synchronises with the host every iteration",
                              RuntimeWarning, stacklevel=3)
            return self.optimization_iteration(target.materialize(), u_coarse, u_guided, seed, update)
        return self._fused_iteration(target, u_coarse, u_guided, seed, update, count=target.count)

    def check_exchange(self):
        if self.peer_exchange is not None:
            self.peer_exchange.check()

    def _count_exchange(self):
        self._peer_calls += 1
        if self.peer_exchange is not None and self.peer_check_interval and self._peer_calls % self.peer_check_interval == 0:
            if not torch.cuda.is_current_stream_capturing():
                self.peer_exchange.check()

    def _exchange(self, sums: torch.Tensor):
        if self.peer_exchange is not None:
            self.peer_exchange.allreduce(sums)
            self._count_exchange()
        else:
            torch.distributed.all_reduce(sums, group=self.process_group)

    def _neus_fused(self) -> bool:
        fc = self._fc
        return fc.encoding in (K.ENC["fourier"], K.ENC["none"]) and fc.skip_mode == K.SKIP["no"]

    def _idle_iteration(self, update=True) -> dict:
        from . import distributed as D
        sums = torch.zeros(16, device=self._device)
        if self.process_group is not None:
            self._exchange(sums)
        rc = self._rc_train
        loss = D.loss_values_from_sums(sums, rc.w_termination, rc.w_photometric, rc.w_depth, rc.w_freespace, rc.w_tsdf,
                                       self._config["photometric_loss"], self._config["depth_loss"])
        if update:
            self._step += 1
            if self._step_dev is None:
                self._step_dev = torch.full((1,), self._step, device=self._device, dtype=torch.int64)
            else:
                self._step_dev += 1
        else:
            loss["grads"] = {}
        loss["prediction"] = None
        return loss

    def _iteration_forward(self, target: Target, u_coarse=None, u_guided=None, seed=0, advance=True, count=None) -> dict:
        L = K.lib()
        fc, rc = self._fc, self._rc_train
        fids = target.field_ids
        F, R = target.ijs.shape[0], target.ijs.shape[1]
        names = K.param_names(fc)
        allp = {n: self._model.all_fields_params[n] for n in names}
        kp = self._model.kernel_params()
        lp = None if self._model.lp_fields_params is None else {n: kp[n] for n in names}
        kernel_p = {n: kp[n] for n in names}
        neus = rc.geometry_mode == K.GEO["neus"]
        if neus:
            kernel_p["_neus_sd"] = self._model.all_fields_params["_neus_sd"]
        ps = ops.params_struct(fc, kernel_p, fids)
        w = self._workspace(F, R)
        keep = []
        if self._step_dev is None:
            self._step_dev = torch.full((1,), self._step, device=self._device, dtype=torch.int64)
        rays = ops.make_rays(rc, target.ijs, target.c2ws, target.near_distances, target.far_distances,
                             target.gt_distances, self._global_map_dict["positions"],
                             self._global_map_dict["orientations"], u_coarse, u_guided, seed, keep=keep,
                             pose_index=fids, philox_offset_dev=self._step_dev, philox_autoinc=advance)
        dm = target.depth_mask.view(torch.uint8) if target.depth_mask.dtype == torch.bool else target.depth_mask
        tm = target.term_mask
        if tm is not None and tm.dtype == torch.bool:
            tm = tm.view(torch.uint8)
        rgbds_t = ops._f32c(target.rgbds)
        tg = K.Targets(ops._ptr(rgbds_t), dm.data_ptr(), ops._ptr(tm), ops._ptr(target.term_probs))
        pred = K.Prediction(w["rgbds"].data_ptr(), w["color_vars"].data_ptr(), w["depth_vars"].data_ptr(),
                            w["term_probs"].data_ptr())
        st = ops._stream()
        defer = self.process_group is None
        fn, args = "ngm_render_fwd", [C.byref(fc), C.byref(rc), C.byref(ps), C.byref(rays), C.byref(tg), C.byref(pred),
                                      None if defer else w["sums"].data_ptr(), w["ws"].data_ptr(), w["wsb"], st]
        if count is not None:
            if count.dtype != torch.int32 or count.numel() != 1 or not count.is_cuda:
                raise TypeError("count must be a device int32 tensor of one element")
            fn += "_counted"
            args.append(count.data_ptr())
        K.check(getattr(L, fn)(*args), fn)
        return dict(fc=fc, rc=rc, ps=ps, rays=rays, tg=tg, pred=pred, w=w, F=F, fids=fids, allp=allp, lp=lp, defer=defer,
                    neus=neus, count=count, keep=(keep, dm, tm, rgbds_t, target))

    def _iteration_backward(self, ctx: dict, update=True) -> dict:
        L = K.lib()
        fc, rc, ps, rays, tg, pred, w, F, fids, allp = (ctx[k] for k in ("fc", "rc", "ps", "rays", "tg", "pred", "w", "F",
                                                                         "fids", "allp"))
        st = ops._stream()
        if "grads" not in w:
            w["grads"], w["gs"], w["gflat"] = ops.alloc_grads(fc, F, self._device)
        grads, gs = w["grads"], w["gs"]
        if ctx.get("neus") and "_neus_sd" not in grads:
            grads["_neus_sd"] = torch.zeros(F, device=self._device)
            gs.neus_sd = grads["_neus_sd"].data_ptr()
        count = ctx.get("count")
        fn, args = "ngm_render_bwd", [C.byref(fc), C.byref(rc), C.byref(ps), C.byref(rays), C.byref(tg), C.byref(pred),
                                      None if ctx.get("defer") else w["sums"].data_ptr(), C.byref(gs)]
        if update:
            arr, n_mlp, lat = ops.adam_tensor_arrays(fc, allp, self._optim_state, grads, ctx.get("lp"))
            fn += "_adam"
            args += [arr, n_mlp, lat, ops._ptr(fids), int(self._step) + 1, ops._ptr(self._step_dev), self._learning_rate, 0.9, 0.999,
                     self._adam_eps, self._adam_weight_decay]
        args += [w["loss"].data_ptr(), w["ws"].data_ptr(), w["wsb"], st]
        if count is not None:
            fn += "_counted"
            args.append(count.data_ptr())
        K.check(getattr(L, fn)(*args), fn)
        if update:
            self._step += 1
        if update and count is None:
            if fc.encoding == K.ENC["triplane"]:
                gp = grads["_encoding.plane_coef"]
                self._adam_one_tensor("_encoding.plane_coef", gp, allp["_encoding.plane_coef"].stride(0), gp.stride(0),
                                      gp[0].numel(), fids, F, st)
            if ctx.get("neus"):
                self._adam_one_tensor("_neus_sd", grads["_neus_sd"], 1, 1, 1, fids, F, st)
        if update:
            self._count_training_iteration(fids, count)
        lv = w["loss"]
        loss = {"combined": lv[0], "termination": lv[1], "photometric_" + self._config["photometric_loss"]: lv[2],
                "depth_" + self._config["depth_loss"]: lv[3],
                "freespace": lv[4], "tsdf": lv[5]}
        if not update:
            loss["grads"] = grads
        loss["prediction"] = Prediction(w["rgbds"], w["color_vars"], w["depth_vars"], w["term_probs"], None, None)
        return loss

    def _adam_one_tensor(self, name, grad, stride, grad_stride, numel, fids, F, st) -> None:
        p, stt = self._model.all_fields_params[name], self._optim_state[name]
        one = (K.AdamTensor * 1)(K.AdamTensor(p.data_ptr(), stt["exp_avg"].data_ptr(), stt["exp_avg_sq"].data_ptr(),
                                              grad.data_ptr(), stride, grad_stride, numel))
        K.check(K.lib().ngm_adam_sparse_multi(one, 1, ops._ptr(fids), F, int(self._step), ops._ptr(self._step_dev),
                                              self._learning_rate, 0.9, 0.999, self._adam_eps, self._adam_weight_decay, 0,
                                              None, st), "ngm_adam_sparse_multi")

    def capture_iteration(self, target: Target, seed=0, u_coarse=None, u_guided=None):
        if self._rc_train.geometry_mode == K.GEO["neus"] and not self._neus_fused():
            raise NotImplementedError("capture_iteration: the staged (neus) iteration allocates under autograd; call "
                                      "optimization_iteration directly")
        count = None
        if isinstance(target, DeviceTarget):
            why = self.counted_step_unsupported()
            if why is not None:
                raise RuntimeError(f"capture_iteration(DeviceTarget): {why} is outside the counted step; capture a "
                                   "materialised Target instead")
            count = target.count
        if self.track_training_iterations:
            self._training_iterations()
        s = torch.cuda.Stream()
        s.wait_stream(torch.cuda.current_stream())
        with torch.cuda.stream(s):
            for _ in range(2):
                self.optimization_iteration(target, u_coarse, u_guided, seed=seed)
        torch.cuda.current_stream().wait_stream(s)

        def whole():
            return self.optimization_iteration(target, u_coarse, u_guided, seed=seed)
        return self._capture("capture_iteration", whole,
                             lambda: self._iteration_forward(target, u_coarse, u_guided, seed, advance=True, count=count))

    def _capture(self, caller: str, whole, forward):
        step0 = self._step
        if self.process_group is None or self.peer_exchange is not None:
            graph = torch.cuda.CUDAGraph()
            with torch.cuda.graph(graph):
                out = whole()
            self._step = step0

            def replay():
                graph.replay()
                self._step += 1
                if self.peer_exchange is not None:
                    self._count_exchange()
                return out
            replay.graph = graph
            return replay
        try:
            g1, g2 = torch.cuda.CUDAGraph(), torch.cuda.CUDAGraph()
            with torch.cuda.graph(g1, capture_error_mode="thread_local"):
                ctx = forward()
            with torch.cuda.graph(g2, pool=g1.pool(), capture_error_mode="thread_local"):
                out = self._iteration_backward(ctx, True)
        except RuntimeError as err:
            self._step = step0
            torch.cuda.synchronize()
            warnings.warn(f"{caller}: graph capture refused ({err}); falling back to plain launches", RuntimeWarning, stacklevel=3)
            whole.graph, whole.capture_error = None, str(err)
            return whole
        self._step = step0
        sums, group = ctx["w"]["sums"], self.process_group

        def replay2():
            g1.replay()
            torch.distributed.all_reduce(sums, group=group)
            g2.replay()
            self._step += 1
            return out
        replay2.graph = (g1, g2)
        return replay2

    def capture_training(self, current_field_ids, c_c2w, nc_rgbd, frame_cid_to_ncid, num_train_fields, num_rays_per_field,
                         seed=0, camera: Optional[Camera] = None, world_size: int = 1, rank: int = 0, *,
                         current_count: Optional[torch.Tensor] = None, num_frames: Optional[torch.Tensor] = None):
        why = self.counted_step_unsupported()
        if why is not None:
            raise RuntimeError(f"capture_training: {why} is outside the counted step (optimization_iteration would fall "
                               "back to DeviceTarget.materialize(), which synchronises)")
        if (current_count is None) != (num_frames is None):
            raise ValueError("capture_training: current_count and num_frames go together (both device tensors, or neither)")
        dev = torch.device(self._device)
        named = dict(current_field_ids=current_field_ids, c_c2w=c_c2w, nc_rgbd=nc_rgbd, frame_cid_to_ncid=frame_cid_to_ncid)
        if current_count is not None:
            named.update(current_count=current_count, num_frames=num_frames)
        for n, t in named.items():
            if not t.is_cuda or not t.is_contiguous():
                raise ValueError(f"capture_training: {n} must be a contiguous device tensor (it is read in place at every replay)")
        for n in ("current_field_ids", "frame_cid_to_ncid"):
            if named[n].dtype != torch.int64:
                raise TypeError(f"capture_training: {n} must be int64")
        num_fields = self._global_map_dict["num"]
        grow = self._reserved is not None and current_count is not None

        def watched():
            ts = dict(named, positions=self._global_map_dict["positions"], orientations=self._global_map_dict["orientations"])
            ts.update({"param " + n: v for n, v in self._model.all_fields_params.items()})
            if self.track_training_iterations:
                ts["training_iterations"] = self._training_iterations()
            if not grow:
                return {n: (t.data_ptr(), tuple(t.shape)) for n, t in ts.items()}
            seen = {n: (t.data_ptr(), tuple(t.shape) if n in named else tuple(t.shape[1:])) for n, t in ts.items()}
            rs, mr = self._reserved, self._model._reserved
            if rs is None or mr is None:
                return dict(seen, reservation=None)
            caps = {"reserved " + n: t for n, t in mr["params"].items()}
            caps.update({"reserved lp " + n: t for n, t in (mr["lp"] or {}).items()})
            for n, st in rs["state"].items():
                caps["reserved exp_avg " + n], caps["reserved exp_avg_sq " + n] = st["exp_avg"], st["exp_avg_sq"]
                seen["exp_avg " + n] = (self._optim_state[n]["exp_avg"].data_ptr(),)
                seen["exp_avg_sq " + n] = (self._optim_state[n]["exp_avg_sq"].data_ptr(),)
            for n in ("positions", "orientations", "training_iterations", "num_fields_dev"):
                caps["reserved " + n] = rs[n]
            seen.update({n: (t.data_ptr(), tuple(t.shape)) for n, t in caps.items()})
            seen["reservation"] = (rs["max"], rs["epoch"])
            return seen
        for n in ("positions", "orientations"):
# ... 49 lines not shown
```

Measured before the change: 2.230 billion ray-samples/s.

## Keep a persistent bf16x3 split-plane image of hidden weights, refreshed by fused Adam

```diff
diff --git a/include/ngm_hip.h b/include/ngm_hip.h
--- a/include/ngm_hip.h
+++ b/include/ngm_hip.h
@@ -87,6 +87,8 @@
   int64_t planes_stride;
   const float* neus_sd;
   int64_t neus_sd_stride;
+  void* b3_image;
+  int64_t b3_image_stride;
 } ngm_params;
 
 typedef struct ngm_grads {
@@ -254,6 +256,10 @@
                         int32_t num_mlp_tensors, const ngm_adam_tensor* lattice_tensor, const int64_t* field_index,
                         int64_t step, int64_t* step_dev, float lr, float beta1, float beta2, float eps,
                         float weight_decay, float* loss_values, void* workspace, int64_t workspace_bytes, void* stream);
+int64_t ngm_b3_image_bytes(const ngm_field_cfg* fcfg);
+int ngm_b3_image_takes(const ngm_field_cfg* fcfg, const ngm_render_cfg* rcfg, int32_t F, int32_t R);
+int ngm_b3_image_build(const ngm_field_cfg* fcfg, const ngm_params* params, int32_t num_rows, void* stream);
+
 int ngm_render_fwd_counted(const ngm_field_cfg* fcfg, const ngm_render_cfg* rcfg,
                            const ngm_params* params, const ngm_rays* rays, const ngm_targets* targets,
                            const ngm_prediction* pred, float* loss_sums, void* workspace,
diff --git a/neural_graph_mapping_amd/_capi.py b/neural_graph_mapping_amd/_capi.py
--- a/neural_graph_mapping_amd/_capi.py
+++ b/neural_graph_mapping_amd/_capi.py
@@ -36,7 +36,8 @@
                 ("b", LArr), ("b_stride", SArr), ("field_index", C.c_void_p),
                 ("lattice", f32p), ("lattice_stride", C.c_int64), ("shift", f32p), ("shift_stride", C.c_int64),
                 ("dtype", C.c_int32), ("reserved_", C.c_int32), ("planes", f32p), ("planes_stride", C.c_int64),
-                ("neus_sd", f32p), ("neus_sd_stride", C.c_int64)]
+                ("neus_sd", f32p), ("neus_sd_stride", C.c_int64),
+                ("b3_image", C.c_void_p), ("b3_image_stride", C.c_int64)]
 
 
 class Grads(C.Structure):
@@ -228,6 +229,12 @@
     L.ngm_composite_bwd.argtypes = [P(RenderCfg), i64, i32] + [vp] * 11 + [vp]
     L.ngm_render_workspace.argtypes = [P(FieldCfg), P(RenderCfg), i32, i32, i32]
     L.ngm_render_workspace.restype = i64
+    L.ngm_b3_image_bytes.argtypes = [P(FieldCfg)]
+    L.ngm_b3_image_bytes.restype = i64
+    L.ngm_b3_image_takes.argtypes = [P(FieldCfg), P(RenderCfg), i32, i32]
+    L.ngm_b3_image_takes.restype = C.c_int
+    L.ngm_b3_image_build.argtypes = [P(FieldCfg), P(Params), i32, vp]
+    L.ngm_b3_image_build.restype = C.c_int
     L.ngm_render_fwd.argtypes = [P(FieldCfg), P(RenderCfg), P(Params), P(Rays), P(Targets),
                                  P(Prediction), vp, vp, i64, vp]
     L.ngm_render_bwd.argtypes = [P(FieldCfg), P(RenderCfg), P(Params), P(Rays), P(Targets),
@@ -328,6 +335,7 @@
             "ngm_field_eval_fwd", "ngm_encode_fwd", "ngm_encode_bwd", "ngm_encode_bwd_workspace", "ngm_field_eval_bwd", "ngm_field_eval_bwd_workspace",
             "ngm_field_eval_stash_bytes", "ngm_field_eval_fwd_train", "ngm_field_eval_bwd_stash",
             "ngm_composite_fwd", "ngm_composite_bwd", "ngm_render_workspace", "ngm_render_fwd",
+            "ngm_b3_image_bytes", "ngm_b3_image_takes", "ngm_b3_image_build",
             "ngm_render_bwd", "ngm_render_bwd_adam", "ngm_render_bwd_seeded", "ngm_render_bwd_seeded_vars", "ngm_render_read_samples", "ngm_adam_sparse",
             "ngm_field_eval_knn", "ngm_field_eval_knn_workspace", "ngm_render_eval_knn", "ngm_render_eval_knn_workspace", "ngm_adam_sparse_multi", "ngm_step_advance", "ngm_profile_enable", "ngm_profile_reset", "ngm_profile_read",
             "ngm_debug_phase_cycles", "ngm_debug_fwd_phase_cycles", "ngm_debug_last_bwd_variant", "ngm_debug_last_matmul", "ngm_debug_last_fwd_one_tile", "ngm_debug_last_comp_fused", "ngm_debug_disable_fused_comp", "ngm_debug_stash_mode", "ngm_debug_last_stash_mode", "ngm_debug_plan_bwd", "ngm_debug_plan_fwd", "ngm_target_visibility", "ngm_target_rays", "ngm_target_sv_intersect", "ngm_target_sv_rays",
diff --git a/neural_graph_mapping_amd/csrc/ngm_api.hip b/neural_graph_mapping_amd/csrc/ngm_api.hip
--- a/neural_graph_mapping_amd/csrc/ngm_api.hip
+++ b/neural_graph_mapping_amd/csrc/ngm_api.hip
@@ -362,6 +362,13 @@
   for (int l = 0; l <= fc->num_layers; ++l)
     if (!pr->w[l] || !pr->b[l]) return fail(NGM_E_INVALID, "missing layer weight/bias pointer");
   if (pr->dtype != NGM_DT_F32 && pr->dtype != NGM_DT_BF16 && pr->dtype != NGM_DT_F16) return fail(NGM_E_INVALID, "params.dtype");
+  if (pr->b3_image) {
+    const int64_t need = ngm_b3_image_row_bytes(*fc);
+    if (!need) return fail(NGM_E_INVALID, "params.b3_image: the split path is not compiled for this configuration (ngm_b3_image_bytes is 0), so it takes no plane image");
+    if (reinterpret_cast<uintptr_t>(pr->b3_image) & 15) return fail(NGM_E_INVALID, "params.b3_image: not 16-byte aligned");
+    if (pr->b3_image_stride < need || (pr->b3_image_stride & 15))
+      return fail(NGM_E_INVALID, "params.b3_image_stride: rows are ngm_b3_image_bytes(cfg) bytes at least, a multiple of 16");
+  }
   return NGM_OK;
 }
 
@@ -919,6 +926,32 @@
   return p;
 }
 
+int64_t ngm_b3_image_bytes(const ngm_field_cfg* fcfg) {
+  const int e = check_field_cfg(fcfg);
+  return e ? e : ngm_b3_image_row_bytes(*fcfg);
+}
+int ngm_b3_image_takes(const ngm_field_cfg* fcfg, const ngm_render_cfg* rcfg, int32_t F, int32_t R) {
+  const int e = check_field_cfg(fcfg);
+  if (e) return e;
+  if (!rcfg || F < 1 || R < 1) return fail(NGM_E_INVALID, "ngm_b3_image_takes: bad argument");
+  if (!ngm_b3_image_row_bytes(*fcfg)) return 0;
+  for (int guided = 0; guided < 2; ++guided) {
+    const RenderPlan p = plan_render(fcfg, rcfg, F, R, guided != 0, true);
+    if (p.fwd.status || p.bwd.status || p.fwd.matmul != NGM_MATMUL_BF16X3 || p.bwd.variant != 3 || p.bwd.half) return 0;
+  }
+  return 1;
+}
+int ngm_b3_image_build(const ngm_field_cfg* fcfg, const ngm_params* params, int32_t num_rows, void* stream) {
+  int e = check_field_cfg(fcfg);
+  if (e) return e;
+  e = check_params(fcfg, params);
+  if (e) return e;
+  if (!params->b3_image) return fail(NGM_E_INVALID, "ngm_b3_image_build: params.b3_image is NULL");
+  if (num_rows < 1) return fail(NGM_E_INVALID, "ngm_b3_image_build: num_rows < 1");
+  if (ngm_launch_b3_image_build(*fcfg, *params, num_rows, (hipStream_t)stream)) return fail(NGM_E_INVALID, "ngm_b3_image_build: no image for this configuration");
+  return check_launch("ngm_b3_image_build");
+}
+
 int64_t ngm_render_workspace(const ngm_field_cfg* fcfg, const ngm_render_cfg* rcfg, int32_t F, int32_t R, int32_t train) {
   const int e = check_field_cfg(fcfg);
   if (e) return e;
@@ -987,6 +1020,8 @@
   if (save && (!pred->rgbds || !pred->term_probs)) return fail(NGM_E_INVALID, "render_fwd(save): pred.rgbds/term_probs required");
   const RenderPlan p = plan_render(fcfg, rcfg, rays->F, rays->R, rays->gt != nullptr, save, BwdAsk(), num_active != nullptr);
   if (p.fwd.status) return fail(p.fwd.status, p.fwd.why);
+  if (params->b3_image && p.fwd.matmul != NGM_MATMUL_BF16X3)
+    return fail(NGM_E_INVALID, "render_fwd: params.b3_image given, but the plan of this batch shape is exact-fp32 MFMA (ngm_b3_image_takes is 0): pass NULL");
   if (save && workspace_bytes < p.total) return fail(NGM_E_WORKSPACE, "render_fwd: workspace too small");
   char* ws = reinterpret_cast<char*>(align_up((int64_t)workspace, 256));
   RenderFwdArgs a;
@@ -1107,7 +1142,7 @@
   if (fcfg->encoding == NGM_ENC_TRIPLANE) { ngm_launch_tri_finish(a, st); e = check_launch("ngm_tri_finish"); if (e) return e; }
   GradReduceArgs g;
   memset(&g.adam, 0, sizeof(g.adam));
-  if (adam) g.adam = *adam;
+  if (adam) { g.adam = *adam; g.img = params->b3_image; g.img_stride = params->b3_image_stride; }
   g.num_active = num_active;
   g.fc = *fcfg; g.gr = *grads; g.F = rays->F; g.blocks_per_field = a.blocks_per_field; g.partials = a.partials; g.p_pad = a.p_pad;
   bool mlp_reduced = false;
diff --git a/neural_graph_mapping_amd/csrc/ngm_field.h b/neural_graph_mapping_amd/csrc/ngm_field.h
--- a/neural_graph_mapping_amd/csrc/ngm_field.h
+++ b/neural_graph_mapping_amd/csrc/ngm_field.h
@@ -550,6 +550,48 @@
       P[plane + e4] = __builtin_bit_cast(ngm_u32x4, M);
       P[2 * plane + e4] = __builtin_bit_cast(ngm_u32x4, Lo);
     }
+  }
+}
+
+#define NGM_IMG_PLANE 512
+#define NGM_IMG_SET (3 * NGM_IMG_PLANE * 16)
+__host__ __device__ constexpr int64_t ngm_img_row_bytes(int L) { return (int64_t)L * NGM_IMG_SET; }
+__host__ __device__ constexpr int64_t ngm_img_dgrad_off(int l) { return (int64_t)l * NGM_IMG_SET; }
+__host__ __device__ constexpr int ngm_img_dgrad_slot(int o, int c) {
+  return (((((c >> 5) * 4 + (o >> 4)) * 2 + ((o >> 3) & 1)) * 32 + (c & 31)) << 3) + (o & 7);
+}
+__device__ __forceinline__ void b3_image_store(char* row_img, int l, int o, int c, float x) {
+  uint32_t h, m, lo;
+  b3_split(x, h, m, lo);
+  unsigned short* pd = reinterpret_cast<unsigned short*>(row_img + ngm_img_dgrad_off(l)) + ngm_img_dgrad_slot(o, c);
+  pd[0] = (unsigned short)(h >> 16); pd[NGM_IMG_PLANE * 8] = (unsigned short)(m >> 16); pd[2 * NGM_IMG_PLANE * 8] = (unsigned short)(lo >> 16);
+}
+__device__ __forceinline__ float ngm_stored_value(float v, int dt) {
+  if (dt == NGM_DT_F32) return v;
+  unsigned short h;
+  if (dt == NGM_DT_BF16) {
+    const uint32_t u = __float_as_uint(v);
+    h = (v != v) ? (unsigned short)0x7fc0 : (unsigned short)((u + 0x7fffu + ((u >> 16) & 1u)) >> 16);
+  } else {
+    h = __builtin_bit_cast(unsigned short, (_Float16)v);
+  }
+  return ngm_widen(h, dt);
+}
+__device__ __forceinline__ void b3_image_to_lds(const char* src, uint32_t lds_base, int bytes, int tid, int nthr) {
+  const uint32_t wave_off = (uint32_t)(tid & ~63) * 16u;
+  for (int b0 = 0; b0 < bytes; b0 += nthr * 16) {
+    const uint32_t m0v = __builtin_amdgcn_readfirstlane(lds_base + (uint32_t)b0 + wave_off);
+    const char* p = src + b0 + (size_t)tid * 16;
+    uint32_t keep;
+    asm volatile(
+        "s_mov_b32 %0, m0\n\t"
+        "s_mov_b32 m0, %2\n\t"
+        "s_nop 0\n\t"
+        "global_load_lds_dwordx4 %1, off\n\t"
+        "s_mov_b32 m0, %0"
+        : "=&s"(keep)
+        : "v"(p), "s"(m0v)
+        : "memory");
   }
 }
 
diff --git a/neural_graph_mapping_amd/csrc/ngm_field_bwd.hip b/neural_graph_mapping_amd/csrc/ngm_field_bwd.hip
--- a/neural_graph_mapping_amd/csrc/ngm_field_bwd.hip
+++ b/neural_graph_mapping_amd/csrc/ngm_field_bwd.hip
@@ -493,7 +493,10 @@
   for (int64_t p = threadIdx.x; p < ptot; p += NGM_BLOCK) dst[p] = red[p];
 }
 
-struct GradSeg { int64_t off, size; float* dst; int64_t stride; float* param; float* m; float* v; int64_t pstride; void* lp; int lp_dt; };
+struct GradSeg {
+  int64_t off, size; float* dst; int64_t stride; float* param; float* m; float* v; int64_t pstride; void* lp; int lp_dt;
+  int img_l, din;
+};
 struct GradReduceK {
   int F, blocks_per_field, nseg;
   const float* partials;
@@ -501,7 +504,13 @@
   GradSeg seg[2 * (NGM_MAX_LAYERS + 1) + 1];
   AdamHyper hyper;
   const int32_t* num_active;
+  char* img; int64_t img_stride;
 };
+__device__ __forceinline__ void grad_reduce_planes(const GradReduceK& a, const GradSeg& sg, int64_t row, int64_t i, float pn) {
+  if (!a.img || sg.img_l < 0) return;
+  const uint32_t iu = (uint32_t)i, o = iu / (uint32_t)sg.din, c = iu - o * (uint32_t)sg.din;
+  b3_image_store(a.img + row * a.img_stride, sg.img_l, (int)o, (int)c, sg.lp ? ngm_stored_value(pn, sg.lp_dt) : pn);
+}
 
 template <bool COUNTED>
 __global__ void __launch_bounds__(256) k_grad_reduce(GradReduceK a) {
@@ -512,7 +521,7 @@
   }
   const int64_t p = (int64_t)blockIdx.x * 64 + l;
   int seg = -1;
-  int64_t so = 0;
+  int64_t so = 0, row = 0;
   float pv = 0.f, m0 = 0.f, v0 = 0.f;
   AdamCoef co = {0.f, 1.f};
   const bool adam = q == 0 && p < a.ptot;
@@ -520,7 +529,7 @@
     for (int k = 0; k < a.nseg; ++k)
       if (p >= a.seg[k].off && p < a.seg[k].off + a.seg[k].size) { seg = k; break; }
     if (seg >= 0 && a.seg[seg].param) {
-      const int64_t row = a.hyper.field_index ? a.hyper.field_index[f] : f;
+      row = a.hyper.field_index ? a.hyper.field_index[f] : f;
       so = row * a.seg[seg].pstride + (p - a.seg[seg].off);
       pv = a.seg[seg].param[so]; m0 = a.seg[seg].m[so]; v0 = a.seg[seg].v[so];
     }
@@ -571,6 +580,7 @@
     a.seg[seg].m[so] = m0; a.seg[seg].v[so] = v0;
     a.seg[seg].param[so] = pn;
     if (a.seg[seg].lp) ngm_stp(a.seg[seg].lp, so, pn, a.seg[seg].lp_dt);
+    grad_reduce_planes(a, a.seg[seg], row, i, pn);
   }
 }
 
@@ -583,11 +593,11 @@
   int seg = -1;
   for (int k = 0; k < a.nseg; ++k)
     if (p >= a.seg[k].off && p < a.seg[k].off + a.seg[k].size) { seg = k; break; }
-  int64_t so = 0;
+  int64_t so = 0, row = 0;
   float pv = 0.f, m0 = 0.f, v0 = 0.f;
   const bool adam = seg >= 0 && a.seg[seg].param;
   if (adam) {
-    const int64_t row = a.hyper.field_index ? a.hyper.field_index[f] : f;
+    row = a.hyper.field_index ? a.hyper.field_index[f] : f;
     so = row * a.seg[seg].pstride + (p - a.seg[seg].off);
     pv = a.seg[seg].param[so]; m0 = a.seg[seg].m[so]; v0 = a.seg[seg].v[so];
   }
@@ -629,6 +639,7 @@
     a.seg[seg].m[so] = m0; a.seg[seg].v[so] = v0;
     a.seg[seg].param[so] = pn;
     if (a.seg[seg].lp) ngm_stp(a.seg[seg].lp, so, pn, a.seg[seg].lp_dt);
+    grad_reduce_planes(a, a.seg[seg], row, i, pn);
   }
 }
 template <bool COUNTED>
@@ -639,18 +650,20 @@
 static int build_grad_reduce(const GradReduceArgs& g, GradReduceK& k) {
   k.F = g.F; k.blocks_per_field = g.blocks_per_field; k.partials = g.partials; k.p_pad = g.p_pad;
   k.num_active = g.num_active;
+  k.img = nullptr; k.img_stride = 0;
   int64_t enc_off, w_off[NGM_MAX_LAYERS + 1], b_off[NGM_MAX_LAYERS + 1];
   k.ptot = ngm_param_offsets(&g.fc, &enc_off, w_off, b_off);
   int n = 0;
   if (g.fc.encoding == NGM_ENC_FOURIER) {
     const int64_t sz = (int64_t)(g.fc.raw_coords ? g.fc.dim_enc - 3 : g.fc.dim_enc) * 3;
-    k.seg[n++] = GradSeg{enc_off, sz, g.gr.enc_w, g.gr.enc_w_stride, nullptr, nullptr, nullptr, 0, nullptr, 0};
+    k.seg[n++] = GradSeg{enc_off, sz, g.gr.enc_w, g.gr.enc_w_stride, nullptr, nullptr, nullptr, 0, nullptr, 0, -1, 0};
   }
   for (int l = 0; l <= g.fc.num_layers; ++l) {
     const int din = (l == 0) ? g.fc.dim_enc : g.fc.dim_hidden + (g.fc.skip_mode == NGM_SKIP_CONCAT ? g.fc.dim_enc : 0);
     const int dout = (l == g.fc.num_layers) ? g.fc.dim_out : g.fc.dim_hidden;
-    k.seg[n++] = GradSeg{w_off[l], (int64_t)din * dout, g.gr.w[l], g.gr.w_stride[l], nullptr, nullptr, nullptr, 0, nullptr, 0};
-    k.seg[n++] = GradSeg{b_off[l], (int64_t)dout, g.gr.b[l], g.gr.b_stride[l], nullptr, nullptr, nullptr, 0, nullptr, 0};
+    k.seg[n++] = GradSeg{w_off[l], (int64_t)din * dout, g.gr.w[l], g.gr.w_stride[l], nullptr, nullptr, nullptr, 0, nullptr, 0,
+                         l < g.fc.num_layers ? l : -1, din};
+    k.seg[n++] = GradSeg{b_off[l], (int64_t)dout, g.gr.b[l], g.gr.b_stride[l], nullptr, nullptr, nullptr, 0, nullptr, 0, -1, 0};
   }
   k.nseg = n;
   k.hyper = AdamHyper{nullptr, nullptr, 1, 0.f, 0.f, 0.f, 0.f, 0.f};
@@ -663,6 +676,7 @@
       k.seg[i].lp = t.param_lp; k.seg[i].lp_dt = t.lp_dtype;
     }
     k.hyper = g.adam.hyper;
+    k.img = static_cast<char*>(g.img); k.img_stride = g.img_stride;
   }
   return 0;
 }
diff --git a/neural_graph_mapping_amd/csrc/ngm_field_bwd_b3.hip b/neural_graph_mapping_amd/csrc/ngm_field_bwd_b3.hip
--- a/neural_graph_mapping_amd/csrc/ngm_field_bwd_b3.hip
+++ b/neural_graph_mapping_amd/csrc/ngm_field_bwd_b3.hip
@@ -82,10 +82,11 @@
   }
 }
 
-template <int L, bool NEED_COS, bool ENC_GRAD, bool FC = false, bool HS = false, bool COUNTED = false>
+template <int L, bool NEED_COS, bool ENC_GRAD, bool FC = false, bool HS = false, bool COUNTED = false, bool IMG = false>
 __global__ __launch_bounds__(B3B_THREADS) void k_field_bwd_b3(FieldBwdArgs a) {
   extern __shared__ __attribute__((aligned(16))) float sm[];
   using LY = LdsB3b<L, ENC_GRAD, HS>;
+  static_assert(!IMG || !HS, "the half-stash instance builds its planes itself");
 #ifdef NGM_PROLOGUE_TIMING
   unsigned long long ptk_[8] = {0, 0, 0, 0, 0, 0, 0, 0};
   const unsigned long long pt0_ = __builtin_readcyclecounter();
@@ -201,14 +202,19 @@
     if constexpr (!HS) issue_tile32(fs.act[L - 1], fs.gb, first, end, lane, wl_lds + LY::HL * 4);
     if (L == 2) issue_tile32(fs.act[0], fs.gb, first, end, lane, wl_lds + LY::H1 * 4);
   }
+  if constexpr (IMG && LY::NPL > 0) {
+    constexpr int l0 = ENC_GRAD ? 0 : 1;
+    b3_image_to_lds(static_cast<const char*>(a.pr.b3_image) + row * a.pr.b3_image_stride + ngm_img_dgrad_off(l0),
+                    (uint32_t)(uintptr_t)(__attribute__((address_space(3))) char*)sm, LY::NPL * NGM_IMG_SET, threadIdx.x, B3B_THREADS);
+  }
   float4* cwout = reinterpret_cast<float4*>(sm + LY::CONSTS);
   float4* cenc = cwout + 64;
   __shared__ float s_red[FC ? 16 : 1][17];
   __shared__ float s_sums[NGM_NUM_LOSS_SUMS];
-  constexpr int NSETS = (ENC_GRAD ? 1 : 0) + (L == 2 ? 1 : 0) + (HS ? 1 : 0);
+  constexpr int NSETS = IMG ? 0 : (ENC_GRAD ? 1 : 0) + (L == 2 ? 1 : 0) + (HS ? 1 : 0);
   constexpr int NPX = NSETS > 0 ? NSETS * 16 : 1;
   float px_[NPX];
-  {
+  if constexpr (!IMG) {
     int off_[NPX];
     int si = 0;
     if (ENC_GRAD) { planes_offsets<false>(a.fc, 0, 0, *reinterpret_cast<int(*)[8]>(off_ + 16 * si)); planes_offsets<false>(a.fc, 0, 1, *reinterpret_cast<int(*)[8]>(off_ + 16 * si + 8)); ++si; }
@@ -256,7 +262,9 @@
       s_red[lpart][lslot] = s_;
     }
   }
-  {
+  if constexpr (IMG) {
+    DMA_WAIT(0);
+  } else {
     int si = 0;
     if (ENC_GRAD) { planes_commit<false>(a.fc, 0, 0, px_ + 16 * si, planes + LY::plane_slot(0) * 3 * PLANE_G); planes_commit<false>(a.fc, 0, 1, px_ + 16 * si + 8, planes + LY::plane_slot(0) * 3 * PLANE_G); ++si; }
     if (L == 2) { planes_commit<false>(a.fc, 1, 0, px_ + 16 * si, planes + LY::plane_slot(1) * 3 * PLANE_G); planes_commit<false>(a.fc, 1, 1, px_ + 16 * si + 8, planes + LY::plane_slot(1) * 3 * PLANE_G); ++si; }
@@ -790,6 +798,20 @@
   } while (0)
 #define NGM_LBB3_ONE(NC, EG, FC_)                                                                                     \
   do {                                                                                                                \
+    if constexpr (!HS && !(NC)) {                                                                                     \
+      if (a.pr.b3_image) {                          \
+        if (a.num_active) {                                                                                           \
+          (void)hipFuncSetAttribute((const void*)k_field_bwd_b3<L, NC, EG, FC_, HS, true, true>,                      \
+                                    hipFuncAttributeMaxDynamicSharedMemorySize, (int)lds);                            \
+          hipLaunchKernelGGL((k_field_bwd_b3<L, NC, EG, FC_, HS, true, true>), dim3(blocks), dim3(B3B_THREADS), lds, st, a); \
+        } else {                                                                                                      \
+          (void)hipFuncSetAttribute((const void*)k_field_bwd_b3<L, NC, EG, FC_, HS, false, true>,                     \
+                                    hipFuncAttributeMaxDynamicSharedMemorySize, (int)lds);                            \
+          hipLaunchKernelGGL((k_field_bwd_b3<L, NC, EG, FC_, HS, false, true>), dim3(blocks), dim3(B3B_THREADS), lds, st, a); \
+        }                                                                                                             \
+        break;                                                                                                        \
+      }                                                                                                               \
+    }                                                                                                                 \
     if (a.num_active) {                                                                                               \
       (void)hipFuncSetAttribute((const void*)k_field_bwd_b3<L, NC, EG, FC_, HS, true>, hipFuncAttributeMaxDynamicSharedMemorySize, \
                                 (int)lds);                                                                            \
diff --git a/neural_graph_mapping_amd/csrc/ngm_field_fwd.hip b/neural_graph_mapping_amd/csrc/ngm_field_fwd.hip
--- a/neural_graph_mapping_amd/csrc/ngm_field_fwd.hip
+++ b/neural_graph_mapping_amd/csrc/ngm_field_fwd.hip
@@ -646,6 +646,39 @@
 #endif
 }
 
+struct B3ImageArgs { ngm_field_cfg fc; ngm_params pr; };
+__global__ __launch_bounds__(256) void k_b3_image_build(B3ImageArgs a) {
+  const int64_t row = a.pr.field_index ? a.pr.field_index[blockIdx.x] : (int64_t)blockIdx.x;
+  const int l = (int)blockIdx.y;
+  const int Din = (l == 0) ? a.fc.dim_enc : a.fc.dim_hidden, H = a.fc.dim_hidden;
+  const float* W = a.pr.w[l];
+  const int64_t w0 = row * a.pr.w_stride[l];
+  ngm_u32x4* P = reinterpret_cast<ngm_u32x4*>(static_cast<char*>(a.pr.b3_image) + row * a.pr.b3_image_stride + ngm_img_dgrad_off(l));
+  for (int g = threadIdx.x; g < NGM_IMG_PLANE; g += 256) {
+    const int n = g & 31, kh = (g >> 5) & 1, kb = (g >> 6) & 3, nt = g >> 8;
+    const int c = 32 * nt + n;
+    float x[8];
+#pragma unroll
+    for (int e = 0; e < 8; ++e) {
+      const int o = 16 * kb + 8 * kh + e;
+      x[e] = (o < H && c < Din) ? ngm_ldp(W, w0 + (int64_t)o * Din + c, a.pr.dtype) : 0.f;
+    }
+    ngm_bf16x8 h, m, lo;
+    b3_split8(x, h, m, lo);
+    P[g] = __builtin_bit_cast(ngm_u32x4, h);
+    P[NGM_IMG_PLANE + g] = __builtin_bit_cast(ngm_u32x4, m);
+    P[2 * NGM_IMG_PLANE + g] = __builtin_bit_cast(ngm_u32x4, lo);
+  }
+}
+int64_t ngm_b3_image_row_bytes(const ngm_field_cfg& fc) { return ngm_fwd_split_takes(fc) ? ngm_img_row_bytes(fc.num_layers) : 0; }
+int ngm_launch_b3_image_build(const ngm_field_cfg& fc, const ngm_params& pr, int num_rows, hipStream_t st) {
+  if (!ngm_fwd_split_takes(fc) || !pr.b3_image || num_rows < 1) return NGM_E_INVALID;
+  B3ImageArgs a;
+  a.fc = fc; a.pr = pr;
+  hipLaunchKernelGGL(k_b3_image_build, dim3((unsigned)num_rows, (unsigned)fc.num_layers), dim3(256), 0, st, a);
+  return 0;
+}
+
 static bool fwd_shape_compiled(const ngm_field_cfg& fc) { return ngm_fwd_lds_bytes(fc, false, 0, 0) >= 0; }
 int64_t ngm_fwd_lds_bytes(const ngm_field_cfg& fc, bool b3, int waves, int maxs) {
   const FieldShape s = field_shape(&fc);
diff --git a/neural_graph_mapping_amd/csrc/ngm_launch.h b/neural_graph_mapping_amd/csrc/ngm_launch.h
--- a/neural_graph_mapping_amd/csrc/ngm_launch.h
+++ b/neural_graph_mapping_amd/csrc/ngm_launch.h
@@ -121,6 +121,7 @@
   int64_t p_pad;
   GradAdam adam;
   const int32_t* num_active = nullptr;
+  void* img = nullptr; int64_t img_stride = 0;
 };
 
 struct CompositeArgs {
@@ -193,6 +194,8 @@
 bool ngm_knn_eval_takes(const ngm_field_cfg& fc, bool b3);
 int64_t ngm_fwd_lds_bytes(const ngm_field_cfg& fc, bool b3, int waves, int maxs);
 int ngm_launch_points_fwd(const PointsFwdArgs& a, const FwdPlan& p, hipStream_t st);
+int64_t ngm_b3_image_row_bytes(const ngm_field_cfg& fc);
+int ngm_launch_b3_image_build(const ngm_field_cfg& fc, const ngm_params& pr, int num_rows, hipStream_t st);
 int64_t ngm_encode_bwd_fourier_scratch(int F, int64_t P);
 int ngm_launch_encode_bwd_fourier(const ngm_field_cfg& fc, const ngm_params& pr, int F, int64_t P, const float* points,
                                   const float* pos, const float* quat, const float* d_enc, float* grad, int64_t grad_stride,
diff --git a/neural_graph_mapping_amd/ops.py b/neural_graph_mapping_amd/ops.py
--- a/neural_graph_mapping_amd/ops.py
+++ b/neural_graph_mapping_amd/ops.py
@@ -825,6 +825,10 @@
                                           int(bool(advance and step_dev is not None)),
                                           _ptr(philox_offset_dev) if advance else None, _stream()),
             "ngm_adam_sparse_multi")
+    for n in names:
+        torch.autograd.graph.increment_version(params[n])
+        if lp is not None:
+            torch.autograd.graph.increment_version(lp[n])
 
 
 def keyframes_struct(c2ws, rgbd_store, frame_to_store, fx, fy, cx, cy) -> K.Keyframes:
diff --git a/neural_graph_mapping_amd/renderer.py b/neural_graph_mapping_amd/renderer.py
--- a/neural_graph_mapping_amd/renderer.py
+++ b/neural_graph_mapping_amd/renderer.py
@@ -144,6 +144,7 @@
         self._step = 0
         self._step_dev = None
         self._ws_cache = {}
+        self._pimg = None
         self.process_group = None
         self.eval_fused = True
         self.eval_fallbacks = []
@@ -272,6 +273,7 @@
             ops.fields_append(tensors, positions, orientations, rs["positions"], rs["orientations"], rs["training_iterations"],
                               rs["num_fields_dev"], first)
             m._set_num(first + num_new)
+            self._planes_invalidate()
         self._set_num(first + num_new)
 
     def add_fields(self, num_new: int, positions: Optional[torch.Tensor] = None, orientations: Optional[torch.Tensor] = None):
@@ -562,6 +564,7 @@
         if self._step_dev is not None:
             self._step_dev.fill_(self._step)
         self._model.refresh_lp()
+        self._planes_invalidate()
         self._count_training_iteration(fids, None)
         return out
 
@@ -820,6 +823,46 @@
         mse = ((prediction.clamp(0.0, 1.0) - target.clamp(0.0, 1.0)) ** 2).mean()
         return float(10.0 * torch.log10(1.0 / mse))
 
+    def _hidden_weights(self):
+        kp = self._model.kernel_params()
+        names = [n for n in K.param_names(self._fc) if n.startswith("_linears.") and n.endswith(".weight")]
+        return kp, [kp[n] for n in names[:self._fc.num_layers]]
+
+    def _planes_invalidate(self) -> None:
+        if isinstance(self._pimg, dict):
+            self._pimg["sig"] = None
+
+    def _plane_image(self) -> Optional[torch.Tensor]:
+        st = self._pimg
+        if st is False:
+            return None
+        fc = self._fc
+        if st is None:
+            nb = int(K.lib().ngm_b3_image_bytes(C.byref(fc)))
+            if nb <= 0:
+                self._pimg = False
+                return None
+            st = self._pimg = dict(bytes=nb, t=None, sig=None, keep=None)
+        kp, ws = self._hidden_weights()
+        num = ws[0].shape[0]
+        if num == 0:
+            return None
+        mr = self._model._reserved
+        cap = mr["max"] if mr is not None else num
+        if st["t"] is None or st["t"].shape[0] != cap or st["t"].device != ws[0].device:
+            st["t"], st["sig"] = torch.zeros(cap, st["bytes"], dtype=torch.uint8, device=ws[0].device), None
+        sig = tuple((w.data_ptr(), w._version, w.shape[0], w.dtype) for w in ws)
+        if sig != st["sig"]:
+            ps = ops.params_struct(fc, {n: kp[n] for n in K.param_names(fc)}, None)
+            ps.b3_image, ps.b3_image_stride = st["t"].data_ptr(), st["t"].stride(0)
+            K.check(K.lib().ngm_b3_image_build(C.byref(fc), C.byref(ps), num, ops._stream()), "ngm_b3_image_build")
+            st["sig"], st["keep"] = sig, ws
+        return st["t"]
+
+    def _planes_sync(self) -> None:
+        if isinstance(self._pimg, dict) and self._pimg["t"] is not None:
+            self._plane_image()
+
     def _workspace(self, F, R):
         key = (F, R)
         if key not in self._ws_cache:
@@ -832,7 +875,8 @@
                 rgbds=torch.empty(F, R, 4, device=dev), color_vars=torch.empty(F, R, 3, device=dev),
                 depth_vars=torch.empty(F, R, device=dev), term_probs=torch.empty(F, R, device=dev),
                 sums=torch.zeros(K.NGM_NUM_LOSS_SUMS, device=dev), loss=torch.zeros(8, device=dev),
-                philox=torch.zeros(1, device=dev, dtype=torch.int64))
+                philox=torch.zeros(1, device=dev, dtype=torch.int64),
+                planes=K.lib().ngm_b3_image_takes(C.byref(self._fc), C.byref(self._rc_train), F, R) == 1)
         return self._ws_cache[key]
 
     def optimization_iteration(self, target: Target, u_coarse=None, u_guided=None, seed=0, update=True) -> dict:
@@ -929,6 +973,9 @@
             kernel_p["_neus_sd"] = self._model.all_fields_params["_neus_sd"]
         ps = ops.params_struct(fc, kernel_p, fids)
         w = self._workspace(F, R)
+        img = self._plane_image() if w["planes"] else None
+        if img is not None:
+            ps.b3_image, ps.b3_image_stride = img.data_ptr(), img.stride(0)
         keep = []
         if self._step_dev is None:
             self._step_dev = torch.full((1,), self._step, device=self._device, dtype=torch.int64)
@@ -981,6 +1028,8 @@
             fn += "_counted"
             args.append(count.data_ptr())
         K.check(getattr(L, fn)(*args), fn)
+        if update and not ps.b3_image:
+            self._planes_invalidate()
         if update:
             self._step += 1
         if update and count is None:
@@ -1043,6 +1092,7 @@
             self._step = step0
 
             def replay():
+                self._planes_sync()
                 graph.replay()
                 self._step += 1
                 if self.peer_exchange is not None:
@@ -1066,6 +1116,7 @@
         sums, group = ctx["w"]["sums"], self.process_group
 
         def replay2():
+            self._planes_sync()
             g1.replay()
             torch.distributed.all_reduce(sums, group=group)
             g2.replay()
```

Measured after the change: 2.232 billion ray-samples/s (median of 4 runs). No clear change (+0.1%).
